# kfkq/DQMC

Measured on AMD Instinct MI355X. Metric: MC sweeps/sec, 2D Hubbard N=256 Ltau=200, higher is better.
Workload: dtype f64; 1 GPU; cfg3: 16x16 Hubbard U=8.0 beta=8.0 Ltau=200 n_stab=10 t=1 mu=-0.1; chains_per_gpu=1, n_chains_total=1, parallelism=independent chains, 1 gpu x 1 chain

## Files before the change

### dqmc_amd/csrc/common.h

```cpp
#pragma once

#include <hip/hip_runtime.h>
#include <cstdint>
#include <memory>
#include <string>

struct dqmc_engine;

namespace dq {

constexpr int WAVE = 64;

void set_error(const std::string& msg);
const char* get_error();

#define DQ_HIP(call)                                                                    \
    do {                                                                                \
        hipError_t _e = (call);                                                         \
        if (_e != hipSuccess) {                                                         \
            ::dq::set_error(std::string(#call) + ": " + hipGetErrorString(_e));         \
            return -2;                                              \
        }                                                                               \
    } while (0)

#define DQ_TRY(expr)                \
    do {                            \
        int _rc = (expr);           \
        if (_rc != 0) return _rc;   \
    } while (0)

template <class T, hipError_t (*Free)(void*)> struct HipDelete { void operator()(T* p) const { (void)Free(p); } };
template <class T> using DevPtr = std::unique_ptr<T[], HipDelete<T, hipFree>>;
using PinnedPtr = std::unique_ptr<char[], HipDelete<char, hipHostFree>>;
template <class T> int dev_alloc(DevPtr<T>& out, size_t count) {
    void* p = nullptr;
    DQ_HIP(hipMalloc(&p, sizeof(T) * count));
    out.reset(static_cast<T*>(p));
    return 0;
}

constexpr int DQ_STATUS_PIVOT = 1;
constexpr int DQ_STATUS_COOP_QR = 2;
constexpr int DQ_STATUS_HANDOFF = 4;
constexpr int DQ_STATUS_CENSUS = 8;

struct Mat {
    double* p = nullptr;
    long stride = 0;
    __host__ __device__ double* at(int c) const { return p + (long)c * stride; }
};
struct CMat {
    const double* p = nullptr;
    long stride = 0;
    CMat() = default;
    __host__ __device__ CMat(const double* p_, long s) : p(p_), stride(s) {}
    __host__ __device__ CMat(const Mat& m) : p(m.p), stride(m.stride) {}
    __host__ __device__ const double* at(int c) const { return p + (long)c * stride; }
};
using Vec = Mat;
using CVec = CMat;

struct GemmDesc {
    CMat A, B;
    Mat C;
    Mat CT{nullptr, 0};
    CVec rs, ks, cs;
    int n = 0;
    int transA = 0;
    int accumulate = 0;
};
int launch_gemm(const GemmDesc& g, int n_chains, hipStream_t s);

int launch_build_expv(const int8_t* fields, long f_stride, int nt, int n, const double* tab_expv ,
                      double* expv, double* invexpv, long v_stride, int n_chains, hipStream_t s);
int launch_split_d(CVec d, Vec dl_inv, Vec ds, double* logsum, int n, int n_chains, hipStream_t s);
int launch_split_d2(CVec d1, Vec dl1, Vec ds1, CVec d2, Vec dl2, Vec ds2, int n, int n_chains, hipStream_t s);
int launch_measure_equal_time(CMat G, double* out, long out_stride, int L1, int L2, int accumulate, int n_chains, hipStream_t s);
int launch_measure_unequal_time(const double* Gtt, const double* Gt0, const double* G0t, double* out, long out_stride, int L1, int L2, int nt,
                                int accumulate, int n_chains, hipStream_t s);
int launch_axpb_identity(CMat in, Mat out, double a, double b, int n, int n_chains, hipStream_t s);
int launch_copy(CMat in, Mat out, long count, int n_chains, hipStream_t s);
int launch_set_identity(Mat out, int n, int n_chains, hipStream_t s);
int launch_transpose_scale(CMat in, Mat out, CVec rs, int n, int n_chains, hipStream_t s);
int launch_max_abs_diff(CMat A, CMat B, double* err, long err_stride, int n, int n_chains, hipStream_t s);
int launch_add_scaled_cols(CMat A, CMat B, CVec cs, Mat C, int n, int n_chains, hipStream_t s);
int launch_scale_rows(CMat in, CVec rs, Mat out, int n, int n_chains, hipStream_t s);
struct DevStats { double acc_rate, max_err, sum_err, n_err; long long n_accepted, n_proposed; };
int launch_fold_stats(DevStats* st, const int* acc, long acc_stride, int n_slices, const double* err, long err_stride, int n_err,
                      int n, int nt, int n_chains, hipStream_t s);

struct QrWork {
    double* tau; long tau_stride;
    int* jpvt; long jpvt_stride;
    unsigned long long* sync = nullptr; long sync_stride = 0;
    int* abort_words = nullptr;
    int* info = nullptr;
    double* pw = nullptr; long pw_stride = 0;
    bool pw_two_launch = false;
    int* pivpos = nullptr; long pivpos_stride = 0;
    bool pw_compact = true;
};
bool qr_panel_fused_fits(int n);
bool qr_panel_fused_default(int n);
long qr_panel_work_doubles(int n, bool two_launch);
int launch_qr_panel(Mat A, Mat L, QrWork w, int n, int n_chains, hipStream_t s);
long qrcp_coop_sync_granules(int n);
int qrcp_coop_workgroups(int n, int n_chains);
enum class QrFamily { Panel, ColumnOwner, Cooperative, Streaming };
int launch_to_ldr(QrFamily f, Mat A, Mat L, Vec d, Mat R, QrWork w, int n, int n_chains, hipStream_t s);

int launch_lu_blocked(Mat A, int* perm, long perm_stride, int* rowpos, long rowpos_stride, double* logabsdet, int accumulate_logdet,
                      int* info, int n, int n_chains, hipStream_t s);
int launch_lu_solve(CMat LU, const int* perm, long perm_stride, Mat X, CVec dg, int mode, int n, int n_chains, hipStream_t s);

int launch_tri_solve(CMat R, const int* perm, long perm_stride, Mat X, CVec dg, double* scratch, long scratch_stride, int n, int n_chains, hipStream_t s);

bool gj_fused_fits(int n);
bool gj_fused_default(int n);
int launch_gj_solve(Mat A, Mat B, Mat X, Mat SA, double* tinv, int* perm, long perm_stride, int* rowpos, int* rowpos_alt, long rowpos_stride,
                    double* logabsdet, int accumulate_logdet, int* info, int n, int n_chains, bool fused, bool compact, hipStream_t s);

struct UpdateTables {
    double rb[4][3];
    double delta[4][3];
    double ev[4];
    double iev[4];
    double pad[32];
};
struct SliceRider {
    const double* A = nullptr; const double* B = nullptr; double* C = nullptr; const double* rs = nullptr; const double* ks = nullptr;
    __host__ __device__ GemmDesc gemm(int n) const { GemmDesc g; g.A = CMat(A, 0); g.B = CMat(B, 0); g.C = Mat{C, 0}; g.rs = CVec(rs, 0); g.ks = CVec(ks, 0); g.n = n; return g; }
};
struct UpdateDesc {
    Mat G;
    int8_t* fields; long f_stride;
    double* expv; double* invexpv; long v_stride;
    const UpdateTables* tabs;
    const int32_t* perm; const uint8_t* kprop; const double* u; long rs_stride;
    double* Upanel; double* Wpanel; long panel_stride;
    double* Cpanel = nullptr;
    int* state; long state_stride;
    double* prep; long prep_stride;
    Mat GT{nullptr, 0};
    int gt_valid = 0;
    void* slice_sync = nullptr;
    unsigned slice_epoch = 0;
    int slice_absent_tile = -1;
    int slice_absent_l = -1;
    int slice_late_tile = -1, slice_late_us = 0;
    int* info = nullptr;
    int* acc_out; long acc_stride;
    int n, nt;
    SliceRider rider;
};
constexpr int UPDATE_KD = 32;

struct SliceSync {
    unsigned long long seq; unsigned int error; unsigned int solo_count; unsigned int pad[12];
    unsigned int arrive[496];
};
constexpr size_t SLICE_SYNC_BYTES = 2048;
static_assert(sizeof(SliceSync) == SLICE_SYNC_BYTES, "SliceSync layout");
constexpr unsigned SLICE_EPOCH_LIMIT = 1u << 24;
constexpr unsigned SLICE_SOLO_BIT = 1u << 30, SLICE_FINAL_BIT = 1u << 31;
constexpr int SLICE_RING_ROWS = 2 * UPDATE_KD;
constexpr unsigned SLICE_K_MASK = 0xffu, SLICE_BASE_SHIFT = 8, SLICE_BASE_MASK = SLICE_RING_ROWS - 1;
__host__ __device__ inline unsigned slice_tag(unsigned epoch, unsigned window) { return (epoch << 8) | window; }
enum class SlicePath { PersistentWalk, PersistentWalkDump, PersistentSubmatrix, Solo, Pairs, PairsTailSolo };
int launch_update_slice(SlicePath path, const UpdateDesc& d, int l, int acc_slot, int n_chains, hipStream_t s);
int launch_update_slice_sm(const UpdateDesc& d, int l, int acc_slot, int n_chains, hipStream_t s);
int slice_flush_workgroups(int n);
bool slice_reserve(int device, int n, int n_chains);
void slice_release(int device, int n, int n_chains);
int launch_rank1(Mat G, int i, double delta, double* scratch , long scratch_stride, int n, int n_chains, hipStream_t s);

int launch_rng_fill(int32_t* perm, uint8_t* kprop, double* u, int n, int nt, unsigned long long seed, unsigned first_chain, unsigned h,
                    int n_chains, hipStream_t s);

struct CbDesc {
    CMat in;
    Mat out{nullptr, 0}, outT{nullptr, 0};
    const int* partner = nullptr;
// ... 20 lines not shown
```

### dqmc_amd/csrc/elementwise.hip

```cpp
#include "common.h"
#include "wave.h"

namespace dq {

__global__ void build_expv_kernel(const int8_t* fields, long f_stride, long total, const double* tab,
                                  double* expv, double* invexpv, long v_stride) {
    const int c = blockIdx.y;
    const double* t = tab + (long)c * 8;
    for (long k = blockIdx.x * (long)blockDim.x + threadIdx.x; k < total; k += (long)gridDim.x * blockDim.x) {
        const int f = fields[(long)c * f_stride + k] & 3;
        expv[(long)c * v_stride + k] = t[f];
        invexpv[(long)c * v_stride + k] = t[4 + f];
    }
}
int launch_build_expv(const int8_t* fields, long f_stride, int nt, int n, const double* tab, double* expv, double* invexpv,
                      long v_stride, int n_chains, hipStream_t s) {
    const long total = (long)nt * n;
    dim3 grid((unsigned)((total + 255) / 256 > 512 ? 512 : (total + 255) / 256), n_chains);
    hipLaunchKernelGGL(build_expv_kernel, grid, dim3(256), 0, s, fields, f_stride, total, tab, expv, invexpv, v_stride);
    DQ_HIP(hipGetLastError());
    return 0;
}

__global__ void split_d_kernel(CVec d, Vec dl_inv, Vec ds, double* logsum, int n) {
// ... 70 lines not shown
    const int ti = blockIdx.x % tiles, tj = blockIdx.x / tiles;
    const int tx = threadIdx.x & 31, ty = threadIdx.x >> 5;
    for (int r = ty; r < 32; r += 8) {
        const int i = ti * 32 + tx, j = tj * 32 + r;
        tile[r][tx] = (i < n && j < n) ? a[i + (long)n * j] : 0.0;
    }
    __syncthreads();
    for (int r = ty; r < 32; r += 8) {
        const int i = tj * 32 + tx, j = ti * 32 + r;
        if (i < n && j < n) {
            double v = tile[tx][r];
            if (rs.p) v *= rs.at(c)[i];
            o[i + (long)n * j] = v;
        }
    }
}
int launch_transpose_scale(CMat in, Mat out, CVec rs, int n, int n_chains, hipStream_t s) {
    const int tiles = (n + 31) / 32;
    hipLaunchKernelGGL(transpose_scale_kernel, dim3(tiles * tiles, n_chains), dim3(256), 0, s, in, out, rs, n, tiles);
    DQ_HIP(hipGetLastError());
    return 0;
}

__global__ __launch_bounds__(256) void max_abs_diff_kernel(CMat A, CMat B, double* err, long err_stride, int n) {
    const int c = blockIdx.y;
    const double* __restrict__ a = A.at(c); const double* __restrict__ b = B.at(c);
    const long total = (long)n * n;
    unsigned long long m = 0ULL;
    for (long k = (long)blockIdx.x * blockDim.x + threadIdx.x; k < total; k += (long)gridDim.x * blockDim.x) {
        const unsigned long long d = (unsigned long long)__double_as_longlong(fabs(a[k] - b[k]));
        m = d > m ? d : m;
    }
    m = wave_max_u64(m);
    __shared__ unsigned long long red[4];
    if ((threadIdx.x & 63) == 0) red[threadIdx.x >> 6] = m;
    __syncthreads();
    if (threadIdx.x == 0) {
        unsigned long long r = red[0];
        for (int q = 1; q < 4; ++q) r = red[q] > r ? red[q] : r;
        atomicMax(reinterpret_cast<unsigned long long*>(err + (long)c * err_stride), r);
    }
}
int launch_max_abs_diff(CMat A, CMat B, double* err, long err_stride, int n, int n_chains, hipStream_t s) {
    const long total = (long)n * n;
    const long want = (total + 4095) / 4096;
    const int blocks = (int)(want < 1 ? 1 : (want > 16 ? 16 : want));
    hipLaunchKernelGGL(max_abs_diff_kernel, dim3(blocks, n_chains), dim3(256), 0, s, A, B, err, err_stride, n);
    DQ_HIP(hipGetLastError());
    return 0;
}

__global__ void add_scaled_cols_kernel(CMat A, CMat B, CVec cs, Mat C, int n) {
    const int c = blockIdx.y;
    const double* a = A.at(c); const double* b = B.at(c); double* o = C.at(c);
    const long total = (long)n * n;
    for (long k = blockIdx.x * (long)blockDim.x + threadIdx.x; k < total; k += (long)gridDim.x * blockDim.x) {
        double bv = b[k];
        if (cs.p) bv *= cs.at(c)[k / n];
        o[k] = a[k] + bv;
    }
}
int launch_add_scaled_cols(CMat A, CMat B, CVec cs, Mat C, int n, int n_chains, hipStream_t s) {
    const long total = (long)n * n;
    long blocks = (total + 255) / 256; if (blocks > 1024) blocks = 1024;
    hipLaunchKernelGGL(add_scaled_cols_kernel, dim3((unsigned)blocks, n_chains), dim3(256), 0, s, A, B, cs, C, n);
    DQ_HIP(hipGetLastError());
    return 0;
}

__global__ void scale_rows_kernel(CMat in, CVec rs, Mat out, int n) {
    const int c = blockIdx.y;
    const double* a = in.at(c); double* o = out.at(c); const double* r = rs.at(c);
    const long total = (long)n * n;
    for (long k = blockIdx.x * (long)blockDim.x + threadIdx.x; k < total; k += (long)gridDim.x * blockDim.x) o[k] = a[k] * r[k % n];
}
int launch_scale_rows(CMat in, CVec rs, Mat out, int n, int n_chains, hipStream_t s) {
    const long total = (long)n * n;
    long blocks = (total + 255) / 256; if (blocks > 1024) blocks = 1024;
    hipLaunchKernelGGL(scale_rows_kernel, dim3((unsigned)blocks, n_chains), dim3(256), 0, s, in, rs, out, n);
    DQ_HIP(hipGetLastError());
    return 0;
}

__global__ void fold_stats_kernel(DevStats* st, const int* acc, long acc_stride, int n_slices, const double* err, long err_stride,
                                  int n_err, int n, int nt, int n_chains) {
    const int c = blockIdx.x * blockDim.x + threadIdx.x;
    if (c >= n_chains) return;
    DevStats s = st[c];
    for (int k = 0; k < n_slices; ++k) {
        const int a = acc[(long)c * acc_stride + k];
        s.acc_rate += (static_cast<double>(a) / n) / nt;
        s.n_accepted += a; s.n_proposed += n;
    }
    for (int k = 0; k < n_err; ++k) {
        const double e = err[(long)c * err_stride + k];
        if (e > s.max_err || e != e) s.max_err = e;
        s.sum_err += e; s.n_err += 1.0;
    }
    st[c] = s;
}
int launch_fold_stats(DevStats* st, const int* acc, long acc_stride, int n_slices, const double* err, long err_stride, int n_err,
                      int n, int nt, int n_chains, hipStream_t s) {
    hipLaunchKernelGGL(fold_stats_kernel, dim3((n_chains + 63) / 64), dim3(64), 0, s, st, acc, acc_stride, n_slices, err, err_stride, n_err, n, nt, n_chains);
    DQ_HIP(hipGetLastError());
    return 0;
}


__global__ __launch_bounds__(1024) void measure_equal_time_kernel(CMat Gm, double* out_p, long out_stride, int L1, int L2, int accumulate) {
    __shared__ double red[3][16];
    __shared__ double s_navg;
    const int chain = blockIdx.y;
    const int n = L1 * L2;
    const double* __restrict__ G = Gm.at(chain);
    double* out = out_p + (long)chain * out_stride;
    const int t = threadIdx.x, lane = t & 63, wave = t >> 6, nwaves = (blockDim.x + 63) >> 6;
    double dens = 0.0, docc = 0.0, sw = 0.0;
    if (t < n) {
        const double c = 1.0 - G[t + (long)n * t];
        dens = 2.0 * c; docc = c * c;
        for (int j = 0; j < n; ++j) { const double x = (j == t ? 1.0 : 0.0) - G[j + (long)n * t]; sw += x * x; }
    }
    dens = wave_sum(dens); docc = wave_sum(docc); sw = wave_sum(sw);
    if (lane == 0) { red[0][wave] = dens; red[1][wave] = docc; red[2][wave] = sw; }
    __syncthreads();
    if (t == 0) {
        double a = 0.0, b = 0.0, c = 0.0;
        for (int q = 0; q < nwaves; ++q) { a += red[0][q]; b += red[1][q]; c += red[2][q]; }
        a /= n; b /= n; c /= n;
        s_navg = a;
        if (accumulate) { out[0] += a; out[1] += b; out[2] += c; } else { out[0] = a; out[1] = b; out[2] = c; }
    }
    __syncthreads();
    if (t < n) {
        const int dx = (t % L1) - (L1 / 2 - 1), dy = (t / L1) - (L2 / 2 - 1);
        const double navg = s_navg;
        double acc = 0.0;
        for (int i = 0; i < n; ++i) {
            const int xi = i % L1, yi = i / L1;
            const int xj = ((xi + dx) % L1 + L1) % L1, yj = ((yi + dy) % L2 + L2) % L2;
            const int j = yj * L1 + xj;
            const double ni = 2.0 * (1.0 - G[i + (long)n * i]), nj = 2.0 * (1.0 - G[j + (long)n * j]);
            acc += ni * nj + 2.0 * (1.0 - G[j + (long)n * i]) * G[i + (long)n * j] - navg * navg;
        }
        acc /= n;
        if (accumulate) out[3 + t] += acc; else out[3 + t] = acc;
    }
}

int launch_measure_equal_time(CMat G, double* out, long out_stride, int L1, int L2, int accumulate, int n_chains, hipStream_t s) {
    const int n = L1 * L2;
    if (n < 1 || n > 1024) { set_error("measure_equal_time: L1*L2 must be in 1..1024"); return -1; }
    const int threads = ((n + 63) / 64) * 64;
    hipLaunchKernelGGL(measure_equal_time_kernel, dim3(1, n_chains), dim3(threads), 0, s, G, out, out_stride, L1, L2, accumulate);
    DQ_HIP(hipGetLastError());
    return 0;
}


__global__ void axpb_identity_kernel(CMat in, Mat out, double a, double b, int n) {
    const int chain = blockIdx.y;
    const double* x = in.at(chain);
    double* y = out.at(chain);
    const long nn = (long)n * n;
    for (long k = (long)blockIdx.x * blockDim.x + threadIdx.x; k < nn; k += (long)gridDim.x * blockDim.x)
        y[k] = a * x[k] + ((k % n) == (k / n) ? b : 0.0);
}
int launch_axpb_identity(CMat in, Mat out, double a, double b, int n, int n_chains, hipStream_t s) {
    hipLaunchKernelGGL(axpb_identity_kernel, dim3(64, n_chains), dim3(256), 0, s, in, out, a, b, n);
    DQ_HIP(hipGetLastError());
    return 0;
}


__global__ __launch_bounds__(1024) void measure_unequal_time_kernel(const double* Gtt_p, const double* Gt0_p, const double* G0t_p, double* out_p,
                                                                    long out_stride, int L1, int L2, int nt, int accumulate, int n_chains) {
    const int tau = blockIdx.x, chain = blockIdx.y;
    const int n = L1 * L2;
    const long nn = (long)n * n;
    const double* __restrict__ Gtt = Gtt_p + ((long)tau * n_chains + chain) * nn;
    const double* __restrict__ Gt0 = Gt0_p + ((long)tau * n_chains + chain) * nn;
    const double* __restrict__ G0t = G0t_p + ((long)tau * n_chains + chain) * nn;
    const double* __restrict__ G00 = Gtt_p + (long)chain * nn;
    double* out = out_p + (long)chain * out_stride;
    const int t = threadIdx.x;
    if (t >= n) return;
// ... 34 lines not shown
```

### dqmc_amd/csrc/engine.hip

```cpp
#include "common.h"
#include "../../include/dqmc_hip.h"

#include <cmath>
#include <cstdlib>
#include <cstring>
#include <map>
#include <memory>
#include <mutex>
#include <vector>

namespace dq {

static thread_local std::string g_err;
void set_error(const std::string& msg) { g_err = msg; }
const char* get_error() { return g_err.c_str(); }

int init_device_kernels(int device) {
    static std::mutex mu; static bool done[64] = {};
    std::lock_guard<std::mutex> lk(mu);
    if (device < 0 || device >= 64) { set_error("device ordinal out of range"); return -1; }
    if (done[device]) return 0;
    DQ_HIP(hipSetDevice(device));
    DQ_TRY(update_init_device()); DQ_TRY(update_sm_init_device()); DQ_TRY(qr_init_device()); DQ_TRY(qr_colown_init_device());
    done[device] = true;
    return 0;
}

struct Switches { bool qr_panel; int qr_panel_fused, gj_fused; bool qr_streaming, walk_submatrix, lu_classic, slice_multikernel, bbar_rider, slice_stream, panel_compact; };
static const Switches& switches() {
    static const Switches sw = [] {
        const char* panel = getenv("DQMC_QR_PANEL");
        const char* fused = getenv("DQMC_QR_PANEL_FUSED");
        const char* gj = getenv("DQMC_GJ_FUSED");
        const char* rider = getenv("DQMC_BBAR_RIDER");
        const char* stream = getenv("DQMC_SLICE_STREAM");
        const char* compact = getenv("DQMC_PANEL_COMPACT");
        return Switches{!(panel && atoi(panel) == 0), fused ? (atoi(fused) != 0 ? 1 : 0) : -1, gj ? (atoi(gj) != 0 ? 1 : 0) : -1, getenv("DQMC_QR_STREAMING") != nullptr, getenv("DQMC_WALK_SUBMATRIX") != nullptr,
                        getenv("DQMC_LU_CLASSIC") != nullptr, getenv("DQMC_SLICE_MULTIKERNEL") != nullptr, !(rider && atoi(rider) == 0), !(stream && atoi(stream) == 0), !(compact && atoi(compact) == 0)};
    }();
    return sw;
}

constexpr int GJ_MAX_N = 1024, GJ_MAX_CHAINS = 8;
constexpr int TRI_MAX_N = 640;

static QrFamily pick_qr(int n, int chains, bool allow_panel) {
    const Switches& sw = switches();
    if (sw.qr_streaming) return QrFamily::Streaming;
    if (allow_panel && sw.qr_panel && n >= 64 && n <= 1024 && n % 16 == 0 && chains <= 8) return QrFamily::Panel;
    if (n <= 256) return QrFamily::ColumnOwner;
    return qrcp_coop_workgroups(n, chains) <= 200 ? QrFamily::Cooperative : QrFamily::Streaming;
}

struct KernelPlan {
    QrFamily qr;
    enum class Solve { GaussJordan, BlockedLu } solve;
    enum class Rinv { Blocked, PerColumn } rinv;
    static KernelPlan pick(int n, int chains) {
        return KernelPlan{pick_qr(n, chains, true),
                          n <= GJ_MAX_N && chains <= GJ_MAX_CHAINS && !switches().lu_classic ? Solve::GaussJordan : Solve::BlockedLu,
                          n <= TRI_MAX_N ? Rinv::Blocked : Rinv::PerColumn};
    }
};

static SlicePath pick_slice_path(int n, int chains, bool reserved) {
    const Switches& sw = switches();
    const bool walk = n <= 256;
    if (sw.slice_multikernel) return SlicePath::Pairs;
    if (reserved) return walk && !sw.walk_submatrix ? (sw.slice_stream ? SlicePath::PersistentWalk : SlicePath::PersistentWalkDump) : SlicePath::PersistentSubmatrix;
    if (!walk) return SlicePath::Pairs;
    return chains >= 224 ? SlicePath::Solo : SlicePath::PairsTailSolo;
}
static bool is_persistent_walk(SlicePath p) { return p == SlicePath::PersistentWalk || p == SlicePath::PersistentWalkDump; }
static bool is_persistent(SlicePath p) { return is_persistent_walk(p) || p == SlicePath::PersistentSubmatrix; }

struct LdrRef {
    Mat L; Vec d; Mat R;
    int* jpvt = nullptr;
    bool* tri = nullptr;
    Mat X{nullptr, 0};
    bool* xok = nullptr;
    void touch() const { if (xok) *xok = false; }
};
struct LdrStore {
    int n = 0, C = 0;
    DevPtr<double> L, d, R, X;
    DevPtr<int> jpvt;
    std::unique_ptr<bool[]> tri, xok;
    int alloc(int k, int n_, int C_, bool with_x = false) {
        n = n_; C = C_;
        const size_t nn = (size_t)n * n;
        DQ_TRY(dev_alloc(L, (size_t)k * C * nn)); DQ_TRY(dev_alloc(d, (size_t)k * C * n));
        DQ_TRY(dev_alloc(R, (size_t)k * C * nn)); DQ_TRY(dev_alloc(jpvt, (size_t)k * C * n));
        if (with_x) DQ_TRY(dev_alloc(X, (size_t)k * C * nn));
        tri.reset(new bool[k]()); xok.reset(new bool[k]());
        return 0;
    }
    LdrRef at(int i) const {
        const long nn = (long)n * n;
        LdrRef f{Mat{L.get() + (long)i * C * nn, nn}, Vec{d.get() + (long)i * C * n, (long)n}, Mat{R.get() + (long)i * C * nn, nn},
                 jpvt.get() + (long)i * C * n, &tri[i]};
        if (X) { f.X = Mat{X.get() + (long)i * C * nn, nn}; f.xok = &xok[i]; }
        return f;
    }
};

struct Ctx {
    int n = 0, C = 0, device = 0;
    long nn = 0;
    hipStream_t stream = nullptr;
    static constexpr int NT = 6, NV = 5;
    DevPtr<double> pool;
    DevPtr<double> vpool;
    DevPtr<int> ipool;
    DevPtr<unsigned long long> qsync;
    DevPtr<int> qabort;
    DevPtr<double> tinv;
    DevPtr<double> qpw;
    bool gj_fused = false;
    bool qpw_two_launch = false;
    DevPtr<int> qpivpos;
    DevPtr<double> trinv;
    KernelPlan plan{};

    Mat T(int k) const { return Mat{pool.get() + (long)k * C * nn, nn}; }
    Vec V(int k) const { return Vec{vpool.get() + (long)k * C * n, (long)n}; }
    int* jpvt() const { return ipool.get(); }
    int* lperm() const { return ipool.get() + (long)C * n; }
    int* rowpos() const { return ipool.get() + 2L * C * n; }
    int* rowpos_alt() const { return ipool.get() + 3L * C * n; }
    int* info() const { return ipool.get() + 4L * C * n; }

    int init(int n_, int C_, int device_) {
        n = n_; C = C_; device = device_; nn = (long)n * n;
        DQ_HIP(hipSetDevice(device));
        DQ_TRY(init_device_kernels(device));
        DQ_HIP(hipStreamCreateWithFlags(&stream, hipStreamNonBlocking));
        DQ_TRY(dev_alloc(pool, (size_t)NT * C * nn));
        DQ_TRY(dev_alloc(vpool, (size_t)NV * C * n));
        DQ_TRY(dev_alloc(ipool, 4L * C * n + 4));
        plan = KernelPlan::pick(n, C);
        if (plan.qr == QrFamily::Cooperative) { DQ_TRY(dev_alloc(qsync, (size_t)qrcp_coop_sync_granules(n) * C)); DQ_TRY(dev_alloc(qabort, C)); }
        if (plan.qr == QrFamily::Panel) {
            const int fused = switches().qr_panel_fused;
            qpw_two_launch = !(fused < 0 ? qr_panel_fused_default(n) : fused == 1 && qr_panel_fused_fits(n));
            const size_t qpw_count = (size_t)qr_panel_work_doubles(n, qpw_two_launch) * C;
            DQ_TRY(dev_alloc(qpw, qpw_count)); DQ_TRY(dev_alloc(qpivpos, (size_t)n * C));
            DQ_HIP(hipMemsetAsync(qpw.get(), 0, sizeof(double) * qpw_count, stream));
        }
        if (plan.solve == KernelPlan::Solve::GaussJordan) {
            DQ_TRY(dev_alloc(tinv, (size_t)2048 * C));
            const int fused = switches().gj_fused;
            gj_fused = fused < 0 ? gj_fused_default(n) : fused == 1 && gj_fused_fits(n);
        }
        if (plan.rinv == KernelPlan::Rinv::Blocked) DQ_TRY(dev_alloc(trinv, (size_t)16 * (n + 16) * C));
        DQ_HIP(hipMemsetAsync(ipool.get(), 0, sizeof(int) * (4L * C * n + 4), stream));
        return 0;
    }
    ~Ctx() { if (stream) (void)hipStreamDestroy(stream); }

    int gemm(CMat A, CMat B, Mat Cm, CVec rs = CVec(), CVec ks = CVec(), CVec cs = CVec(), int transA = 0, int accumulate = 0, Mat CT = Mat{nullptr, 0}) {
        GemmDesc g; g.A = A; g.B = B; g.C = Cm; g.CT = CT; g.rs = rs; g.ks = ks; g.cs = cs; g.n = n; g.transA = transA; g.accumulate = accumulate;
        return launch_gemm(g, C, stream);
    }
    int to_ldr(Mat A, LdrRef out, bool direct = true) {
        const bool keep = direct && out.jpvt != nullptr;
        QrWork w{V(4).p, (long)n, keep ? out.jpvt : jpvt(), (long)n};
        w.sync = qsync.get(); w.sync_stride = qrcp_coop_sync_granules(n); w.abort_words = qabort.get(); w.info = info();
        w.pw = qpw.get(); w.pw_stride = qr_panel_work_doubles(n, qpw_two_launch); w.pw_two_launch = qpw_two_launch; w.pivpos = qpivpos.get(); w.pivpos_stride = n;
        w.pw_compact = switches().panel_compact;
        if (out.tri) *out.tri = keep;
        out.touch();
        return launch_to_ldr(plan.qr, A, out.L, out.d, out.R, w, n, C, stream);
    }
    int r_inverse_scaled(LdrRef F, CVec dinv, Mat scratch, Mat lu_scratch, Mat* Xout) {
        const Mat X = F.X.p ? F.X : scratch;
        *Xout = X;
        if (F.xok && *F.xok) return 0;
        if (F.tri && *F.tri && F.jpvt) {
            if (plan.rinv == KernelPlan::Rinv::Blocked) DQ_TRY(launch_tri_solve(F.R, F.jpvt, n, X, dinv, trinv.get(), 16L * (n + 16), n, C, stream));
            else DQ_TRY(launch_lu_solve(F.R, F.jpvt, n, X, dinv, 2, n, C, stream));
        } else {
            DQ_TRY(launch_copy(F.R, lu_scratch, nn, C, stream));
            DQ_TRY(launch_lu_blocked(lu_scratch, lperm(), n, rowpos(), n, nullptr, 0, info(), n, C, stream));
            DQ_TRY(launch_lu_solve(lu_scratch, lperm(), n, X, dinv, 1, n, C, stream));
        }
        if (F.xok) *F.xok = true;
        return 0;
    }
    int mat_mul_ldr(CMat M, LdrRef F, LdrRef out) {
        DQ_TRY(gemm(M, F.L, T(0), CVec(), CVec(), CVec(F.d)));
        LdrRef q{out.L, out.d, T(1)};
        DQ_TRY(to_ldr(T(0), q));
        if (out.tri) *out.tri = false;
        out.touch();
        return gemm(T(1), F.R, out.R);
    }
    int ldr_mul_mat(LdrRef F, CMat M, LdrRef out) {
        DQ_TRY(gemm(F.R, M, T(0), CVec(F.d)));
        LdrRef q{T(1), out.d, out.R, out.jpvt, out.tri};
        q.xok = out.xok;
        DQ_TRY(to_ldr(T(0), q));
        return gemm(F.L, T(1), out.L);
    }
    int ldr_mul_ldr(LdrRef F1, LdrRef F2, LdrRef out) {
        DQ_TRY(gemm(F1.R, F2.L, T(0), CVec(F1.d), CVec(), CVec(F2.d)));
        LdrRef q{T(1), out.d, T(2)};
        DQ_TRY(to_ldr(T(0), q));
        if (out.tri) *out.tri = false;
        out.touch();
        DQ_TRY(gemm(F1.L, T(1), out.L));
        return gemm(T(2), F2.R, out.R);
    }
    int solve(Mat M, Mat RHS, Mat out, double* logdet_acc, Mat* Y) {
        if (plan.solve == KernelPlan::Solve::GaussJordan) {
            DQ_TRY(launch_gj_solve(M, RHS, out, T(5), tinv.get(), lperm(), n, rowpos(), rowpos_alt(), n, logdet_acc, 1, info(), n, C, gj_fused, switches().panel_compact, stream));
            *Y = out; return 0;
        }
        DQ_TRY(launch_lu_blocked(M, lperm(), n, rowpos(), n, logdet_acc, 1, info(), n, C, stream));
        DQ_TRY(launch_lu_solve(M, lperm(), n, RHS, CVec(), 0, n, C, stream));
        *Y = RHS; return 0;
    }
    int inv_I_plus_ldr(LdrRef F, Mat G, double* logdet ) {
        DQ_TRY(launch_split_d(F.d, V(0), V(1), logdet, n, C, stream));
        Mat X; DQ_TRY(r_inverse_scaled(F, V(0), T(1), T(0), &X));
        DQ_TRY(launch_add_scaled_cols(X, F.L, V(1), T(2), n, C, stream));
        DQ_TRY(launch_transpose_scale(T(2), T(3), CVec(), n, C, stream));
        DQ_TRY(launch_transpose_scale(X, T(4), CVec(), n, C, stream));
        Mat Y; DQ_TRY(solve(T(3), T(4), T(0), logdet, &Y));
        return launch_transpose_scale(Y, G, CVec(), n, C, stream);
    }
    int inv_I_plus_ldr_mul_ldr(LdrRef F1, LdrRef F2, Mat G, Mat GT = Mat{nullptr, 0}) {
        DQ_TRY(launch_split_d2(F1.d, V(0), V(1), F2.d, V(2), V(3), n, C, stream));
        Mat X; DQ_TRY(r_inverse_scaled(F2, V(2), T(1), T(0), &X));
        DQ_TRY(gemm(F1.L, X, T(2), V(0), CVec(), CVec(), 1));
        DQ_TRY(gemm(F1.R, F2.L, T(2), V(1), CVec(), V(3), 0, 1));
        DQ_TRY(launch_transpose_scale(F1.L, T(3), V(0), n, C, stream));
        Mat Y; DQ_TRY(solve(T(2), T(3), T(0), nullptr, &Y));
        return gemm(X, Y, G, CVec(), CVec(), CVec(), 0, 0, GT);
    }
    int inv_invldr_plus_ldr(LdrRef F1, LdrRef F2, Mat G, bool negate) {
        DQ_TRY(launch_split_d(F1.d, V(0), V(1), nullptr, n, C, stream));
        DQ_TRY(launch_split_d(F2.d, V(2), V(3), nullptr, n, C, stream));
        Mat X; DQ_TRY(r_inverse_scaled(F2, V(2), T(1), T(0), &X));
        DQ_TRY(gemm(F1.L, X, T(2), V(0), CVec(), CVec(), 1));
        DQ_TRY(gemm(F1.R, F2.L, T(2), V(1), CVec(), V(3), 0, 1));
        DQ_TRY(launch_scale_rows(F1.R, V(1), T(3), n, C, stream));
        Mat Y; DQ_TRY(solve(T(2), T(3), T(0), nullptr, &Y));
        DQ_TRY(gemm(X, Y, G));
        if (negate) DQ_TRY(launch_axpb_identity(G, G, -1.0, 0.0, n, C, stream));
        return 0;
    }
};

static int take_status(const Ctx& c, int* bits = nullptr) {
    int w[4] = {0, 0, 0, 0};
    DQ_HIP(hipMemcpy(w, c.info(), sizeof w, hipMemcpyDeviceToHost));
    if (bits) *bits = w[0];
    if (w[0] == 0) return 0;
    (void)hipMemset(c.info(), 0, sizeof w);
    if (w[0] & DQ_STATUS_HANDOFF) {
        set_error("persistent slice kernel: a workgroup that had checked in stopped answering (device fault or pre-emption beyond the spin bound); the chain state is undefined -- set the fields again and call dqmc_init; this engine uses the scan / flush kernel pairs from now on");
    } else if (w[0] & DQ_STATUS_CENSUS) {
        char msg[640];
        snprintf(msg, sizeof msg, "persistent sub-matrix slice kernel: its workgroups did not all become resident at time slice %d (device shared with other "
                 "work?).  That slice and every later slice of the call(s) in flight proposed NOTHING (fields unchanged there, acceptance counts 0, their part of "
                 "the random stream is spent); wraps and stabilisations ran, so fields, G and the stack are consistent with each other, but the sweep is not the "
                 "one the stream describes from that slice on.  This engine uses the scan / flush kernel pairs from now on: restore the fields of the last "
                 "completed sweep and call dqmc_init, or keep the state as a valid (shortened) sweep", w[1] - 1);
        set_error(msg);
    } else if (w[0] & DQ_STATUS_COOP_QR) {
        set_error("cooperative QRCP gave up waiting for a partner workgroup (not co-resident?)");
    } else {
        set_error("LU factorisation hit a zero or NaN pivot");
    }
    return DQMC_ENUMERIC;
}

struct Engine {
    int n = 0, nt = 0, n_stab = 0, n_stack = 0, C = 1, device = 0;
    long nn = 0;
    std::vector<int> loc_l_end;
    std::vector<double> g_host, gamma_host, eta_host;
    std::vector<unsigned char> seen;
    Ctx ctx;
    hipStream_t s = nullptr;

    DevPtr<double> expK, invexpK;
    bool cb = false; int cb_groups = 0;
    DevPtr<int> cb_partner;
    DevPtr<double> cb_par;
    DevPtr<int8_t> fields;
    DevPtr<double> expv, invexpv;
    DevPtr<UpdateTables> tabs; DevPtr<double> tab8;
    bool gt_valid = false;
    bool gt_check = false; long long gt_checks = 0; DevPtr<double> gt_err;
    DevPtr<double> G, Gtmp, GT;
    DevPtr<double> pg_eye, pg_ones;
    DevPtr<double> bb0, bb1;
    long long rider_launches = 0;
    LdrStore stack;
    LdrStore spare;
    DevPtr<double> logdet;
    DevPtr<int32_t> rs_perm; DevPtr<uint8_t> rs_k; DevPtr<double> rs_u;
    PinnedPtr h_stage;
    bool rng_seeded = false; uint64_t rng_seed = 0; uint32_t rng_first_chain = 0, rng_counter = 0;
    hipEvent_t stage_free = nullptr;
    DevPtr<double> Upanel, Wpanel;
    int panel_rows = UPDATE_KD;
    DevPtr<double> Cpanel;
    struct InitBatch { DevPtr<double> bb, tau; LdrStore f; } ib;
    DevPtr<int> state;
    DevPtr<double> prep;
    DevPtr<double> meas_now, meas_sum;
    struct UnequalTime { DevPtr<double> G[3], tmp, err, meas_now, meas_sum; LdrStore bt; } ut;
    bool ut_valid = false; long long ut_meas_count = 0;
    struct HalfWarp { DevPtr<double> expK, invexpK, out; } hw;
    long long meas_count = 0;
    DevPtr<char> slice_sync;
    bool reserved = false;
    SlicePath slice_path = SlicePath::Pairs;
    unsigned slice_epoch = 0;
    int slice_absent_l = -1;
    int slice_late_tile = -1, slice_late_us = 0;
    int slice_absent_tile = -1;
    DevPtr<int> acc;
    struct Exchange { DevPtr<int8_t> saved, recv; DevPtr<int> tab; } xch;
    DevPtr<double> err;
    DevPtr<DevStats> dstats;
    bool stack_valid = false;
    bool profiling = false;
    std::vector<std::pair<hipEvent_t, hipEvent_t>> ev_pairs;
    size_t ev_used = 0;
    double upd_ms = 0.0; long long upd_launches = 0; long long upd_accept_base = 0;

    Mat mG() const { return Mat{G.get(), nn}; }
    CVec ev(int l) const { return CVec(expv.get() + (long)l * n, (long)nt * n); }
    CVec iev(int l) const { return CVec(invexpv.get() + (long)l * n, (long)nt * n); }
    int stack_idx(int l) const { return l / n_stab; }
    int local_l(int l) const { return l % n_stab; }

    ~Engine() {
        if (s) (void)hipStreamSynchronize(s);
        if (reserved) slice_release(device, n, C);
        for (auto& p : ev_pairs) { (void)hipEventDestroy(p.first); (void)hipEventDestroy(p.second); }
        if (stage_free) (void)hipEventDestroy(stage_free);
    }

    int create(int device_, int C_, int n_, int nt_, int n_stab_, const double* g, const double* gamma, const double* eta,
               const double* eK, const double* ieK) {
        device = device_; C = C_; n = n_; nt = nt_; n_stab = n_stab_; nn = (long)n * n;
        n_stack = (int)std::ceil(static_cast<double>(nt) / n_stab);
        loc_l_end.assign(n_stack, n_stab - 1);
        if (nt % n_stab != 0) loc_l_end[n_stack - 1] = nt % n_stab - 1;
        g_host.assign(g, g + C); gamma_host.assign(gamma, gamma + 4); eta_host.assign(eta, eta + 4);
        DQ_TRY(ctx.init(n, C, device)); s = ctx.stream;
        reserved = slice_reserve(device, n, C);
        slice_path = pick_slice_path(n, C, reserved);
        if (const char* a = getenv("DQMC_DEBUG_SLICE_ABSENT")) { slice_absent_tile = atoi(a); if (const char* c = strchr(a, ':')) slice_absent_l = atoi(c + 1); }
        if (const char* a = getenv("DQMC_DEBUG_SLICE_LATE")) { slice_late_tile = atoi(a); if (const char* c = strchr(a, ':')) slice_late_us = atoi(c + 1); }
        DQ_TRY(dev_alloc(expK, C * nn)); DQ_TRY(dev_alloc(invexpK, C * nn));
        DQ_TRY(dev_alloc(fields, (size_t)C * nt * n)); DQ_TRY(dev_alloc(expv, (size_t)C * nt * n)); DQ_TRY(dev_alloc(invexpv, (size_t)C * nt * n));
        DQ_TRY(dev_alloc(tabs, C)); DQ_TRY(dev_alloc(tab8, (size_t)C * 8));
        if (C == 1) { DQ_TRY(dev_alloc(pg_eye, nn)); DQ_TRY(dev_alloc(pg_ones, (size_t)n)); DQ_TRY(launch_set_identity(Mat{pg_eye.get(), nn}, n, 1, s)); const std::vector<double> one_h((size_t)n, 1.0); DQ_HIP(hipMemcpy(pg_ones.get(), one_h.data(), sizeof(double) * n, hipMemcpyHostToDevice)); }
        DQ_TRY(dev_alloc(G, C * nn)); DQ_TRY(dev_alloc(Gtmp, C * nn)); DQ_TRY(dev_alloc(GT, C * nn)); DQ_TRY(dev_alloc(bb0, C * nn)); DQ_TRY(dev_alloc(bb1, C * nn));
        DQ_TRY(stack.alloc(n_stack, n, C, C <= 8)); DQ_TRY(spare.alloc(1, n, C));
        DQ_TRY(dev_alloc(logdet, C));
        DQ_TRY(dev_alloc(rs_perm, (size_t)C * nt * n)); DQ_TRY(dev_alloc(rs_k, (size_t)C * nt * n)); DQ_TRY(dev_alloc(rs_u, (size_t)C * nt * n));
        panel_rows = slice_path == SlicePath::PersistentWalk ? SLICE_RING_ROWS : UPDATE_KD;
        DQ_TRY(dev_alloc(Upanel, (size_t)C * panel_rows * n)); DQ_TRY(dev_alloc(Wpanel, (size_t)C * panel_rows * n)); DQ_TRY(dev_alloc(Cpanel, (size_t)C * UPDATE_KD * UPDATE_KD));
        DQ_TRY(dev_alloc(state, (size_t)C * 4)); DQ_TRY(dev_alloc(prep, (size_t)C * 4 * n)); DQ_TRY(dev_alloc(meas_now, (size_t)C * (3 + n))); DQ_TRY(dev_alloc(meas_sum, (size_t)C * (3 + n))); DQ_HIP(hipMemsetAsync(meas_sum.get(), 0, sizeof(double) * C * (3 + n), s)); DQ_TRY(dev_alloc(slice_sync, (size_t)C * SLICE_SYNC_BYTES)); DQ_HIP(hipMemsetAsync(slice_sync.get(), 0, (size_t)C * SLICE_SYNC_BYTES, s)); DQ_TRY(dev_alloc(acc, (size_t)C * nt)); DQ_TRY(dev_alloc(err, (size_t)C * n_stack));
        DQ_TRY(dev_alloc(dstats, C));
        void* stage = nullptr;
        DQ_HIP(hipHostMalloc(&stage, (size_t)C * nt * n * (sizeof(int32_t) + sizeof(uint8_t) + sizeof(double)), hipHostMallocDefault)); h_stage.reset(static_cast<char*>(stage));
        DQ_HIP(hipEventCreateWithFlags(&stage_free, hipEventDisableTiming));
        DQ_HIP(hipEventRecord(stage_free, s));
        DQ_HIP(hipMemcpyAsync(expK.get(), eK, sizeof(double) * C * nn, hipMemcpyHostToDevice, s));
        DQ_HIP(hipMemcpyAsync(invexpK.get(), ieK, sizeof(double) * C * nn, hipMemcpyHostToDevice, s));
        DQ_HIP(hipMemsetAsync(fields.get(), 0, (size_t)C * nt * n, s));
        DQ_HIP(hipMemsetAsync(G.get(), 0, sizeof(double) * C * nn, s));
        DQ_HIP(hipMemsetAsync(dstats.get(), 0, sizeof(DevStats) * C, s));
        DQ_HIP(hipMemsetAsync(logdet.get(), 0, sizeof(double) * C, s));
        DQ_HIP(hipMemsetAsync(state.get(), 0, sizeof(int) * C * 4, s));
        std::vector<UpdateTables> ht(C); std::vector<double> h8((size_t)C * 8);
        static const int proposal[4][3] = {{1, 2, 3}, {0, 2, 3}, {0, 1, 3}, {0, 1, 2}};
        const double alpha = -1.0;
        for (int c = 0; c < C; ++c) {
            std::memset(&ht[c], 0, sizeof(UpdateTables));
            for (int o = 0; o < 4; ++o) for (int k = 0; k < 3; ++k) {
                const int nf = proposal[o][k];
                const double gammaR = gamma[nf] / gamma[o];
                const double d_eta = eta[nf] - eta[o];
                const double bosonR = std::exp(alpha * g[c] * d_eta);
                ht[c].rb[o][k] = gammaR * bosonR;
                ht[c].delta[o][k] = (1.0 / bosonR) - 1.0;
            }
            for (int f = 0; f < 4; ++f) { ht[c].ev[f] = std::exp(g[c] * eta[f]); ht[c].iev[f] = std::exp(-g[c] * eta[f]); h8[(size_t)c * 8 + f] = ht[c].ev[f]; h8[(size_t)c * 8 + 4 + f] = ht[c].iev[f]; }
        }
        DQ_HIP(hipMemcpyAsync(tabs.get(), ht.data(), sizeof(UpdateTables) * C, hipMemcpyHostToDevice, s));
        DQ_HIP(hipMemcpyAsync(tab8.get(), h8.data(), sizeof(double) * C * 8, hipMemcpyHostToDevice, s));
        DQ_TRY(launch_build_expv(fields.get(), (long)nt * n, nt, n, tab8.get(), expv.get(), invexpv.get(), (long)nt * n, C, s));
        DQ_HIP(hipStreamSynchronize(s));
        return 0;
    }

    int cb_apply(CMat in, Mat out, Mat outT, bool reverse, bool inverse, CVec rs_in, CVec cs_in, CVec rs_out, CVec cs_out, int chains, long par_stride) {
        CbDesc d; d.in = in; d.out = out; d.outT = outT; d.partner = cb_partner.get(); d.n_groups = cb_groups; d.reverse = reverse ? 1 : 0; d.inverse = inverse ? 1 : 0;
        d.par = cb_par.get(); d.par_stride = par_stride; d.rs_in = rs_in; d.cs_in = cs_in; d.rs_out = rs_out; d.cs_out = cs_out; d.n = n;
        return launch_cb_apply(d, chains, s);
    }
    int set_checkerboard(int n_groups, const int32_t* bonds, const int32_t* group_sizes, const double* ch, const double* sh, const double* f) {
        if (n_groups < 1 || n_groups > 64 || !bonds || !group_sizes || !ch || !sh || !f) { set_error("set_checkerboard: bad argument"); return DQMC_EINVAL; }
        if (n > 4096) { set_error("set_checkerboard: n_sites > 4096"); return DQMC_EINVAL; }
        std::vector<int> partner((size_t)n_groups * n);
        size_t b = 0;
        for (int g = 0; g < n_groups; ++g) {
            int* pt = partner.data() + (size_t)g * n;
            for (int i = 0; i < n; ++i) pt[i] = i;
            if (group_sizes[g] < 0 || group_sizes[g] > n / 2) { set_error("set_checkerboard: a group holds at most n_sites/2 bonds"); return DQMC_EINVAL; }
            for (int k = 0; k < group_sizes[g]; ++k, ++b) {
                const int i = bonds[2 * b], j = bonds[2 * b + 1];
                if (i < 0 || i >= n || j < 0 || j >= n || i == j) { set_error("set_checkerboard: bond site out of range"); return DQMC_EINVAL; }
                if (pt[i] != i || pt[j] != j) { set_error("set_checkerboard: the bonds of one group must be disjoint"); return DQMC_EINVAL; }
                pt[i] = j; pt[j] = i;
            }
        }
        std::vector<double> par((size_t)C * 4);
        for (int c = 0; c < C; ++c) {
            if (!(f[c] > 0.0) || !std::isfinite(ch[c]) || !std::isfinite(sh[c])) { set_error("set_checkerboard: diag_factor must be positive, cosh / sinh finite"); return DQMC_EINVAL; }
            par[4 * c] = ch[c]; par[4 * c + 1] = sh[c]; par[4 * c + 2] = f[c]; par[4 * c + 3] = 1.0 / f[c];
        }
        DQ_HIP(hipStreamSynchronize(s));
        if (!cb_par) DQ_TRY(dev_alloc(cb_par, (size_t)C * 4));
        DevPtr<int> pt;
        DQ_TRY(dev_alloc(pt, partner.size()));
        DQ_HIP(hipMemcpy(pt.get(), partner.data(), sizeof(int) * partner.size(), hipMemcpyHostToDevice));
        DQ_HIP(hipMemcpy(cb_par.get(), par.data(), sizeof(double) * par.size(), hipMemcpyHostToDevice));
        cb_partner = std::move(pt); cb_groups = n_groups; cb = true;
        Mat id{bb0.get(), nn};
        DQ_TRY(launch_set_identity(id, n, C, s));
        DQ_TRY(cb_apply(id, Mat{expK.get(), nn}, Mat{nullptr, 0}, false, false, CVec(), CVec(), CVec(), CVec(), C, 4));
        DQ_TRY(cb_apply(id, Mat{invexpK.get(), nn}, Mat{nullptr, 0}, true, true, CVec(), CVec(), CVec(), CVec(), C, 4));
        stack_valid = false; gt_valid = false; ut_valid = false;
        DQ_HIP(hipStreamSynchronize(s));
        return 0;
    }

    int Bbar(int is, Mat* out) {
        const int l0 = is * n_stab;
        Mat cur{bb0.get(), nn}, nxt{bb1.get(), nn};
        DQ_TRY(launch_scale_rows(CMat(expK.get(), nn), ev(l0), cur, n, C, s));
        for (int loc = 1; loc <= loc_l_end[is]; ++loc) {
            if (cb) DQ_TRY(cb_apply(cur, nxt, Mat{nullptr, 0}, false, false, CVec(), CVec(), ev(l0 + loc), CVec(), C, 4));
            else DQ_TRY(ctx.gemm(CMat(expK.get(), nn), cur, nxt, ev(l0 + loc)));
// ... 77 lines not shown
        gt_valid = use_gt();
        GemmDesc g; g.A = CMat(ctx.T(0).p, (long)(Pprev - ctx.T(0).p)); g.B = CMat(expK.get(), 0); g.C = Mat{G.get(), (long)(Pnext - G.get())};
        g.ks = CVec(expv.get() + (long)l * n, 0); g.n = n;
        if (use_gt()) g.CT = Mat{GT.get(), (long)(ctx.T(1).p - GT.get())};
        return launch_gemm(g, 2, s);
    }
    int wrap_backward(int l) {
        if (cb) {
            DQ_TRY(cb_apply(mG(), Mat{nullptr, 0}, ctx.T(0), true, true, iev(l), ev(l), CVec(), CVec(), C, 4));
            gt_valid = use_gt();
            return cb_apply(ctx.T(0), Mat{GT.get(), nn}, mG(), true, false, CVec(), CVec(), CVec(), CVec(), C, 4);
        }
        DQ_TRY(ctx.gemm(CMat(invexpK.get(), nn), mG(), ctx.T(0), CVec(), iev(l)));
        gt_valid = use_gt();
        return ctx.gemm(ctx.T(0), CMat(expK.get(), nn), mG(), CVec(), ev(l), CVec(), 0, 0, use_gt() ? Mat{GT.get(), nn} : Mat{nullptr, 0});
    }
    bool use_gt() const { return n <= 256 || slice_path == SlicePath::PersistentSubmatrix; }
    UpdateDesc udesc() const {
        UpdateDesc d; d.G = mG(); d.fields = fields.get(); d.f_stride = (long)nt * n; d.expv = expv.get(); d.invexpv = invexpv.get(); d.v_stride = (long)nt * n;
        d.tabs = tabs.get(); d.perm = rs_perm.get(); d.kprop = rs_k.get(); d.u = rs_u.get(); d.rs_stride = (long)nt * n; d.Upanel = Upanel.get(); d.Wpanel = Wpanel.get(); d.Cpanel = Cpanel.get();
        d.panel_stride = (long)panel_rows * n; d.state = state.get(); d.state_stride = 4; d.prep = prep.get(); d.prep_stride = 4L * n; d.slice_sync = is_persistent(slice_path) ? slice_sync.get() : nullptr; d.slice_epoch = slice_epoch; d.slice_absent_tile = slice_absent_tile; d.slice_absent_l = slice_absent_l; d.slice_late_tile = slice_late_tile; d.slice_late_us = slice_late_us; d.GT = Mat{GT.get(), nn}; d.gt_valid = gt_valid ? 1 : 0; d.info = ctx.info(); d.acc_out = acc.get(); d.acc_stride = nt; d.n = n; d.nt = nt;
        return d;
    }
    int local_update(int l, const SliceRider* rider = nullptr) {
        hipEvent_t e0 = nullptr, e1 = nullptr;
        if (profiling) {
            if (ev_used == ev_pairs.size()) { hipEvent_t a, b; DQ_HIP(hipEventCreate(&a)); DQ_HIP(hipEventCreate(&b)); ev_pairs.emplace_back(a, b); }
            e0 = ev_pairs[ev_used].first; e1 = ev_pairs[ev_used].second; ++ev_used;
            DQ_HIP(hipEventRecord(e0, s));
        }
        if (is_persistent(slice_path)) {
            if (++slice_epoch >= SLICE_EPOCH_LIMIT) { DQ_HIP(hipMemsetAsync(slice_sync.get(), 0, (size_t)C * SLICE_SYNC_BYTES, s)); slice_epoch = 1; }
        }
        UpdateDesc d = udesc();
        if (rider) d.rider = *rider;
        DQ_TRY(launch_update_slice(slice_path, d, l, l, C, s));
        if (rider) ++rider_launches;
        if (profiling) DQ_HIP(hipEventRecord(e1, s));
        return 0;
    }
    int check_stream(const char* who, const int32_t* perm, const uint8_t* kprop, const double* u, size_t rows) {
        if (!perm || !kprop || !u) { set_error(std::string(who) + ": null random-stream pointer"); return DQMC_EINVAL; }
        seen.assign((size_t)n, 0);
        for (size_t row = 0; row < rows; ++row) {
            const int32_t* pr = perm + row * n; const uint8_t* kr = kprop + row * n; const unsigned char mark = (unsigned char)(1 + (row & 1));
            if ((row & 1) == 0) std::fill(seen.begin(), seen.end(), 0);
            for (int idx = 0; idx < n; ++idx) {
                const int32_t i = pr[idx];
                if (i < 0 || i >= n || seen[i] == mark || kr[idx] > 2) { set_error(std::string(who) + ": perm is not a permutation of the sites, or kprop > 2"); return DQMC_EINVAL; }
                seen[i] = mark;
            }
        }
        return 0;
    }
    int upload_stream(const int32_t* perm, const uint8_t* kprop, const double* u) {
        const size_t cnt = (size_t)C * nt * n;
        DQ_TRY(check_stream("sweep", perm, kprop, u, (size_t)C * nt));
        DQ_HIP(hipEventSynchronize(stage_free));
        char* base = h_stage.get();
        double* hu = reinterpret_cast<double*>(base);
        int32_t* hp = reinterpret_cast<int32_t*>(base + cnt * sizeof(double));
        uint8_t* hk = reinterpret_cast<uint8_t*>(base + cnt * (sizeof(double) + sizeof(int32_t)));
        std::memcpy(hu, u, cnt * sizeof(double)); std::memcpy(hp, perm, cnt * sizeof(int32_t)); std::memcpy(hk, kprop, cnt);
        DQ_HIP(hipMemcpyAsync(rs_u.get(), hu, cnt * sizeof(double), hipMemcpyHostToDevice, s));
        DQ_HIP(hipMemcpyAsync(rs_perm.get(), hp, cnt * sizeof(int32_t), hipMemcpyHostToDevice, s));
        DQ_HIP(hipMemcpyAsync(rs_k.get(), hk, cnt, hipMemcpyHostToDevice, s));
        DQ_HIP(hipEventRecord(stage_free, s));
        return 0;
    }
    int fill_stream(uint32_t h) {
        return launch_rng_fill(rs_perm.get(), rs_k.get(), rs_u.get(), n, nt, rng_seed, rng_first_chain, h, C, s);
    }
    int stage_stream(const char* who, const int32_t* perm, const uint8_t* kprop, const double* u) {
        if (perm && kprop && u) return upload_stream(perm, kprop, u);
        if (perm || kprop || u) { set_error(std::string(who) + ": pass all three random-stream arrays or none"); return DQMC_EINVAL; }
        if (!rng_seeded) { set_error(std::string(who) + ": null random-stream pointer (the engine draws its own stream only after dqmc_rng_seed)"); return DQMC_EINVAL; }
        if (rng_counter == UINT32_MAX) { set_error(std::string(who) + ": the half-sweep counter of this seed is used up (2^32 - 1)"); return DQMC_ERANGE; }
        DQ_TRY(fill_stream(rng_counter));
        ++rng_counter;
        return 0;
    }
    int sweep_fwd() {
        int n_err = 0;
        DQ_HIP(hipMemsetAsync(err.get(), 0, sizeof(double) * C * n_stack, s));
        const bool pg = piggyback(), ride = bbar_rides();
        double* Pcur = bb0.get(); double* Pnxt = bb1.get();
        for (int l = 0; l < nt; ++l) {
            const int is = stack_idx(l), loc = local_l(l);
            if (pg && loc >= 1) {
                const double* Pprev = loc == 1 ? pg_eye.get() : Pcur;
                if (ride) { const SliceRider r = rider_forward(l, Pprev, Pnxt); DQ_TRY(wrap_forward(l)); DQ_TRY(local_update(l, &r)); }
                else { DQ_TRY(wrap_forward_piggy(l, Pprev, Pnxt)); DQ_TRY(local_update(l)); }
                std::swap(Pcur, Pnxt);
            } else { DQ_TRY(wrap_forward(l)); DQ_TRY(local_update(l)); }
            if (loc == loc_l_end[is]) {
                std::swap(G, Gtmp);
                Mat bb;
                if (pg) {
                    if (loc == 0) DQ_TRY(launch_scale_rows(CMat(expK.get(), nn), ev(l), Mat{Pnxt, nn}, n, C, s));
                    else DQ_TRY(ctx.gemm(CMat(expK.get(), nn), CMat(Pcur, nn), Mat{Pnxt, nn}, ev(l)));
                    std::swap(Pcur, Pnxt); bb = Mat{Pcur, nn};
                } else DQ_TRY(Bbar(is, &bb));
                if (is == 0) DQ_TRY(ctx.to_ldr(bb, stack.at(0)));
                else DQ_TRY(ctx.mat_mul_ldr(bb, stack.at(is - 1), stack.at(is)));
                gt_valid = false;
                if (l == nt - 1) DQ_TRY(ctx.inv_I_plus_ldr(stack.at(is), mG(), logdet.get()));
                else DQ_TRY(ctx.inv_I_plus_ldr_mul_ldr(stack.at(is), stack.at(is + 1), mG()));
                DQ_TRY(launch_max_abs_diff(CMat(Gtmp.get(), nn), mG(), err.get() + n_err, n_stack, n, C, s));
                ++n_err;
            }
        }
        return launch_fold_stats(dstats.get(), acc.get(), nt, nt, err.get(), n_stack, n_err, n, nt, C, s);
    }
    int sweep_bwd() {
        int n_err = 0;
        DQ_HIP(hipMemsetAsync(err.get(), 0, sizeof(double) * C * n_stack, s));
        const bool pg = piggyback(), ride = bbar_rides();
        double* Pcur = bb0.get(); double* Pnxt = bb1.get();
        SliceRider pending; bool have_pending = false;
        for (int l = nt - 1; l >= 0; --l) {
            DQ_TRY(local_update(l, have_pending ? &pending : nullptr));
            if (have_pending) { std::swap(Pcur, Pnxt); have_pending = false; }
            const int is = stack_idx(l);
            if (pg) {
                const double* Pprev = local_l(l) == loc_l_end[is] ? pg_eye.get() : Pcur;
                if (ride && local_l(l) != 0) { DQ_TRY(wrap_backward(l)); pending = rider_backward(l, Pprev, Pnxt); have_pending = true; }
                else { DQ_TRY(wrap_backward_piggy(l, Pprev, Pnxt)); std::swap(Pcur, Pnxt); }
            } else DQ_TRY(wrap_backward(l));
            if (local_l(l) == 0) {
                std::swap(G, Gtmp);
                Mat bb;
                if (pg) bb = Mat{Pcur, nn}; else DQ_TRY(Bbar(is, &bb));
                if (is == n_stack - 1) DQ_TRY(ctx.to_ldr(bb, stack.at(is)));
                else DQ_TRY(ctx.ldr_mul_mat(stack.at(is + 1), bb, stack.at(is)));
                gt_valid = false;
                if (l == 0) DQ_TRY(ctx.inv_I_plus_ldr(stack.at(is), mG(), logdet.get()));
                else {
                    DQ_TRY(ctx.inv_I_plus_ldr_mul_ldr(stack.at(is - 1), stack.at(is), mG(), use_gt() ? Mat{GT.get(), nn} : Mat{nullptr, 0}));
                    gt_valid = use_gt();
                    if (gt_check && gt_valid) {
                        DQ_TRY(launch_transpose_scale(mG(), ctx.T(0), CVec(), n, C, s));
                        DQ_TRY(launch_max_abs_diff(CMat(GT.get(), nn), ctx.T(0), gt_err.get(), 1, n, C, s));
                        ++gt_checks;
                    }
                }
                DQ_TRY(launch_max_abs_diff(CMat(Gtmp.get(), nn), mG(), err.get() + n_err, n_stack, n, C, s));
                ++n_err;
            }
        }
        return launch_fold_stats(dstats.get(), acc.get(), nt, nt, err.get(), n_stack, n_err, n, nt, C, s);
    }
    Mat utm(int which, int l) const { return Mat{ut.G[which].get() + (long)l * C * nn, nn}; }
    int sweep_unequal() {
        if (!ut.tmp) {
            UnequalTime u;
            for (int w = 0; w < 3; ++w) DQ_TRY(dev_alloc(u.G[w], (size_t)(nt + 1) * C * nn));
            DQ_TRY(dev_alloc(u.tmp, (size_t)3 * C * nn)); DQ_TRY(dev_alloc(u.err, (size_t)C * 3 * n_stack));
            const size_t mcount = (size_t)C * 3 * (nt + 1) * n;
            DQ_TRY(dev_alloc(u.meas_now, mcount)); DQ_TRY(dev_alloc(u.meas_sum, mcount)); DQ_TRY(u.bt.alloc(2, n, C));
            DQ_HIP(hipMemsetAsync(u.meas_sum.get(), 0, sizeof(double) * mcount, s));
            ut = std::move(u);
        }
        auto bt = [&](int b) { return ut.bt.at(b); };
        int cur = 0, n_err = 0;
        DQ_HIP(hipMemsetAsync(ut.err.get(), 0, sizeof(double) * C * 3 * n_stack, s));
        DQ_TRY(launch_copy(mG(), utm(0, 0), nn, C, s));
        for (int l = 0; l < nt; ++l) {
            if (l == 0) {
                DQ_TRY(launch_copy(utm(0, 0), utm(1, 0), nn, C, s));
                DQ_TRY(launch_axpb_identity(utm(0, 0), utm(2, 0), 1.0, -1.0, n, C, s));
            }
            DQ_TRY(ctx.gemm(CMat(expK.get(), nn), utm(0, l), ctx.T(0)));
            DQ_TRY(ctx.gemm(ctx.T(0), CMat(invexpK.get(), nn), utm(0, l + 1), ev(l), CVec(), iev(l)));
            DQ_TRY(ctx.gemm(CMat(expK.get(), nn), utm(1, l), utm(1, l + 1), ev(l)));
            DQ_TRY(ctx.gemm(utm(2, l), CMat(invexpK.get(), nn), utm(2, l + 1), CVec(), CVec(), iev(l)));
            const int is = stack_idx(l);
            if (local_l(l) == loc_l_end[is]) {
                for (int w = 0; w < 3; ++w) DQ_TRY(launch_copy(utm(w, l + 1), Mat{ut.tmp.get() + (long)w * C * nn, nn}, nn, C, s));
                Mat bb; DQ_TRY(Bbar(is, &bb));
                if (is == 0) DQ_TRY(ctx.to_ldr(bb, bt(cur)));
                else { DQ_TRY(ctx.mat_mul_ldr(bb, bt(cur), bt(cur ^ 1))); cur ^= 1; }
                if (l == nt - 1) {
                    DQ_TRY(ctx.inv_I_plus_ldr(bt(cur), utm(0, l + 1), logdet.get()));
                    DQ_TRY(launch_axpb_identity(utm(0, l + 1), utm(1, l + 1), -1.0, 1.0, n, C, s));
                    DQ_TRY(launch_axpb_identity(utm(0, l + 1), utm(2, l + 1), -1.0, 0.0, n, C, s));
                } else {
                    DQ_TRY(ctx.inv_I_plus_ldr_mul_ldr(bt(cur), stack.at(is + 1), utm(0, l + 1)));
                    DQ_TRY(ctx.inv_invldr_plus_ldr(bt(cur), stack.at(is + 1), utm(1, l + 1), false));
                    DQ_TRY(ctx.inv_invldr_plus_ldr(stack.at(is + 1), bt(cur), utm(2, l + 1), true));
                }
                for (int w = 0; w < 3; ++w) {
                    DQ_TRY(launch_max_abs_diff(CMat(ut.tmp.get() + (long)w * C * nn, nn), utm(w, l + 1), ut.err.get() + n_err, 3L * n_stack, n, C, s));
                    ++n_err;
                }
            }
        }
        ut_valid = true;
        return launch_fold_stats(dstats.get(), acc.get(), nt, 0, ut.err.get(), 3L * n_stack, n_err, n, nt, C, s);
    }
    int sync_and_check() {
        DQ_HIP(hipStreamSynchronize(s));
        if (profiling && ev_used) {
            for (size_t k = 0; k < ev_used; ++k) { float ms = 0.f; DQ_HIP(hipEventElapsedTime(&ms, ev_pairs[k].first, ev_pairs[k].second)); upd_ms += ms; }
            upd_launches += (long long)ev_used; ev_used = 0;
        }
        int bits = 0;
        const int rc = take_status(ctx, &bits);
        if (bits & (DQ_STATUS_HANDOFF | DQ_STATUS_CENSUS)) {
            slice_path = pick_slice_path(n, C, false); gt_valid = false;
            if (bits & DQ_STATUS_HANDOFF) { (void)hipMemset(slice_sync.get(), 0, (size_t)C * SLICE_SYNC_BYTES); slice_epoch = 0; }
        }
        return rc;
    }
    int download_fields(std::vector<int8_t>& f) const {
        std::vector<int8_t> dev((size_t)C * nt * n);
        DQ_HIP(hipMemcpy(dev.data(), fields.get(), dev.size(), hipMemcpyDeviceToHost));
        f.resize(dev.size());
        for (int c = 0; c < C; ++c) for (int i = 0; i < n; ++i) for (int l = 0; l < nt; ++l)
            f[(size_t)c * nt * n + l + (size_t)nt * i] = dev[(size_t)c * nt * n + (size_t)l * n + i];
        return 0;
    }
    int copy_out_equal_time(const double* src, double* scalars, double* chi_r) const {
        const size_t w = 3 + (size_t)n;
        std::vector<double> tmp((size_t)C * w);
        DQ_HIP(hipMemcpy(tmp.data(), src, sizeof(double) * tmp.size(), hipMemcpyDeviceToHost));
        for (int c = 0; c < C; ++c) {
            if (scalars) std::copy(tmp.begin() + c * w, tmp.begin() + c * w + 3, scalars + 3 * (size_t)c);
            if (chi_r) std::copy(tmp.begin() + c * w + 3, tmp.begin() + (c + 1) * w, chi_r + (size_t)c * n);
        }
        return 0;
    }
};

struct Stateless {
    Ctx ctx;
    LdrStore ldr;
    DevPtr<double> mats;
    DevPtr<double> logdet;
    Mat M(int k) const { return Mat{mats.get() + k * ctx.nn, ctx.nn}; }
};
static std::mutex g_ctx_mu;
static std::map<int, std::unique_ptr<Stateless>> g_ctx;

static int get_ctx(int n, Stateless** out) {
    if (n <= 0) { set_error("n must be positive"); return DQMC_EINVAL; }
    int count = 0;
    if (hipGetDeviceCount(&count) != hipSuccess || count == 0) { set_error("no HIP device available: this library requires a gfx950 GPU"); return DQMC_ENODEVICE; }
    auto it = g_ctx.find(n);
    if (it == g_ctx.end()) {
        std::unique_ptr<Stateless> x(new Stateless);
        DQ_TRY(x->ctx.init(n, 1, 0));
        DQ_TRY(x->ldr.alloc(3, n, 1)); DQ_TRY(dev_alloc(x->mats, 4L * n * n)); DQ_TRY(dev_alloc(x->logdet, 1));
        it = g_ctx.emplace(n, std::move(x)).first;
    }
    *out = it->second.get();
    return hipSetDevice(0) == hipSuccess ? 0 : DQMC_ENODEVICE;
}
static int upload_ldr(Stateless* x, int k, const double* L, const double* d, const double* R, LdrRef* out) {
    const Ctx& c = x->ctx;
    *out = x->ldr.at(k); *out->tri = false;
    DQ_HIP(hipMemcpyAsync(out->L.p, L, sizeof(double) * c.nn, hipMemcpyHostToDevice, c.stream));
    DQ_HIP(hipMemcpyAsync(out->R.p, R, sizeof(double) * c.nn, hipMemcpyHostToDevice, c.stream));
    DQ_HIP(hipMemcpyAsync(out->d.p, d, sizeof(double) * c.n, hipMemcpyHostToDevice, c.stream));
    return 0;
}
static int download_ldr(Ctx* c, LdrRef f, double* L, double* d, double* R) {
    DQ_HIP(hipMemcpyAsync(L, f.L.p, sizeof(double) * c->nn, hipMemcpyDeviceToHost, c->stream));
    DQ_HIP(hipMemcpyAsync(R, f.R.p, sizeof(double) * c->nn, hipMemcpyDeviceToHost, c->stream));
    DQ_HIP(hipMemcpyAsync(d, f.d.p, sizeof(double) * c->n, hipMemcpyDeviceToHost, c->stream));
    DQ_HIP(hipStreamSynchronize(c->stream));
    return take_status(*c);
}

}

using namespace dq;

struct dqmc_engine { Engine e; };

#define ENGINE_CALL(h) if (!(h)) { set_error("null engine"); return DQMC_EINVAL; } Engine& e = (h)->e; DQ_HIP(hipSetDevice(e.device))

namespace dq {
int engine_fields_view(dqmc_engine* h, EngineFieldsView* v) {
    if (!h || !v) { set_error("null engine"); return DQMC_EINVAL; }
    Engine& e = h->e;
    v->device = e.device; v->n = e.n; v->nt = e.nt; v->n_chains = e.C; v->fields = e.fields.get(); v->stream = e.s;
    return 0;
}
int engine_fields_changed(dqmc_engine* h) {
    ENGINE_CALL(h);
    e.stack_valid = false; e.gt_valid = false;
    return launch_build_expv(e.fields.get(), (long)e.nt * e.n, e.nt, e.n, e.tab8.get(), e.expv.get(), e.invexpv.get(), (long)e.nt * e.n, e.C, e.s);
}
int engine_exchange_scratch(dqmc_engine* h, int8_t** saved, int8_t** recv, int** tab) {
    ENGINE_CALL(h);
    if (!e.xch.tab) {
        Engine::Exchange x; DQ_TRY(dev_alloc(x.saved, (size_t)e.C * e.nt * e.n)); DQ_TRY(dev_alloc(x.recv, (size_t)2 * e.nt * e.n)); DQ_TRY(dev_alloc(x.tab, (size_t)2 * e.C));
        e.xch = std::move(x);
    }
    *saved = e.xch.saved.get(); *recv = e.xch.recv.get(); *tab = e.xch.tab.get();
    return 0;
}
}

#define API_LOCK std::lock_guard<std::mutex> _lk(g_ctx_mu)

extern "C" {

const char* dqmc_last_error(void) { return get_error(); }
const char* dqmc_backend(void) { return "hip:gfx950"; }
int dqmc_device_count(void) { int c = 0; if (hipGetDeviceCount(&c) != hipSuccess) return 0; return c; }

int dqmc_to_ldr(int n, const double* M, double* L, double* d, double* R) {
    API_LOCK; Stateless* x; DQ_TRY(get_ctx(n, &x)); Ctx* c = &x->ctx;
    if (!M || !L || !d || !R) { set_error("null pointer"); return DQMC_EINVAL; }
    DQ_HIP(hipMemcpyAsync(x->M(0).p, M, sizeof(double) * c->nn, hipMemcpyHostToDevice, c->stream));
    LdrRef out = x->ldr.at(0);
    DQ_TRY(c->to_ldr(x->M(0), out));
    return download_ldr(c, out, L, d, R);
}
int dqmc_ldr_mul_mat(int n, const double* L, const double* d, const double* R, const double* M, double* Lo, double* d_o, double* Ro) {
    API_LOCK; Stateless* x; DQ_TRY(get_ctx(n, &x)); Ctx* c = &x->ctx;
    LdrRef F; DQ_TRY(upload_ldr(x, 0, L, d, R, &F));
    DQ_HIP(hipMemcpyAsync(x->M(0).p, M, sizeof(double) * c->nn, hipMemcpyHostToDevice, c->stream));
    LdrRef out = x->ldr.at(2);
    DQ_TRY(c->ldr_mul_mat(F, x->M(0), out));
    return download_ldr(c, out, Lo, d_o, Ro);
}
int dqmc_mat_mul_ldr(int n, const double* M, const double* L, const double* d, const double* R, double* Lo, double* d_o, double* Ro) {
    API_LOCK; Stateless* x; DQ_TRY(get_ctx(n, &x)); Ctx* c = &x->ctx;
    LdrRef F; DQ_TRY(upload_ldr(x, 0, L, d, R, &F));
    DQ_HIP(hipMemcpyAsync(x->M(0).p, M, sizeof(double) * c->nn, hipMemcpyHostToDevice, c->stream));
    LdrRef out = x->ldr.at(2);
    DQ_TRY(c->mat_mul_ldr(x->M(0), F, out));
    return download_ldr(c, out, Lo, d_o, Ro);
}
int dqmc_ldr_mul_ldr(int n, const double* L1, const double* d1, const double* R1, const double* L2, const double* d2, const double* R2, double* Lo, double* d_o, double* Ro) {
    API_LOCK; Stateless* x; DQ_TRY(get_ctx(n, &x)); Ctx* c = &x->ctx;
    LdrRef F1, F2; DQ_TRY(upload_ldr(x, 0, L1, d1, R1, &F1)); DQ_TRY(upload_ldr(x, 1, L2, d2, R2, &F2));
    LdrRef out = x->ldr.at(2);
    DQ_TRY(c->ldr_mul_ldr(F1, F2, out));
    return download_ldr(c, out, Lo, d_o, Ro);
}
// ... 93 lines not shown
    DQ_HIP(hipMemcpy(e.G.get(), G, sizeof(double) * e.C * e.nn, hipMemcpyHostToDevice)); e.gt_valid = false; return 0;
}
int dqmc_get_logdet(dqmc_engine* h, double* ld) {
    ENGINE_CALL(h); DQ_TRY(e.sync_and_check());
    DQ_HIP(hipMemcpy(ld, e.logdet.get(), sizeof(double) * e.C, hipMemcpyDeviceToHost)); return 0;
}
int dqmc_n_stack(dqmc_engine* h) { return h ? h->e.n_stack : 0; }
int dqmc_get_stack(dqmc_engine* h, int i, double* L, double* d, double* R) {
    ENGINE_CALL(h);
    if (i < 0 || i >= e.n_stack) { set_error("LDR Stack index out of bounds"); return DQMC_ERANGE; }
    if (!e.stack_valid) { set_error("stack not initialised: call dqmc_init first"); return DQMC_EINVAL; }
    DQ_TRY(e.sync_and_check());
    LdrRef f = e.stack.at(i);
    DQ_HIP(hipMemcpy(L, f.L.p, sizeof(double) * e.C * e.nn, hipMemcpyDeviceToHost));
    DQ_HIP(hipMemcpy(R, f.R.p, sizeof(double) * e.C * e.nn, hipMemcpyDeviceToHost));
    DQ_HIP(hipMemcpy(d, f.d.p, sizeof(double) * e.C * e.n, hipMemcpyDeviceToHost));
    return 0;
}
int dqmc_sweep_0_to_beta(dqmc_engine* h, const int32_t* perm, const uint8_t* kprop, const double* u) {
    ENGINE_CALL(h);
    if (!e.stack_valid) { set_error("dqmc_init must be called before sweeping"); return DQMC_EINVAL; }
    DQ_TRY(e.stage_stream("sweep_0_to_beta", perm, kprop, u)); return e.sweep_fwd();
}
int dqmc_sweep_beta_to_0(dqmc_engine* h, const int32_t* perm, const uint8_t* kprop, const double* u) {
    ENGINE_CALL(h);
    if (!e.stack_valid) { set_error("dqmc_init must be called before sweeping"); return DQMC_EINVAL; }
    DQ_TRY(e.stage_stream("sweep_beta_to_0", perm, kprop, u)); return e.sweep_bwd();
}
int dqmc_sync(dqmc_engine* h) { ENGINE_CALL(h); return e.sync_and_check(); }
int dqmc_rng_seed(dqmc_engine* h, uint64_t seed, uint32_t first_chain, uint32_t counter) {
    ENGINE_CALL(h);
    if ((uint64_t)first_chain + (uint64_t)e.C - 1 > UINT32_MAX) { set_error("rng_seed: first_chain + n_chains - 1 exceeds 32 bits"); return DQMC_EINVAL; }
    e.rng_seeded = true; e.rng_seed = seed; e.rng_first_chain = first_chain; e.rng_counter = counter;
    return 0;
}
int dqmc_rng_state(dqmc_engine* h, uint64_t* seed, uint32_t* first_chain, uint32_t* counter, int* seeded) {
    if (!h) { set_error("null engine"); return DQMC_EINVAL; }
    const Engine& e = h->e;
    if (seed) *seed = e.rng_seed;
    if (first_chain) *first_chain = e.rng_first_chain;
    if (counter) *counter = e.rng_counter;
    if (seeded) *seeded = e.rng_seeded ? 1 : 0;
    return 0;
}
int dqmc_rng_draw(dqmc_engine* h, uint32_t counter, int32_t* perm, uint8_t* kprop, double* u) {
    ENGINE_CALL(h);
    if (!perm || !kprop || !u) { set_error("rng_draw: null pointer"); return DQMC_EINVAL; }
    if (!e.rng_seeded) { set_error("rng_draw: the engine has no seed (dqmc_rng_seed)"); return DQMC_EINVAL; }
    DQ_TRY(e.fill_stream(counter));
    DQ_TRY(e.sync_and_check());
    const size_t cnt = (size_t)e.C * e.nt * e.n;
    DQ_HIP(hipMemcpy(perm, e.rs_perm.get(), cnt * sizeof(int32_t), hipMemcpyDeviceToHost));
    DQ_HIP(hipMemcpy(kprop, e.rs_k.get(), cnt, hipMemcpyDeviceToHost));
    DQ_HIP(hipMemcpy(u, e.rs_u.get(), cnt * sizeof(double), hipMemcpyDeviceToHost));
    return 0;
}
int dqmc_get_stats(dqmc_engine* h, dqmc_stats* out) {
    ENGINE_CALL(h); DQ_TRY(e.sync_and_check());
    static_assert(sizeof(DevStats) == sizeof(dqmc_stats), "stats layout");
    DQ_HIP(hipMemcpy(out, e.dstats.get(), sizeof(DevStats) * e.C, hipMemcpyDeviceToHost)); return 0;
}
int dqmc_wrap_forward(dqmc_engine* h, int l) {
    ENGINE_CALL(h);
    if (l < 0 || l >= e.nt) { set_error("time slice out of range"); return DQMC_ERANGE; }
    return e.wrap_forward(l);
}
int dqmc_wrap_backward(dqmc_engine* h, int l) {
    ENGINE_CALL(h);
    if (l < 0 || l >= e.nt) { set_error("time slice out of range"); return DQMC_ERANGE; }
    return e.wrap_backward(l);
}
int dqmc_local_update_slice(dqmc_engine* h, int l, const int32_t* perm, const uint8_t* kprop, const double* u, int* accepted) {
    ENGINE_CALL(h);
    if (l < 0 || l >= e.nt) { set_error("time slice out of range"); return DQMC_ERANGE; }
    DQ_TRY(e.check_stream("local_update_slice", perm, kprop, u, e.C));
    DQ_HIP(hipStreamSynchronize(e.s));
    for (int c = 0; c < e.C; ++c) {
        const size_t off = ((size_t)c * e.nt + l) * e.n;
        DQ_HIP(hipMemcpy(e.rs_perm.get() + off, perm + (size_t)c * e.n, sizeof(int32_t) * e.n, hipMemcpyHostToDevice));
        DQ_HIP(hipMemcpy(e.rs_k.get() + off, kprop + (size_t)c * e.n, e.n, hipMemcpyHostToDevice));
        DQ_HIP(hipMemcpy(e.rs_u.get() + off, u + (size_t)c * e.n, sizeof(double) * e.n, hipMemcpyHostToDevice));
    }
    DQ_TRY(e.local_update(l));
    DQ_TRY(launch_fold_stats(e.dstats.get(), e.acc.get() + l, e.nt, 1, e.err.get(), e.n_stack, 0, e.n, e.nt, e.C, e.s));
    DQ_TRY(e.sync_and_check());
    if (accepted) for (int c = 0; c < e.C; ++c) DQ_HIP(hipMemcpy(accepted + c, e.acc.get() + (size_t)c * e.nt + l, sizeof(int), hipMemcpyDeviceToHost));
    return 0;
}
int dqmc_rng_fill_time(dqmc_engine* h, int launches, double* ms_per_launch) {
    ENGINE_CALL(h);
    if (launches < 1 || !ms_per_launch) { set_error("rng_fill_time: launches >= 1 and a result pointer"); return DQMC_EINVAL; }
    if (!e.rng_seeded) { set_error("rng_fill_time: the engine has no seed (dqmc_rng_seed)"); return DQMC_EINVAL; }
    hipEvent_t e0 = nullptr, e1 = nullptr;
    DQ_HIP(hipEventCreate(&e0));
    if (hipEventCreate(&e1) != hipSuccess) { (void)hipEventDestroy(e0); set_error("rng_fill_time: hipEventCreate failed"); return DQMC_ENODEVICE; }
    int rc = e.fill_stream(e.rng_counter);
    if (rc == 0 && hipEventRecord(e0, e.s) != hipSuccess) rc = DQMC_ENODEVICE;
    for (int k = 0; k < launches && rc == 0; ++k) rc = e.fill_stream(e.rng_counter);
    if (rc == 0 && hipEventRecord(e1, e.s) != hipSuccess) rc = DQMC_ENODEVICE;
    if (rc == 0) rc = e.sync_and_check();
    float ms = 0.f;
    if (rc == 0 && hipEventElapsedTime(&ms, e0, e1) != hipSuccess) rc = DQMC_ENODEVICE;
    (void)hipEventDestroy(e0); (void)hipEventDestroy(e1);
    if (rc == 0) *ms_per_launch = (double)ms / launches;
    return rc;
}
int dqmc_calculate_Bbar(dqmc_engine* h, int is, double* out) {
    ENGINE_CALL(h);
    if (is < 0 || is >= e.n_stack) { set_error("stack index out of range"); return DQMC_ERANGE; }
    Mat bb; DQ_TRY(e.Bbar(is, &bb)); DQ_HIP(hipStreamSynchronize(e.s));
    DQ_HIP(hipMemcpy(out, bb.p, sizeof(double) * e.C * e.nn, hipMemcpyDeviceToHost)); return 0;
}
int dqmc_global_action(dqmc_engine* h, double* S) {
    ENGINE_CALL(h); DQ_TRY(e.sync_and_check());
    std::vector<int8_t> tmp; std::vector<double> ld(e.C);
    DQ_TRY(e.download_fields(tmp));
    DQ_HIP(hipMemcpy(ld.data(), e.logdet.get(), sizeof(double) * e.C, hipMemcpyDeviceToHost));
    const double alpha = -1.0;
    const size_t per = (size_t)e.nt * e.n;
    for (int c = 0; c < e.C; ++c) {
        double lb = 0.0, lg = 0.0;
        for (size_t k = 0; k < per; ++k) {
            const int f = tmp[c * per + k];
            lb += alpha * e.g_host[c] * e.eta_host[f]; lg += std::log(e.gamma_host[f]);
        }
        S[c] = -2.0 * ld[c] - (lb + lg);
    }
    return 0;
}
int dqmc_sweep_unequal_time(dqmc_engine* h) {
    ENGINE_CALL(h);
    if (!e.stack_valid) { set_error("sweep_unequal_time: call dqmc_init first"); return DQMC_EINVAL; }
    return e.sweep_unequal();
}
int dqmc_get_G_tau(dqmc_engine* h, int which, int l, double* out) {
    ENGINE_CALL(h);
    if (which < 0 || which > 2 || l < 0 || l > e.nt) { set_error("get_G_tau: which in 0..2, l in 0..nt"); return DQMC_ERANGE; }
    if (!e.ut_valid) { set_error("get_G_tau: run dqmc_sweep_unequal_time first"); return DQMC_EINVAL; }
    DQ_TRY(e.sync_and_check());
    DQ_HIP(hipMemcpy(out, e.utm(which, l).p, sizeof(double) * e.C * e.nn, hipMemcpyDeviceToHost));
    return 0;
}
int dqmc_half_warp(dqmc_engine* h, const double* expK_half, const double* invexpK_half, int which, int l, double* out) {
    ENGINE_CALL(h);
    if (!out) { set_error("half_warp: out is NULL"); return DQMC_EINVAL; }
    if (which < -1 || which > 2 || (which >= 0 && (l < 0 || l > e.nt))) { set_error("half_warp: which in -1..2, l in 0..nt"); return DQMC_ERANGE; }
    if (which >= 0 && !e.ut_valid) { set_error("half_warp: run dqmc_sweep_unequal_time first"); return DQMC_EINVAL; }
    if ((expK_half == nullptr) != (invexpK_half == nullptr)) { set_error("half_warp: pass both half-step matrices or neither"); return DQMC_EINVAL; }
    if (expK_half) {
        if (!e.hw.out) { Engine::HalfWarp x; DQ_TRY(dev_alloc(x.expK, e.nn)); DQ_TRY(dev_alloc(x.invexpK, e.nn)); DQ_TRY(dev_alloc(x.out, (size_t)e.C * e.nn)); e.hw = std::move(x); }
        DQ_HIP(hipStreamSynchronize(e.s));
        DQ_HIP(hipMemcpy(e.hw.expK.get(), expK_half, sizeof(double) * e.nn, hipMemcpyHostToDevice));
        DQ_HIP(hipMemcpy(e.hw.invexpK.get(), invexpK_half, sizeof(double) * e.nn, hipMemcpyHostToDevice));
    } else if (!e.hw.out) { set_error("half_warp: no half-step matrices uploaded yet"); return DQMC_EINVAL; }
    const CMat M = which < 0 ? CMat(e.mG()) : CMat(e.utm(which, l));
    DQ_TRY(e.ctx.gemm(CMat(e.hw.invexpK.get(), 0), M, e.ctx.T(0)));
    DQ_TRY(e.ctx.gemm(e.ctx.T(0), CMat(e.hw.expK.get(), 0), Mat{e.hw.out.get(), e.nn}));
    DQ_TRY(e.sync_and_check());
    DQ_HIP(hipMemcpy(out, e.hw.out.get(), sizeof(double) * e.C * e.nn, hipMemcpyDeviceToHost));
    return 0;
}
int dqmc_measure_unequal_time(dqmc_engine* h, int L1, int L2, int accumulate, double* out) {
    ENGINE_CALL(h);
    if (L1 < 1 || L2 < 1 || L1 * L2 != e.n) { set_error("measure_unequal_time: L1*L2 must equal n_sites"); return DQMC_EINVAL; }
    if (!e.ut_valid) { set_error("measure_unequal_time: run dqmc_sweep_unequal_time first"); return DQMC_EINVAL; }
    const long stride = 3L * (e.nt + 1) * e.n;
    if (accumulate) {
// ... 89 lines not shown
```

### dqmc_amd/csrc/gemm.hip

```cpp
#include "common.h"
#include "gemm_tile.h"
#include <cstdlib>

namespace dq {

using d4 = __attribute__((ext_vector_type(4))) double;

template <bool TRANSA, bool GUARD>
__global__ __launch_bounds__(256) void gemm_kernel(GemmDesc g, int tiles_per_dim) {
    const int chain = blockIdx.y;
    const int n = g.n;
    const double* __restrict__ A = g.A.at(chain);
    const double* __restrict__ B = g.B.at(chain);
    double* __restrict__ C = g.C.at(chain);
    const double* __restrict__ ks = g.ks.p ? g.ks.at(chain) : nullptr;

    const int lane = threadIdx.x & 63;
    const int wave = threadIdx.x >> 6;
    const int bt_i = blockIdx.x % tiles_per_dim, bt_j = blockIdx.x / tiles_per_dim;
    const int i0 = bt_i * 32 + (wave & 1) * 16;
    const int j0 = bt_j * 32 + (wave >> 1) * 16;
    if (GUARD && (i0 >= n || j0 >= n)) return;

    const int r = lane & 15, kk = lane >> 4;
    const int ia = i0 + r;
    const int jb = j0 + r;
    const bool ia_ok = !GUARD || ia < n, jb_ok = !GUARD || jb < n;

    d4 acc = {0.0, 0.0, 0.0, 0.0};
#pragma unroll 2
    for (int k0 = 0; k0 < n; k0 += 16) {
        const int kb = k0 + 4 * kk;
        double av[4], bv[4];
#pragma unroll
        for (int s = 0; s < 4; ++s) {
            const int k = kb + s;
            const bool k_ok = !GUARD || k < n;
            bv[s] = (k_ok && jb_ok) ? B[k + (long)n * jb] : 0.0;
            double a = 0.0;
            if (k_ok && ia_ok) {
                a = TRANSA ? A[k + (long)n * ia] : A[ia + (long)n * k];
                if (ks) a *= ks[k];
            }
            av[s] = a;
        }
#pragma unroll
        for (int s = 0; s < 4; ++s) acc = __builtin_amdgcn_mfma_f64_16x16x4f64(bv[s], av[s], acc, 0, 0, 0);
    }
    if (ia_ok) {
        const double rsv = g.rs.p ? g.rs.at(chain)[ia] : 1.0;
#pragma unroll
        for (int reg = 0; reg < 4; ++reg) {
            const int j = j0 + kk + 4 * reg;
            if (!GUARD || j < n) {
                double v = acc[reg] * rsv;
                if (g.cs.p) v *= g.cs.at(chain)[j];
                double* dst = C + ia + (long)n * j;
                if (g.accumulate) v += *dst;
                *dst = v;
            }
        }
    }
}

template <bool TRANSA, int KQ >
__global__ __launch_bounds__(256) void gemm_splitk_kernel(GemmDesc g, int tiles_per_dim) {
    __shared__ double part[4][4][64];
    gemm_splitk_tile<TRANSA, KQ>(g, blockIdx.y, (blockIdx.x % tiles_per_dim) * 16, (blockIdx.x / tiles_per_dim) * 16, part);
}

template <bool TRANSA>
__global__ __launch_bounds__(256) void gemm_tile64_kernel(GemmDesc g, int tiles_per_dim) {
    constexpr int LDT = 80;
    __shared__ double As[2][16][LDT];
    __shared__ double Bs[2][16][LDT];
    const int tiles2 = tiles_per_dim * tiles_per_dim;
    const int total = tiles2 * (int)gridDim.y;
    int lin = (int)blockIdx.x + tiles2 * (int)blockIdx.y;
    if ((total & 7) == 0) lin = (lin & 7) * (total >> 3) + (lin >> 3);
    const int chain = lin / tiles2, tile = lin % tiles2;
    const int n = g.n;
    const double* __restrict__ A = g.A.at(chain);
    const double* __restrict__ B = g.B.at(chain);
    double* __restrict__ C = g.C.at(chain);
    const double* __restrict__ ks = g.ks.p ? g.ks.at(chain) : nullptr;
    const int t = threadIdx.x, lane = t & 63, wave = t >> 6;
    const int i0 = (tile % tiles_per_dim) * 64, j0 = (tile / tiles_per_dim) * 64;
    const int r = lane & 15, kk = lane >> 4;
    const int wi = (wave & 1) * 32, wj = (wave >> 1) * 32;
    const int ai = t & 63, akq = t >> 6;
    const int bkp = t & 7, bj = t >> 3;
    double ra[4]; double2 rb0, rb1;
    auto load_stage = [&](int kb) {
#pragma unroll
        for (int s = 0; s < 4; ++s) {
            const int k = kb + 4 * akq + s;
            double v = TRANSA ? A[k + (long)n * (i0 + ai)] : A[(i0 + ai) + (long)n * k];
            if (ks) v *= ks[k];
            ra[s] = v;
        }
        rb0 = *reinterpret_cast<const double2*>(B + (kb + 2 * bkp) + (long)n * (j0 + bj));
        rb1 = *reinterpret_cast<const double2*>(B + (kb + 2 * bkp) + (long)n * (j0 + bj + 32));
    };
    auto store_stage = [&](int buf) {
#pragma unroll
        for (int s = 0; s < 4; ++s) As[buf][4 * akq + s][ai] = ra[s];
        Bs[buf][2 * bkp][bj] = rb0.x; Bs[buf][2 * bkp + 1][bj] = rb0.y;
        Bs[buf][2 * bkp][bj + 32] = rb1.x; Bs[buf][2 * bkp + 1][bj + 32] = rb1.y;
    };
    d4 acc[2][2];
#pragma unroll
    for (int a = 0; a < 2; ++a)
#pragma unroll
        for (int b = 0; b < 2; ++b) acc[a][b] = d4{0.0, 0.0, 0.0, 0.0};
    load_stage(0); store_stage(0);
    __syncthreads();
    const int nstage = n / 16;
    for (int st = 0; st < nstage; ++st) {
        const int buf = st & 1;
        if (st + 1 < nstage) load_stage(16 * (st + 1));
#pragma unroll
        for (int q = 0; q < 4; ++q) {
            const int k = 4 * q + kk;
            const double a0 = As[buf][k][wi + r], a1 = As[buf][k][wi + 16 + r];
            const double b0 = Bs[buf][k][wj + r], b1 = Bs[buf][k][wj + 16 + r];
            acc[0][0] = __builtin_amdgcn_mfma_f64_16x16x4f64(b0, a0, acc[0][0], 0, 0, 0);
            acc[0][1] = __builtin_amdgcn_mfma_f64_16x16x4f64(b1, a0, acc[0][1], 0, 0, 0);
            acc[1][0] = __builtin_amdgcn_mfma_f64_16x16x4f64(b0, a1, acc[1][0], 0, 0, 0);
            acc[1][1] = __builtin_amdgcn_mfma_f64_16x16x4f64(b1, a1, acc[1][1], 0, 0, 0);
        }
        if (st + 1 < nstage) store_stage(buf ^ 1);
        __syncthreads();
    }
#pragma unroll
    for (int ti = 0; ti < 2; ++ti) {
        const int i = i0 + wi + 16 * ti + r;
        const double rsv = g.rs.p ? g.rs.at(chain)[i] : 1.0;
#pragma unroll
        for (int tj = 0; tj < 2; ++tj)
#pragma unroll
            for (int reg = 0; reg < 4; ++reg) {
                const int j = j0 + wj + 16 * tj + kk + 4 * reg;
                double v = acc[ti][tj][reg] * rsv;
                if (g.cs.p) v *= g.cs.at(chain)[j];
                double* dst = C + i + (long)n * j;
                if (g.accumulate) v += *dst;
                *dst = v;
            }
    }
}

// ... 54 lines not shown
            const double* qpa = pa[s] + st * sa; const double* qpb = pb[s] + st * KS;
            DQ_GLOAD(a[s], qpa); DQ_GLOAD(b[s], qpb);
            if (HAS_KS) { const double* qpk = pk[s] + st * KS; DQ_GLOAD(kf[s], qpk); }
        }
    };
#undef DQ_GLOAD
    auto wait_stage = [&](double (&a)[NL], double (&b)[NL], double (&kf)[NL]) {
#pragma unroll
        for (int s = 0; s < NL; ++s) asm volatile("s_waitcnt vmcnt(%3)" : "+v"(a[s]), "+v"(b[s]), "+v"(kf[s]) : "n"((D - 1) * LPS) : "memory");
    };
    static_assert((D - 1) * LPS <= 63, "vmcnt is a 6-bit counter");
    auto store_stage = [&](int st, const double (&a)[NL], const double (&b)[NL], const double (&kf)[NL]) {
        const bool masked = !interior || (ragged && st == nst - 1);
#pragma unroll
        for (int s = 0; s < NL; ++s) {
            const int xk = rhi + 8 * s, xr = khi + XS * s;
            double va = a[s], vb = b[s];
            if (HAS_KS) va *= kf[s];
            if (masked) {
                const int k = KS * st + (TRANSA ? klo : xk), row = i0 + (TRANSA ? xr : rlo);
                if (!(k < n && row < n)) va = 0.0;
                if (!(KS * st + klo < n && j0 + xr < n)) vb = 0.0;
            }
            if (TRANSA) As[xr * PK + klo] = va; else As[xk * PR + rlo] = va;
            Bs[xr * PK + klo] = vb;
        }
    };
#pragma unroll
    for (int u = 0; u < D; ++u) load_stage(min(u, nst - 1), qa[u], qb[u], qk[u]);
    d4 acc = {0.0, 0.0, 0.0, 0.0}, acc2 = {0.0, 0.0, 0.0, 0.0};
    for (int st0 = 0; st0 < nst; st0 += D) {
#pragma unroll
        for (int u = 0; u < D; ++u) {
            const int st = st0 + u;
            if (st < nst) {
                wait_stage(qa[u], qb[u], qk[u]);
                lds_only_barrier();
                store_stage(st, qa[u], qb[u], qk[u]);
                load_stage(min(st + D, nst - 1), qa[u], qb[u], qk[u]);
                lds_only_barrier();
#pragma unroll
                for (int q = 0; q < KS / 4; ++q) {
                    const int k = 4 * q + kk;
                    const double av = TRANSA ? As[(wi + r) * PK + k] : As[k * PR + wi + r];
                    if (q & 1) acc2 = __builtin_amdgcn_mfma_f64_16x16x4f64(Bs[(wj + r) * PK + k], av, acc2, 0, 0, 0);
                    else acc = __builtin_amdgcn_mfma_f64_16x16x4f64(Bs[(wj + r) * PK + k], av, acc, 0, 0, 0);
                }
            }
        }
    }
#pragma unroll
    for (int u = 0; u < D; ++u)
#pragma unroll
        for (int s = 0; s < NL; ++s) asm volatile("s_waitcnt vmcnt(0)" : "+v"(qa[u][s]), "+v"(qb[u][s]), "+v"(qk[u][s]) :: "memory");
    const int i = i0 + wi + r;
    const double rsv = (g.rs.p && i < n) ? g.rs.at(chain)[i] : 1.0;
#pragma unroll
    for (int reg = 0; reg < 4; ++reg) {
        const int jl = wj + kk + 4 * reg, j = j0 + jl;
        double v = (acc[reg] + acc2[reg]) * rsv;
        if (i < n && j < n) {
            if (g.cs.p) v *= g.cs.at(chain)[j];
            double* dst = C + i + (long)n * j;
            if (g.accumulate) v += *dst;
            *dst = v;
        }
        Ct[wi + r][jl] = v;
    }
    if (g.CT.p) {
        __syncthreads();
        double* __restrict__ CT = g.CT.at(chain);
#pragma unroll
        for (int s = 0; s < 4; ++s) {
            const int il = rhi + 8 * s;
            if (i0 + il < n && j0 + rlo < n) CT[(j0 + rlo) + (long)n * (i0 + il)] = Ct[il][rlo];
        }
    }
}

template <int KQ>
static void launch_splitk(const GemmDesc& g, int n_chains, hipStream_t s) {
    const int tiles = (g.n + 15) / 16;
    dim3 grid(tiles * tiles, n_chains), block(256);
    if (g.transA) hipLaunchKernelGGL((gemm_splitk_kernel<true, KQ>), grid, block, 0, s, g, tiles);
    else hipLaunchKernelGGL((gemm_splitk_kernel<false, KQ>), grid, block, 0, s, g, tiles);
}

static int launch_gemm_main(const GemmDesc& g, int n_chains, hipStream_t s, bool* ct_done);

int launch_gemm(const GemmDesc& g, int n_chains, hipStream_t s) {
    bool ct_done = false;
    if (int rc = launch_gemm_main(g, n_chains, s, &ct_done)) return rc;
    if (g.CT.p && !ct_done) return launch_transpose_scale(CMat(g.C.p, g.C.stride), g.CT, CVec(), g.n, n_chains, s);
    return 0;
}

static int launch_gemm_main(const GemmDesc& g, int n_chains, hipStream_t s, bool* ct_done) {
    const int n = g.n;
    if (n % 64 == 0 && (long)n_chains * (n / 64) * (n / 64) >= 256) {
        const int tiles = n / 64;
        dim3 grid(tiles * tiles, n_chains), block(256);
        if (g.transA) hipLaunchKernelGGL((gemm_tile64_kernel<true>), grid, block, 0, s, g, tiles);
        else hipLaunchKernelGGL((gemm_tile64_kernel<false>), grid, block, 0, s, g, tiles);
        DQ_HIP(hipGetLastError());
        return 0;
    }
    if (n >= 384) {
        const int T = (n + 31) / 32, chunk = (T * T + 7) / 8;
        dim3 grid(8 * chunk, n_chains), block(256);
#define DQ_ST(TA, KSC) hipLaunchKernelGGL((gemm_stage32_kernel<TA, KSC, 32>), grid, block, 0, s, g, T, chunk)
        if (g.transA) { if (g.ks.p) DQ_ST(true, true); else DQ_ST(true, false); } else { if (g.ks.p) DQ_ST(false, true); else DQ_ST(false, false); }
#undef DQ_ST
        DQ_HIP(hipGetLastError());
        *ct_done = true;
        return 0;
    }
    if (n <= 640) {
        const int kq = gemm_splitk_kq(n);
        if (kq <= 16) launch_splitk<16>(g, n_chains, s);
        else if (kq <= 32) launch_splitk<32>(g, n_chains, s);
        else if (kq <= 48) launch_splitk<48>(g, n_chains, s);
        else if (kq <= 64) launch_splitk<64>(g, n_chains, s);
        else if (kq <= 96) launch_splitk<96>(g, n_chains, s);
        else if (kq <= 128) launch_splitk<128>(g, n_chains, s);
        else launch_splitk<160>(g, n_chains, s);
        DQ_HIP(hipGetLastError());
        *ct_done = true;
        return 0;
    }
    const int tiles = (n + 31) / 32;
    dim3 grid(tiles * tiles, n_chains), block(256);
    const bool guard = (n % 32) != 0;
    if (g.transA) {
        if (guard) hipLaunchKernelGGL((gemm_kernel<true, true>), grid, block, 0, s, g, tiles);
        else hipLaunchKernelGGL((gemm_kernel<true, false>), grid, block, 0, s, g, tiles);
    } else {
        if (guard) hipLaunchKernelGGL((gemm_kernel<false, true>), grid, block, 0, s, g, tiles);
        else hipLaunchKernelGGL((gemm_kernel<false, false>), grid, block, 0, s, g, tiles);
    }
    DQ_HIP(hipGetLastError());
    return 0;
}

}
```

### dqmc_amd/csrc/gemm_tile.h

```cpp
#pragma once

#include "common.h"

namespace dq {

__host__ __device__ inline int gemm_splitk_kq(int n) { return ((n + 3) / 4 + 15) / 16 * 16; }

template <bool TRANSA, int KQ>
__device__ __forceinline__ void gemm_splitk_tile(const GemmDesc& g, int chain, int i0, int j0, double (*part)[4][64], int kq = KQ) {
    using d4 = __attribute__((ext_vector_type(4))) double;
    const int n = g.n;
    const double* __restrict__ A = g.A.at(chain);
    const double* __restrict__ B = g.B.at(chain);
    double* __restrict__ C = g.C.at(chain);
    const double* __restrict__ ks = g.ks.p ? g.ks.at(chain) : nullptr;
    const int lane = threadIdx.x & 63, wave = threadIdx.x >> 6;
    const int r = lane & 15, kk = lane >> 4;
    const int ia = min(i0 + r, n - 1), jb = min(j0 + r, n - 1);
    const bool ia_ok = i0 + r < n, jb_ok = j0 + r < n;
    const int kbeg = wave * kq;
    constexpr int NB = KQ / 16;
    double av[NB][4], bv[NB][4];
#pragma unroll
    for (int b = 0; b < NB; ++b) {
        if (16 * b >= kq) break;
#pragma unroll
        for (int s = 0; s < 4; ++s) {
            const int k = kbeg + 16 * b + 4 * kk + s;
            const int kc = min(k, n - 1);
            double a = TRANSA ? A[kc + (long)n * ia] : A[ia + (long)n * kc];
            double bb = B[kc + (long)n * jb];
            if (ks) a *= ks[kc];
            const bool ok = k < n;
            av[b][s] = (ok && ia_ok) ? a : 0.0;
            bv[b][s] = (ok && jb_ok) ? bb : 0.0;
        }
    }
    d4 acc = {0.0, 0.0, 0.0, 0.0};
#pragma unroll
    for (int b = 0; b < NB; ++b) {
        if (16 * b >= kq) break;
#pragma unroll
        for (int s = 0; s < 4; ++s) acc = __builtin_amdgcn_mfma_f64_16x16x4f64(bv[b][s], av[b][s], acc, 0, 0, 0);
    }
#pragma unroll
    for (int reg = 0; reg < 4; ++reg) part[wave][reg][lane] = acc[reg];
    __syncthreads();
    const double v4 = part[0][wave][lane] + part[1][wave][lane] + part[2][wave][lane] + part[3][wave][lane];
    const int j = j0 + kk + 4 * wave;
    if (ia_ok && j < n) {
        double v = v4;
        if (g.rs.p) v *= g.rs.at(chain)[i0 + r];
        if (g.cs.p) v *= g.cs.at(chain)[j];
        double* dst = C + (i0 + r) + (long)n * j;
        if (g.accumulate) v += *dst;
        *dst = v;
        if (g.CT.p) g.CT.at(chain)[j + (long)n * (i0 + r)] = v;
    }
}

}
```

### dqmc_amd/csrc/lu_gj.hip

```cpp
#include "common.h"
#include "wave.h"
#include <cstdlib>
#include <type_traits>
#include <utility>

namespace dq {

namespace {
constexpr int GJ_NB = 32;
using d4 = __attribute__((ext_vector_type(4))) double;

__device__ __forceinline__ void lds_wait() { asm volatile("s_waitcnt lgkmcnt(0)" ::: "memory"); }

template <int NR, int J>
__device__ __forceinline__ void gj_step(double (&a)[NR][GJ_NB], bool (&live)[NR], int (&mypos)[NR], int& myperm, bool& singular, int lane, int k0) {
    unsigned long long best = 0ULL; int bq = -1;
#pragma unroll
    for (int q = 0; q < NR; ++q) {
        const unsigned long long kq = live[q] ? ((unsigned long long)__double_as_longlong(fabs(a[q][J])) | 1ULL) : 0ULL;
        if (kq > best) { best = kq; bq = q; }
    }
    const unsigned hi = (unsigned)(best >> 32), lo = (unsigned)best;
    const unsigned m1 = wave_max_u32(hi);
    const unsigned m2 = wave_max_u32(hi == m1 ? lo : 0u);
// ... 174 lines not shown
    GST(0)
    double aj = a[0][J]; int bs = 0;
    if (RPL > 1) asm volatile("" : "+v"(aj));
    unsigned long long key = (live & 1u) ? (VAL ? ((unsigned long long)__double_as_longlong(fabs(aj)) & ~0x1FFULL) | 0x100ULL : ((unsigned long long)__double_as_longlong(fabs(aj)) | 1ULL)) : 0ULL;
    static_assert(!VAL || RPL == 1, "the truncated in-wave search is written for one row per lane");
#pragma unroll
    for (int q = 1; q < RPL; ++q) {
        double v = a[q][J];
        asm volatile("" : "+v"(v));
        const unsigned long long kq = ((live >> q) & 1u) ? ((unsigned long long)__double_as_longlong(fabs(v)) | 1ULL) : 0ULL;
        if (kq > key) { key = kq; aj = v; bs = q; }
    }
    double rme = __builtin_amdgcn_rcp(aj);
    rme = fma(fma(-aj, rme, 1.0), rme, rme);
    rme = fma(fma(-aj, rme, 1.0), rme, rme);
    const unsigned hi = (unsigned)(key >> 32), lo = (unsigned)key;
    const unsigned m1 = wave_max_u32(hi);
    const unsigned m2 = wave_max_u32(hi == m1 ? lo : 0u);
    const unsigned long long winners = __ballot(hi == m1 && lo == m2 && key != 0ULL);
    const int cl = winners ? (int)__builtin_ctzll(winners) : 0;
    GST(1)
    if (lane == cl) {
#pragma unroll
        for (int q = 0; q < RPL; ++q) {
            if (bs == q) {
#pragma unroll
                for (int c = C0; c < GJ_NB; c += 2) *reinterpret_cast<double2*>(&slot_row[PAR][wave][c]) = make_double2(a[q][c], a[q][c + 1]);
            }
        }
        slot_row[PAR][wave][GJ_NB] = rme;
        slot_key[PAR][wave] = winners ? ((((unsigned long long)m1 << 32) | m2) & ~0x1FFULL) | (unsigned long long)(cl | (bs << 6)) | 0x100ULL : 0ULL;
    }
    GST(2)
    asm volatile("s_waitcnt lgkmcnt(0)" ::: "memory");
    __builtin_amdgcn_s_barrier();
    asm volatile("" ::: "memory");
    GST(3)
    constexpr int NWK = (NW + 1) & ~1;
    ulonglong2 kp[NWK / 2];
#pragma unroll
    for (int q = 0; q < NWK / 2; ++q) kp[q] = *reinterpret_cast<const ulonglong2*>(&slot_key[PAR][2 * q]);
    unsigned long long best = kp[0].x; int pw = 0;
    if ((kp[0].y >> 9) > (best >> 9)) { best = kp[0].y; pw = 1; }
#pragma unroll
    for (int q = 1; q < NWK / 2; ++q) {
        if ((kp[q].x >> 9) > (best >> 9)) { best = kp[q].x; pw = 2 * q; }
        if ((kp[q].y >> 9) > (best >> 9)) { best = kp[q].y; pw = 2 * q + 1; }
    }
    const int pl = (int)(best & 0x3FULL), ps = (int)((best >> 6) & 3ULL);
    GST(4)
    double prow[GJ_NB - C0];
#pragma unroll
    for (int c = C0; c < GJ_NB; c += 2) { const double2 v = *reinterpret_cast<const double2*>(&slot_row[PAR][pw][c]); prow[c - C0] = v.x; prow[c + 1 - C0] = v.y; }
    const double r = slot_row[PAR][pw][GJ_NB];
    GST(5)
    if (lane == J && wave == 0) myperm = pl + 64 * pw + 64 * NW * ps;
    const bool mine = wave == pw && lane == pl;
    singular = singular || !(fabs(prow[J - C0]) > 0.0);
#pragma unroll
    for (int q = 0; q < RPL; ++q) {
        if (mine && ps == q) { live &= ~(1u << q); mypos[q] = k0 + J; }
        const bool lv = (live >> q) & 1u;
        const double l = lv ? a[q][J] * r : 0.0;
        a[q][J] = lv ? l : a[q][J];
#pragma unroll
        for (int c = J + 1; c < GJ_NB; ++c) a[q][c] = fma(-l, prow[c - C0], a[q][c]);
    }
    GST(6)
}
template <int J, int NW, int RPL, bool VAL>
struct GjStepsMW {
    static __device__ __forceinline__ void run(double (&a)[RPL][GJ_NB], unsigned& live, int (&mypos)[RPL], int& myperm, bool& singular, int lane, int wave, int nbw, int k0,
                                               double (*slot_row)[NW][GJ_NB + 2], unsigned long long (*slot_key)[(NW + 1) & ~1] GST_ARGS) {
        if (J < nbw) gj_step_mw<J, NW, RPL, VAL>(a, live, mypos, myperm, singular, lane, wave, k0, slot_row, slot_key GST_PASS);
        GjStepsMW<J + 1, NW, RPL, VAL>::run(a, live, mypos, myperm, singular, lane, wave, nbw, k0, slot_row, slot_key GST_PASS);
    }
};
template <int NW, int RPL, bool VAL>
struct GjStepsMW<GJ_NB, NW, RPL, VAL> {
    static __device__ __forceinline__ void run(double (&)[RPL][GJ_NB], unsigned&, int (&)[RPL], int&, bool&, int, int, int, int, double (*)[NW][GJ_NB + 2],
                                               unsigned long long (*)[(NW + 1) & ~1] GST_ARGS) {}
};
constexpr int GJ_CMAX = 128;
struct GjCompactShared {
    double rows[GJ_NB][GJ_CMAX];
    int orow[GJ_CMAX];
    int pos[256];
};
template <int J, int C>
__device__ __forceinline__ void gj_step_cw(double (&a)[C][GJ_NB], unsigned& live, const int (&orow)[C], int (&pos)[C], int& myperm, bool& singular, int lane, int k0) {
    unsigned long long key = 0ULL; int bq = 0;
#pragma unroll
    for (int q = 0; q < C; ++q) {
        const unsigned long long kq = ((live >> q) & 1u) ? ((unsigned long long)__double_as_longlong(fabs(a[q][J])) & ~0x1FFULL) | 0x100ULL : 0ULL;
        if (kq > key) { key = kq; bq = q; }
    }
    const unsigned hi = (unsigned)(key >> 32), lo = (unsigned)key;
    const unsigned m1 = wave_max_u32(hi);
    const unsigned m2 = wave_max_u32(hi == m1 ? lo : 0u);
    const unsigned long long winners = __ballot(hi == m1 && lo == m2 && key != 0ULL);
    const int pl = winners ? (int)__builtin_ctzll(winners) : 0;
    const int pq = C > 1 ? __builtin_amdgcn_readlane(bq, pl) : 0;
    double prow[GJ_NB - J]; int prw = 0;
#pragma unroll
    for (int q = 0; q < C; ++q) {
        if (q == pq) {
#pragma unroll
            for (int c = J; c < GJ_NB; ++c) prow[c - J] = readlane_f64(a[q][c], pl);
            prw = __builtin_amdgcn_readlane(orow[q], pl);
        }
    }
    if (lane == J) myperm = prw;
    const double piv = prow[0];
    singular = singular || !(fabs(piv) > 0.0);
    double r = __builtin_amdgcn_rcp(piv);
    r = fma(fma(-piv, r, 1.0), r, r);
    r = fma(fma(-piv, r, 1.0), r, r);
#pragma unroll
    for (int q = 0; q < C; ++q) {
        if (lane == pl && pq == q) { live &= ~(1u << q); pos[q] = k0 + J; }
        const bool lv = (live >> q) & 1u;
        const double l = lv ? a[q][J] * r : 0.0;
        a[q][J] = lv ? l : a[q][J];
#pragma unroll
        for (int c = J + 1; c < GJ_NB; ++c) a[q][c] = fma(-l, prow[c - J], a[q][c]);
    }
}
template <int J, int C>
struct GjStepsCW {
    static __device__ __forceinline__ void run(double (&a)[C][GJ_NB], unsigned& live, const int (&orow)[C], int (&pos)[C], int& myperm, bool& singular, int lane, int nbw, int k0) {
        if (J < nbw) gj_step_cw<J, C>(a, live, orow, pos, myperm, singular, lane, k0);
        GjStepsCW<J + 1, C>::run(a, live, orow, pos, myperm, singular, lane, nbw, k0);
    }
};
template <int C>
struct GjStepsCW<GJ_NB, C> {
    static __device__ __forceinline__ void run(double (&)[C][GJ_NB], unsigned&, const int (&)[C], int (&)[C], int&, bool&, int, int, int) {}
};
template <int C>
__device__ __forceinline__ void gj_chain_cw(GjCompactShared& cs, double (&LU)[GJ_NB][GJ_NB], int& s_sing, int& myperm, int nl, int lane, int nbw, int k0) {
    double a[C][GJ_NB]; int orow[C], pos[C];
    unsigned live = 0u;
#pragma unroll
    for (int q = 0; q < C; ++q) {
        const int slot = C * lane + q;
        const bool ok = slot < nl;
        const int sc = ok ? slot : 0;
#pragma unroll
        for (int c = 0; c < GJ_NB; ++c) { const double v = cs.rows[c][sc]; a[q][c] = ok ? v : 0.0; }
        orow[q] = ok ? cs.orow[sc] : 0;
        pos[q] = -1;
        live |= ok ? (1u << q) : 0u;
    }
    bool singular = false;
    GjStepsCW<0, C>::run(a, live, orow, pos, myperm, singular, lane, nbw, k0);
#pragma unroll
    for (int q = 0; q < C; ++q) {
        if (pos[q] >= 0) {
            cs.pos[orow[q]] = pos[q];
            double* dst = &LU[pos[q] - k0][0];
#pragma unroll
            for (int c = 0; c < GJ_NB; c += 2) *reinterpret_cast<double2*>(dst + c) = make_double2(a[q][c], a[q][c + 1]);
        }
    }
    if (singular && lane == 0) s_sing = 1;
}

template <int NW, int RPL>
struct GjPanelShared {
    double LU[GJ_NB][GJ_NB];
    double slot_row[2][NW][GJ_NB + 2];
    unsigned long long slot_key[2][(NW + 1) & ~1];
    int s_sing;
};
template <int NW, int RPL, bool CLAMPED>
__device__ __forceinline__ void gj_panel_load(const double* __restrict__ A, const int* rowpos, int n, int k0, int nbw, int t, double (&a)[RPL][GJ_NB], unsigned& live,
                                              int (&oldpos)[RPL]) {
    live = 0u;
#pragma unroll
    for (int q = 0; q < RPL; ++q) {
        const int r = t + 64 * NW * q;
        const int rc = r < n ? r : 0;
        if (CLAMPED) {
            double v[GJ_NB];
#pragma unroll
            for (int c = 0; c < GJ_NB; ++c) v[c] = A[rc + (long)n * (k0 + (c < nbw ? c : 0))];
            oldpos[q] = k0 == 0 ? -1 : rowpos[rc];
            const bool lv = r < n && oldpos[q] < 0;
            live |= lv ? (1u << q) : 0u;
#pragma unroll
            for (int c = 0; c < GJ_NB; ++c) a[q][c] = (lv && c < nbw) ? v[c] : 0.0;
        } else {
            oldpos[q] = k0 == 0 ? -1 : rowpos[rc];
            const bool lv = r < n && oldpos[q] < 0;
            live |= lv ? (1u << q) : 0u;
#pragma unroll
            for (int c = 0; c < GJ_NB; ++c) a[q][c] = (lv && c < nbw) ? A[r + (long)n * (k0 + c)] : 0.0;
        }
    }
}
template <int NW, int RPL, bool CMP>
__device__ __forceinline__ void gj_panel_factor(GjPanelShared<NW, RPL>& sh, double (&a)[RPL][GJ_NB], unsigned& live, int (&mypos)[RPL], int& myperm, int t, int nbw, int k0,
                                                GjCompactShared* cs, int nl, int rank
#ifdef DQ_GJ_STAMPS
                                                , unsigned long long& gstart, unsigned long long& gsteps_end
#endif
                                                ) {
    constexpr int NWK = (NW + 1) & ~1;
    static_assert(RPL <= 4, "two key bits name the slot");
    static_assert(!CMP || (NW == 4 && RPL == 1), "the compacted chain is written for one row per lane in at most four waves");
    const int lane = t & 63, wave = t >> 6;
    bool singular = false;
    myperm = 0;
#pragma unroll
    for (int q = 0; q < RPL; ++q) mypos[q] = -1;
    for (int e = t; e < GJ_NB * GJ_NB; e += blockDim.x) (&sh.LU[0][0])[e] = ((e >> 5) == (e & 31)) ? 1.0 : 0.0;
    if (t == 0) sh.s_sing = 0;
    if (t < 2 * NWK) (&sh.slot_key[0][0])[t] = 0ULL;
    if constexpr (CMP) {
        if (cs != nullptr && nl <= GJ_CMAX) {
            cs->pos[t] = -1;
            if ((live & 1u) && rank < GJ_CMAX) {
#pragma unroll
                for (int c = 0; c < GJ_NB; ++c) cs->rows[c][rank] = a[0][c];
                cs->orow[rank] = t;
            }
            lds_wait();
            __builtin_amdgcn_s_barrier();
            asm volatile("" ::: "memory");
#ifdef DQ_GJ_STAMPS
            asm volatile("s_memtime %0\n\ts_waitcnt lgkmcnt(0)" : "=s"(gstart) :: "memory");
#endif
            if (wave == 0) {
                if (nl <= 64) gj_chain_cw<1>(*cs, sh.LU, sh.s_sing, myperm, nl, lane, nbw, k0);
                else gj_chain_cw<2>(*cs, sh.LU, sh.s_sing, myperm, nl, lane, nbw, k0);
            }
#ifdef DQ_GJ_STAMPS
            asm volatile("s_waitcnt lgkmcnt(0)\n\ts_memtime %0\n\ts_waitcnt lgkmcnt(0)" : "=s"(gsteps_end) :: "memory");
            if (t == 0 && k0 == DQ_GJ_STAMP_K0 && blockIdx.x == 0 && blockIdx.y == 0)
                printf("gj panel k0=%d grid.x=%d, compacted: %d live rows on one wave, clocks over %d steps incl. the read-back and the deposit: %llu\n", k0, (int)gridDim.x, nl, nbw, gsteps_end - gstart);
#endif
            lds_wait();
            __builtin_amdgcn_s_barrier();
            asm volatile("" ::: "memory");
            mypos[0] = cs->pos[t];
            return;
        }
    }
    lds_wait();
    __builtin_amdgcn_s_barrier();
    asm volatile("" ::: "memory");

#ifdef DQ_GJ_STAMPS
    unsigned long long gst[8] = {0, 0, 0, 0, 0, 0, 0, 0}, gprev;
    asm volatile("s_waitcnt vmcnt(0)\n\ts_memtime %0\n\ts_waitcnt lgkmcnt(0)" : "=s"(gprev) :: "memory"); gstart = gprev;
#endif
    GjStepsMW<0, NW, RPL, CMP>::run(a, live, mypos, myperm, singular, lane, wave, nbw, k0, sh.slot_row, sh.slot_key GST_PASS);
#ifdef DQ_GJ_STAMPS
    gsteps_end = gprev;
    if (t == 0 && k0 == DQ_GJ_STAMP_K0 && blockIdx.x == 0 && blockIdx.y == 0)
        printf("gj panel k0=%d grid.x=%d, %d waves x %d rows per lane, clocks over %d steps (each segment includes one stamp, ~130): (loop) %llu | search %llu | publish %llu | barrier %llu | keys %llu | row %llu | fma %llu | total %llu\n",
               k0, (int)gridDim.x, (int)(blockDim.x >> 6), RPL, nbw, gst[0], gst[1], gst[2], gst[3], gst[4], gst[5], gst[6], gprev - gstart);
#endif

    lds_wait();
    __builtin_amdgcn_s_barrier();
    asm volatile("" ::: "memory");
#pragma unroll
    for (int q = 0; q < RPL; ++q) {
        if (mypos[q] >= 0) {
            double* dst = &sh.LU[mypos[q] - k0][0];
#pragma unroll
            for (int c = 0; c < GJ_NB; c += 2) *reinterpret_cast<double2*>(dst + c) = make_double2(a[q][c], a[q][c + 1]);
        }
    }
    if (singular && lane == 0) sh.s_sing = 1;
}
__device__ __forceinline__ int gj_compact_rank(const int* rowpos, int n, int t, bool compact, int& nl) {
    int rank = 0;
    nl = GJ_CMAX + 1;
    if (compact) {
        int tot = 0;
        const int lane = t & 63, wave = t >> 6;
        int pw[4];
#pragma unroll
        for (int w = 0; w < 4; ++w) { const int r = lane + 64 * w; pw[w] = rowpos[r < n ? r : n - 1]; }
#pragma unroll
        for (int w = 0; w < 4; ++w) {
            const unsigned long long b = __ballot(lane + 64 * w < n && pw[w] < 0);
            rank += w < wave ? __popcll(b) : (w == wave ? __popcll(b & ((1ULL << lane) - 1ULL)) : 0);
            tot += __popcll(b);
        }
        nl = tot < GJ_CMAX ? tot : GJ_CMAX;
    }
    return rank;
}
#ifdef DQ_GJ_STAMPS
#define GJ_STAMP_VM(x) asm volatile("s_waitcnt vmcnt(0)\n\ts_memtime %0\n\ts_waitcnt lgkmcnt(0)" : "=s"(x) :: "memory")
#endif

template <int NW, int RPL>
__global__ __launch_bounds__(64 * NW) void gj_panel_mw_kernel(CMat Am, int* rowpos_p, long rowpos_stride, int* perm_p, long perm_stride, double* tinv_p,
                                                          double* logabsdet, int accumulate, int* info, int n, int k0, int compact) {
    __shared__ __attribute__((aligned(16))) GjPanelShared<NW, RPL> sh;
    const int chain = blockIdx.y;
    const double* __restrict__ A = Am.at(chain);
    int* rowpos = rowpos_p + (long)chain * rowpos_stride;
    int* perm = perm_p + (long)chain * perm_stride;
    double* tinv = tinv_p + (long)chain * 2 * GJ_NB * GJ_NB;
    const int t = threadIdx.x, lane = t & 63, wave = t >> 6;
#ifdef DQ_GJ_STAMPS
    unsigned long long gentry, gstart, gprev;
    asm volatile("s_memtime %0\n\ts_waitcnt lgkmcnt(0)" : "=s"(gentry) :: "memory");
#endif
    const int nbw = min(GJ_NB, n - k0);
    unsigned live;
    int oldpos[RPL], mypos[RPL], myperm;
    double a[RPL][GJ_NB];
    gj_panel_load<NW, RPL, false>(A, rowpos, n, k0, nbw, t, a, live, oldpos);
    constexpr bool CMP = NW == 4 && RPL == 1;
    __shared__ __attribute__((aligned(16))) std::conditional_t<CMP, GjCompactShared, int> s_cs;
    GjCompactShared* cs = nullptr;
    if constexpr (CMP) { if (compact) cs = &s_cs; }
    int nl = GJ_CMAX + 1;
    const int rank = CMP ? gj_compact_rank(rowpos, n, t, cs != nullptr && k0 > 0 && n - k0 <= GJ_CMAX, nl) : 0;
#ifdef DQ_GJ_STAMPS
    gj_panel_factor<NW, RPL, CMP>(sh, a, live, mypos, myperm, t, nbw, k0, cs, nl, rank, gstart, gprev);
#else
    gj_panel_factor<NW, RPL, CMP>(sh, a, live, mypos, myperm, t, nbw, k0, cs, nl, rank);
#endif
#pragma unroll
    for (int q = 0; q < RPL; ++q) {
        const int r = t + 64 * NW * q;
        if (r < n) { if (k0 == 0) rowpos[r] = mypos[q]; else if (mypos[q] >= 0) rowpos[r] = mypos[q]; }
    }
    if (wave == 0 && lane < nbw) perm[k0 + lane] = myperm;
    __syncthreads();
    for (int e = t; e < GJ_NB * GJ_NB; e += blockDim.x) tinv[e] = (&sh.LU[0][0])[e];
#ifdef DQ_GJ_STAMPS
    unsigned long long gmid;
    GJ_STAMP_VM(gmid);
#endif
    if (wave == 0) gj_panel_tri_inverses(sh.LU, tinv + GJ_NB * GJ_NB, lane);
    else if (wave == 1) gj_panel_logdet(sh.LU, logabsdet, accumulate, info, chain, lane, nbw, k0, sh.s_sing);
#ifdef DQ_GJ_STAMPS
    unsigned long long gend;
    GJ_STAMP_VM(gend);
    if (t == 0 && k0 == DQ_GJ_STAMP_K0 && blockIdx.y == 0) printf("   prologue %llu | steps %llu | LU hand-over (+ printf) %llu | epilogue %llu\n", gstart - gentry, gprev - gstart, gmid - gprev, gend - gmid);
#endif
}

__global__ __launch_bounds__(256) void gj_update_kernel(Mat Am, Mat Bm, Mat SAm, Mat Xm, const int* rowpos_p, long rowpos_stride,
                                                        const int* perm_p, long perm_stride, const double* tinv_p, int n, int k0, int nA, int nS, int nCA) {
    const int chain = blockIdx.y;
    double* __restrict__ A = Am.at(chain);
    double* __restrict__ B = Bm.at(chain);
    double* __restrict__ SA = SAm.at(chain);
    double* __restrict__ X = Xm.at(chain);
    const int* rowpos = rowpos_p + (long)chain * rowpos_stride;
    const int* perm = perm_p + (long)chain * perm_stride;
    const double* __restrict__ LUg = tinv_p + (long)chain * 2 * GJ_NB * GJ_NB;
    const double* __restrict__ Tinv = LUg + GJ_NB * GJ_NB;
    const int nbw = min(GJ_NB, n - k0);
    const int row_tiles = nA + nS + 1;
    const int rt = blockIdx.x % row_tiles, ct = blockIdx.x / row_tiles;
    const int lane = threadIdx.x & 63, wave = threadIdx.x >> 6;
    const int r16 = lane & 15, kk = lane >> 4;
    const int wr = wave & 1, wc = wave >> 1;
    const bool colA = ct < nCA;
    const int col = (colA ? k0 + nbw + 32 * ct : 32 * (ct - nCA)) + 16 * wc + r16;
    const bool col_ok = col < n;
    const long coff = (long)n * (col_ok ? col : n - 1);
    const double* __restrict__ src12 = colA ? A : B;
    double* __restrict__ dstS = colA ? SA : X;

    double a12[2][4];
#pragma unroll
    for (int h = 0; h < 2; ++h)
#pragma unroll
        for (int s = 0; s < 4; ++s) {
            const int k = 16 * h + 4 * s + kk;
            const int pr = perm[k0 + (k < nbw ? k : 0)];
            const double v = src12[pr + coff];
            a12[h][s] = (k < nbw && col_ok) ? v : 0.0;
        }
    const bool writer = rt == nA + nS;
    const bool rowS = rt >= nA;
    const int row0 = (rowS ? 32 * (rt - nA) : 32 * rt) + 16 * wr;
    const int rowlim = rowS ? k0 : n;
    const double* __restrict__ msrc = rowS ? SA : A;
    double* __restrict__ dst = rowS ? dstS : (colA ? A : B);
    double mult[2][4];
    double cold[4];
    bool st_ok[4];
    if (!writer) {
        const int mrow = min(row0 + r16, rowlim - 1);
#pragma unroll
        for (int h = 0; h < 2; ++h)
#pragma unroll
            for (int s = 0; s < 4; ++s) {
                const int k = 16 * h + kk + 4 * s;
                const double v = msrc[mrow + (long)n * (k0 + (k < nbw ? k : 0))];
                mult[h][s] = k < nbw ? v : 0.0;
            }
#pragma unroll
        for (int reg = 0; reg < 4; ++reg) {
            const int r = row0 + kk + 4 * reg;
            const int rc = min(r, rowlim - 1);
            st_ok[reg] = col_ok && r < rowlim && (rowS || rowpos[rc] < 0);
            cold[reg] = dst[rc + coff];
        }
    }
    double lai[4], lbi[4], uai[4], ubi[4], cl[4], cu[4];
#pragma unroll
    for (int s = 0; s < 4; ++s) {
        const int k = 4 * s + kk;
        lai[s] = Tinv[0 * 256 + r16 + 16 * k]; lbi[s] = Tinv[1 * 256 + r16 + 16 * k];
        uai[s] = Tinv[2 * 256 + r16 + 16 * k]; ubi[s] = Tinv[3 * 256 + r16 + 16 * k];
        cl[s] = -LUg[(16 + r16) * 32 + k];
        cu[s] = -LUg[r16 * 32 + 16 + k];
    }
    const d4 zero4 = {0.0, 0.0, 0.0, 0.0};
    d4 t1[2], u[2];
    t1[0] = zero4;
#pragma unroll
    for (int s = 0; s < 4; ++s) t1[0] = __builtin_amdgcn_mfma_f64_16x16x4f64(lai[s], a12[0][s], t1[0], 0, 0, 0);
    d4 w = {a12[1][0], a12[1][1], a12[1][2], a12[1][3]};
#pragma unroll
    for (int s = 0; s < 4; ++s) w = __builtin_amdgcn_mfma_f64_16x16x4f64(cl[s], t1[0][s], w, 0, 0, 0);
    t1[1] = zero4;
#pragma unroll
    for (int s = 0; s < 4; ++s) t1[1] = __builtin_amdgcn_mfma_f64_16x16x4f64(lbi[s], w[s], t1[1], 0, 0, 0);
    u[1] = zero4;
#pragma unroll
    for (int s = 0; s < 4; ++s) u[1] = __builtin_amdgcn_mfma_f64_16x16x4f64(ubi[s], t1[1][s], u[1], 0, 0, 0);
    w = t1[0];
#pragma unroll
    for (int s = 0; s < 4; ++s) w = __builtin_amdgcn_mfma_f64_16x16x4f64(cu[s], u[1][s], w, 0, 0, 0);
    u[0] = zero4;
#pragma unroll
    for (int s = 0; s < 4; ++s) u[0] = __builtin_amdgcn_mfma_f64_16x16x4f64(uai[s], w[s], u[0], 0, 0, 0);
    if (writer) {
#pragma unroll
        for (int reg = 0; reg < 4; ++reg) {
            const int i = 16 * wr + kk + 4 * reg;
            if (i < nbw && col_ok) dstS[k0 + i + coff] = u[wr][reg];
        }
        return;
    }
    d4 acc = {0.0, 0.0, 0.0, 0.0};
#pragma unroll
    for (int h = 0; h < 2; ++h)
#pragma unroll
        for (int s = 0; s < 4; ++s) acc = __builtin_amdgcn_mfma_f64_16x16x4f64(mult[h][s], u[h][s], acc, 0, 0, 0);
#pragma unroll
    for (int reg = 0; reg < 4; ++reg)
        if (st_ok[reg]) dst[row0 + kk + 4 * reg + coff] = cold[reg] - acc[reg];
}

template <int NW, int RPL>
__global__ __launch_bounds__(64 * NW) void gj_step_kernel(Mat Am, Mat Bm, Mat SAm, Mat Xm, const int* rowpos_old_p, int* rowpos_new_p, long rowpos_stride,
                                                          double* logabsdet, int accumulate, int* info, int n, int k0, int nA, int nS, int nCA, int compact) {
    static_assert(NW == 4, "the update's 2 x 2 waves are the panel's");
    __shared__ __attribute__((aligned(16))) GjPanelShared<NW, RPL> sh;
    __shared__ __attribute__((aligned(16))) double s_inv[4 * 256];
    __shared__ int s_rowpos[64 * NW * RPL];
    __shared__ int s_perm[GJ_NB];
    const int chain = blockIdx.y;
    double* __restrict__ A = Am.at(chain);
    double* __restrict__ B = Bm.at(chain);
    double* __restrict__ SA = SAm.at(chain);
    double* __restrict__ X = Xm.at(chain);
    const int* rowpos_old = rowpos_old_p + (long)chain * rowpos_stride;
    int* rowpos_new = rowpos_new_p + (long)chain * rowpos_stride;
    const int t = threadIdx.x, lane = t & 63, wave = t >> 6;
#ifdef DQ_GJ_STAMPS
    unsigned long long gentry, gstart, gprev;
    asm volatile("s_memtime %0\n\ts_waitcnt lgkmcnt(0)" : "=s"(gentry) :: "memory");
#endif
    const int nbw = min(GJ_NB, n - k0);

    unsigned live;
    int oldpos[RPL], mypos[RPL], myperm;
    double a[RPL][GJ_NB];
    gj_panel_load<NW, RPL, true>(A, rowpos_old, n, k0, nbw, t, a, live, oldpos);
    constexpr bool CMP = NW == 4 && RPL == 1;
    __shared__ __attribute__((aligned(16))) std::conditional_t<CMP, GjCompactShared, int> s_cs;
    GjCompactShared* cs = nullptr;
    if constexpr (CMP) { if (compact) cs = &s_cs; }
    int nl = GJ_CMAX + 1;
    const int rank = CMP ? gj_compact_rank(rowpos_old, n, t, cs != nullptr && k0 > 0 && n - k0 <= GJ_CMAX, nl) : 0;

    const int row_tiles = nA + nS + 1;
    const int rt = blockIdx.x % row_tiles, ct = blockIdx.x / row_tiles;
    const int r16 = lane & 15, kk = lane >> 4;
    const int wr = wave & 1, wc = wave >> 1;
    const bool colA = ct < nCA;
    const int col = (colA ? k0 + nbw + 32 * ct : 32 * (ct - nCA)) + 16 * wc + r16;
    const bool col_ok = col < n;
    const long coff = (long)n * (col_ok ? col : n - 1);
    const double* __restrict__ src12 = colA ? A : B;
    double* __restrict__ dstS = colA ? SA : X;
    const bool writer = rt == nA + nS;
    const bool rowS = rt >= nA;
    const int row0 = (rowS ? 32 * (rt - nA) : 32 * rt) + 16 * wr;
    const int rowlim = rowS ? k0 : n;
    const double* __restrict__ msrc = rowS ? SA : A;
    double* __restrict__ dst = rowS ? dstS : (colA ? A : B);
    double mult[2][4];
    double cold[4];
    {
        const int mrow = max(min(row0 + r16, rowlim - 1), 0);
#pragma unroll
        for (int h = 0; h < 2; ++h)
#pragma unroll
            for (int s = 0; s < 4; ++s) {
                const int k = 16 * h + kk + 4 * s;
                const double v = msrc[mrow + (long)n * (k0 + (k < nbw ? k : 0))];
                mult[h][s] = k < nbw ? v : 0.0;
            }
#pragma unroll
        for (int reg = 0; reg < 4; ++reg) cold[reg] = dst[max(min(row0 + kk + 4 * reg, rowlim - 1), 0) + coff];
    }

#ifdef DQ_GJ_STAMPS
    gj_panel_factor<NW, RPL, CMP>(sh, a, live, mypos, myperm, t, nbw, k0, cs, nl, rank, gstart, gprev);
#else
    gj_panel_factor<NW, RPL, CMP>(sh, a, live, mypos, myperm, t, nbw, k0, cs, nl, rank);
#endif
#pragma unroll
    for (int q = 0; q < RPL; ++q) {
        const int r = t + 64 * NW * q;
        const int np = mypos[q] >= 0 ? mypos[q] : oldpos[q];
        s_rowpos[r] = np;
        if (blockIdx.x == 0 && r < n) rowpos_new[r] = np;
    }
    if (wave == 0 && lane < GJ_NB) s_perm[lane] = lane < nbw ? myperm : 0;
    __syncthreads();
#ifdef DQ_GJ_STAMPS
    unsigned long long gmid, ginv, ggather;
    GJ_STAMP_VM(gmid);
#endif

    double a12[2][4];
#pragma unroll
    for (int h = 0; h < 2; ++h)
#pragma unroll
        for (int s = 0; s < 4; ++s) {
            const int k = 16 * h + 4 * s + kk;
            const double v = src12[s_perm[k < nbw ? k : 0] + coff];
            a12[h][s] = (k < nbw && col_ok) ? v : 0.0;
        }
    bool st_ok[4];
#pragma unroll
    for (int reg = 0; reg < 4; ++reg) {
        const int r = row0 + kk + 4 * reg;
        st_ok[reg] = !writer && col_ok && r < rowlim && (rowS || s_rowpos[max(min(r, rowlim - 1), 0)] < 0);
    }
    if (wave == 0) gj_panel_tri_inverses(sh.LU, s_inv, lane);
    else if (wave == 1 && blockIdx.x == 0) gj_panel_logdet(sh.LU, logabsdet, accumulate, info, chain, lane, nbw, k0, sh.s_sing);
#ifdef DQ_GJ_STAMPS
    asm volatile("s_waitcnt lgkmcnt(0)\n\ts_memtime %0\n\ts_waitcnt lgkmcnt(0)" : "=s"(ginv) :: "memory");
#endif
    __syncthreads();
#ifdef DQ_GJ_STAMPS
    GJ_STAMP_VM(ggather);
#endif

    const double* LUs = &sh.LU[0][0];
    double lai[4], lbi[4], uai[4], ubi[4], cl[4], cu[4];
#pragma unroll
    for (int s = 0; s < 4; ++s) {
        const int k = 4 * s + kk;
        lai[s] = s_inv[0 * 256 + r16 + 16 * k]; lbi[s] = s_inv[1 * 256 + r16 + 16 * k];
        uai[s] = s_inv[2 * 256 + r16 + 16 * k]; ubi[s] = s_inv[3 * 256 + r16 + 16 * k];
        cl[s] = -LUs[(16 + r16) * 32 + k];
        cu[s] = -LUs[r16 * 32 + 16 + k];
    }
    const d4 zero4 = {0.0, 0.0, 0.0, 0.0};
    d4 t1[2], u[2];
    t1[0] = zero4;
#pragma unroll
    for (int s = 0; s < 4; ++s) t1[0] = __builtin_amdgcn_mfma_f64_16x16x4f64(lai[s], a12[0][s], t1[0], 0, 0, 0);
    d4 w = {a12[1][0], a12[1][1], a12[1][2], a12[1][3]};
#pragma unroll
    for (int s = 0; s < 4; ++s) w = __builtin_amdgcn_mfma_f64_16x16x4f64(cl[s], t1[0][s], w, 0, 0, 0);
    t1[1] = zero4;
#pragma unroll
    for (int s = 0; s < 4; ++s) t1[1] = __builtin_amdgcn_mfma_f64_16x16x4f64(lbi[s], w[s], t1[1], 0, 0, 0);
    u[1] = zero4;
#pragma unroll
    for (int s = 0; s < 4; ++s) u[1] = __builtin_amdgcn_mfma_f64_16x16x4f64(ubi[s], t1[1][s], u[1], 0, 0, 0);
    w = t1[0];
#pragma unroll
    for (int s = 0; s < 4; ++s) w = __builtin_amdgcn_mfma_f64_16x16x4f64(cu[s], u[1][s], w, 0, 0, 0);
    u[0] = zero4;
#pragma unroll
    for (int s = 0; s < 4; ++s) u[0] = __builtin_amdgcn_mfma_f64_16x16x4f64(uai[s], w[s], u[0], 0, 0, 0);
    if (writer) {
#pragma unroll
        for (int reg = 0; reg < 4; ++reg) {
            const int i = 16 * wr + kk + 4 * reg;
            if (i < nbw && col_ok) dstS[k0 + i + coff] = u[wr][reg];
        }
    } else {
        d4 acc = {0.0, 0.0, 0.0, 0.0};
#pragma unroll
        for (int h = 0; h < 2; ++h)
#pragma unroll
            for (int s = 0; s < 4; ++s) acc = __builtin_amdgcn_mfma_f64_16x16x4f64(mult[h][s], u[h][s], acc, 0, 0, 0);
#pragma unroll
        for (int reg = 0; reg < 4; ++reg)
            if (st_ok[reg]) dst[row0 + kk + 4 * reg + coff] = cold[reg] - acc[reg];
    }
#ifdef DQ_GJ_STAMPS
    unsigned long long gend;
    GJ_STAMP_VM(gend);
    if (t == 0 && k0 == DQ_GJ_STAMP_K0 && blockIdx.x == 0 && blockIdx.y == 0)
        printf("   fused step: prologue %llu | chain %llu | deposit (+ printf) %llu | inverses (wave 0) %llu | gather wait %llu | update %llu\n", gstart - gentry, gprev - gstart,
               gmid - gprev, ginv - gmid, ggather - ginv, gend - ggather);
#endif
}
bool gj_fused_fits(int n) { return n > 64 && n <= 256; }
bool gj_fused_default(int n) { return n > 128 && n <= 256; }

int launch_gj_solve(Mat A, Mat B, Mat X, Mat SA, double* tinv, int* perm, long perm_stride, int* rowpos, int* rowpos_alt, long rowpos_stride,
                    double* logabsdet, int accumulate_logdet, int* info, int n, int n_chains, bool fused, bool compact, hipStream_t s) {
    if (n > 1024) { set_error("gj_solve supports n <= 1024"); return -1; }
    if (fused && rowpos_alt && gj_fused_fits(n)) {
        int p = 0;
        for (int k0 = 0; k0 < n; k0 += GJ_NB, ++p) {
            const int nbw = n - k0 < GJ_NB ? n - k0 : GJ_NB;
            const int nA = (n + 31) / 32, nS = k0 / 32;
            const int nCA = (n - k0 - nbw + 31) / 32, nCB = (n + 31) / 32;
            hipLaunchKernelGGL((gj_step_kernel<4, 1>), dim3((nA + nS + 1) * (nCA + nCB), n_chains), dim3(256), 0, s, A, B, SA, X, (const int*)((p & 1) ? rowpos_alt : rowpos),
                               (p & 1) ? rowpos : rowpos_alt, rowpos_stride, logabsdet, accumulate_logdet, info, n, k0, nA, nS, nCA, compact ? 1 : 0);
        }
        DQ_HIP(hipGetLastError());
        return 0;
    }
    for (int k0 = 0; k0 < n; k0 += GJ_NB) {
        const dim3 pg(1, n_chains);
#define DQ_GJ_PANEL(NW, RPL) hipLaunchKernelGGL((gj_panel_mw_kernel<NW, RPL>), pg, dim3(RPL == 1 ? 64 * ((n + 63) / 64) : 64 * NW), 0, s, CMat(A), rowpos, rowpos_stride, perm, perm_stride, tinv, logabsdet, accumulate_logdet, info, n, k0, compact ? 1 : 0)
        if (n > 768) DQ_GJ_PANEL(8, 2);
        else if (n > 576) DQ_GJ_PANEL(4, 3);
        else if (n > 512) DQ_GJ_PANEL(3, 3);
        else if (n > 256) DQ_GJ_PANEL(4, 2);
        else if (n > 64) DQ_GJ_PANEL(4, 1);
        else hipLaunchKernelGGL((gj_panel_kernel<1>), pg, dim3(64), 0, s, CMat(A), rowpos, rowpos_stride, perm, perm_stride, tinv, logabsdet, accumulate_logdet, info, n, k0);
        const int nbw = n - k0 < GJ_NB ? n - k0 : GJ_NB;
        const int nA = (n + 31) / 32, nS = k0 / 32;
        const int nCA = (n - k0 - nbw + 31) / 32, nCB = (n + 31) / 32;
        hipLaunchKernelGGL(gj_update_kernel, dim3((nA + nS + 1) * (nCA + nCB), n_chains), dim3(256), 0, s, A, B, SA, X, (const int*)rowpos, rowpos_stride,
                           (const int*)perm, perm_stride, (const double*)tinv, n, k0, nA, nS, nCA);
    }
#undef DQ_GJ_PANEL
    DQ_HIP(hipGetLastError());
    return 0;
}

}
```

### dqmc_amd/csrc/qr.hip

```cpp
#include "common.h"
#include "wave.h"
#include <cstdlib>

namespace dq {


template <int NR>
__global__ __launch_bounds__(1024) void qrcp_kernel(Mat Am, QrWork w, int n) {
    extern __shared__ __attribute__((aligned(16))) unsigned char smem[];
    double* vn1 = reinterpret_cast<double*>(smem);
    double* vn2 = vn1 + n;
    double* v = vn2 + n;
    double* candcol = v + n;
    double* cand_v = candcol + 16 * (size_t)n;
    double* red = cand_v + 16;
    int* cand_i = reinterpret_cast<int*>(red + 16);
    int* pivpos = cand_i + 16;
    const int chain = blockIdx.y;
    double* __restrict__ A = Am.at(chain);
    double* tau = w.tau + (long)chain * w.tau_stride;
    int* jpvt = w.jpvt + (long)chain * w.jpvt_stride;
    const int t = threadIdx.x, lane = t & 63, wave = t >> 6;
    const double tol3z = 1.0536712127723509e-08;
    constexpr int QR_CB = NR <= 2 ? 8 : (NR <= 4 ? 4 : (NR <= 9 ? 2 : 1));
// ... 180 lines not shown
                                                 int n, int rg, int ii) {
        const int ic = ii > 0 ? ii : 0;
        const long cb = (long)n * s_jpvt[ic]; t = s_tau[ic];
#pragma unroll
        for (int j = J0; j < NRR; ++j) v[j] = A[16 * j + rg + cb];
    }
    static __device__ __forceinline__ void apply(double (&q)[NRR], const double (&v)[NRR], double ti, int c, int i, int rg) {
        if (ti == 0.0) return;
        const int rm = 16 * M + rg;
        const double vm = (rm > i) ? v[M] : (rm == i ? 1.0 : 0.0);
        double s0 = vm * q[M], s1 = 0.0;
#pragma unroll
        for (int j = M + 1; j < NRR; ++j) { if ((j - M) & 1) s1 = fma(v[j], q[j], s1); else s0 = fma(v[j], q[j], s0); }
        double s = row16_sum(s0 + s1) * ti;
        if (c < i) s = 0.0;
        q[M] = fma(-s, vm, q[M]);
#pragma unroll
        for (int j = M + 1; j < NRR; ++j) q[j] = fma(-s, v[j], q[j]);
    }
    static __device__ __forceinline__ void run(double (&q)[NRR], double (&vq)[4][NRR], double (&tq)[4], const double* __restrict__ A, const int* s_jpvt,
                                               const double* s_tau, int n, int rg, int c, int cw_max) {
        const int mtop = cw_max >> 4;
        if (M <= mtop) {
            const int hi = M == mtop ? cw_max : 16 * M + 15;
            if (M == mtop) {
#pragma unroll
                for (int e = 0; e < 4; ++e) fetch(vq[e], tq[e], A, s_jpvt, s_tau, n, rg, hi - e);
            }
            for (int top = hi; top >= 16 * M; top -= 4) {
#pragma unroll
                for (int e = 0; e < 4; ++e) {
                    apply(q, vq[e], tq[e], c, top - e, rg);
                    fetch(vq[e], tq[e], A, s_jpvt, s_tau, n, rg, top - e - 4);
                }
            }
        }
        FormQBlock<NRR, M - 1>::run(q, vq, tq, A, s_jpvt, s_tau, n, rg, c, cw_max);
    }
};
template <int NRR>
struct FormQBlock<NRR, -1> {
    static __device__ __forceinline__ void run(double (&)[NRR], double (&)[4][NRR], double (&)[4], const double*, const int*, const double*, int, int, int, int) {}
};
template <int NRR>
__global__ __launch_bounds__(256) void formq_blocked_kernel(CMat Am, const double* tau_p, long tau_stride, const int* jpvt_p, long jpvt_stride, Mat Qm, int n) {
    const int chain = blockIdx.y;
    const double* __restrict__ A = Am.at(chain);
    const double* __restrict__ tau = tau_p + (long)chain * tau_stride;
    const int* __restrict__ jpvt = jpvt_p + (long)chain * jpvt_stride;
    double* __restrict__ Q = Qm.at(chain);
    const int lane = threadIdx.x & 63, wave = threadIdx.x >> 6;
    const int rg = lane & 15, cq = lane >> 4;
    const int c = blockIdx.x * 16 + wave * 4 + cq;
    const int cw_max = blockIdx.x * 16 + wave * 4 + 3;
    __shared__ int s_jpvt[16 * NRR];
    __shared__ double s_tau[16 * NRR];
    for (int k = threadIdx.x; k < n; k += blockDim.x) { s_jpvt[k] = jpvt[k]; s_tau[k] = tau[k]; }
    __syncthreads();
    double q[NRR];
#pragma unroll
    for (int j = 0; j < NRR; ++j) q[j] = (16 * j + rg == c) ? 1.0 : 0.0;
    double vq[4][NRR]; double tq[4];
#pragma unroll
    for (int e = 0; e < 4; ++e) {
        tq[e] = 0.0;
#pragma unroll
        for (int j = 0; j < NRR; ++j) vq[e][j] = 0.0;
    }
    FormQBlock<NRR, NRR - 1>::run(q, vq, tq, A, s_jpvt, s_tau, n, rg, c, cw_max);
#pragma unroll
    for (int j = 0; j < NRR; ++j) { const int r = 16 * j + rg; if (r < n) Q[r + (long)n * c] = q[j]; }
}

static bool formq_blocked_ok(int n) {
    return (n == 16 || n == 32 || n == 64 || n == 128 || n == 256 || n == 576);
}
static void launch_formq_blocked(CMat A, const QrWork& w, Mat L, int n, int n_chains, hipStream_t s) {
    const dim3 grid(n / 16, n_chains), block(256);
#define DQ_FQ(NRR) hipLaunchKernelGGL((formq_blocked_kernel<NRR>), grid, block, 0, s, A, (const double*)w.tau, w.tau_stride, (const int*)w.jpvt, w.jpvt_stride, L, n)
    if (n <= 16) DQ_FQ(1); else if (n <= 32) DQ_FQ(2); else if (n <= 64) DQ_FQ(4); else if (n <= 128) DQ_FQ(8); else if (n <= 256) DQ_FQ(16); else DQ_FQ(36);
#undef DQ_FQ
}

__global__ void assemble_r_kernel(CMat Am, const int* jpvt_p, long jpvt_stride, Vec dv, Mat Rm, int n) {
    const int chain = blockIdx.y;
    const double* __restrict__ A = Am.at(chain);
    const int* jpvt = jpvt_p + (long)chain * jpvt_stride;
    double* __restrict__ R = Rm.at(chain);
    double* d = dv.at(chain);
    const int j = blockIdx.x;
    const int col = jpvt[j];
    for (int r = threadIdx.x; r < n; r += blockDim.x) {
        double val = 0.0;
        if (r <= j) val = A[r + (long)n * col] / fabs(A[r + (long)n * jpvt[r]]);
        R[r + (long)n * col] = val;
    }
    if (threadIdx.x == 0) d[j] = fabs(A[j + (long)n * col]);
}

int qr_init_device() {
    DQ_HIP(hipFuncSetAttribute(reinterpret_cast<const void*>(qrcp_kernel<1>), hipFuncAttributeMaxDynamicSharedMemorySize, 160 * 1024));
    DQ_HIP(hipFuncSetAttribute(reinterpret_cast<const void*>(qrcp_kernel<2>), hipFuncAttributeMaxDynamicSharedMemorySize, 160 * 1024));
    DQ_HIP(hipFuncSetAttribute(reinterpret_cast<const void*>(qrcp_kernel<4>), hipFuncAttributeMaxDynamicSharedMemorySize, 160 * 1024));
    DQ_HIP(hipFuncSetAttribute(reinterpret_cast<const void*>(qrcp_kernel<9>), hipFuncAttributeMaxDynamicSharedMemorySize, 160 * 1024));
    DQ_HIP(hipFuncSetAttribute(reinterpret_cast<const void*>(qrcp_kernel<16>), hipFuncAttributeMaxDynamicSharedMemorySize, 160 * 1024));
    return 0;
}

int launch_qrcp_coop(Mat A, QrWork w, int n, int n_chains, hipStream_t s);
int launch_qrcp_colown(Mat A, QrWork w, int n, int n_chains, hipStream_t s);

static int launch_assemble_r(Mat A, Vec d, Mat R, const QrWork& w, int n, int n_chains, hipStream_t s) {
    hipLaunchKernelGGL(assemble_r_kernel, dim3(n, n_chains), dim3(128), 0, s, CMat(A), (const int*)w.jpvt, w.jpvt_stride, d, R, n);
    DQ_HIP(hipGetLastError());
    return 0;
}
static int formq_assemble(Mat A, Mat L, Vec d, Mat R, const QrWork& w, int n, int n_chains, hipStream_t s) {
    if (formq_blocked_ok(n)) launch_formq_blocked(CMat(A), w, L, n, n_chains, s);
    else if (n <= 256) hipLaunchKernelGGL((formq_kernel<16>), dim3((n + 15) / 16, n_chains), dim3(256), 0, s, CMat(A), (const double*)w.tau, w.tau_stride,
                                          (const int*)w.jpvt, w.jpvt_stride, L, n);
    else if (n <= 576) hipLaunchKernelGGL((formq_kernel<36>), dim3((n + 15) / 16, n_chains), dim3(256), 0, s, CMat(A), (const double*)w.tau, w.tau_stride,
                                          (const int*)w.jpvt, w.jpvt_stride, L, n);
    else hipLaunchKernelGGL((formq_kernel<64>), dim3((n + 15) / 16, n_chains), dim3(256), 0, s, CMat(A), (const double*)w.tau, w.tau_stride,
                            (const int*)w.jpvt, w.jpvt_stride, L, n);
    return launch_assemble_r(A, d, R, w, n, n_chains, s);
}
static int to_ldr_panel(Mat A, Mat L, Vec d, Mat R, const QrWork& w, int n, int n_chains, hipStream_t s) {
    DQ_TRY(launch_qr_panel(A, L, w, n, n_chains, s));
    return launch_assemble_r(A, d, R, w, n, n_chains, s);
}
template <int NR>
static int to_ldr_streaming(Mat A, Mat L, Vec d, Mat R, const QrWork& w, int n, int n_chains, hipStream_t s) {
    const size_t lds = sizeof(double) * ((size_t)3 * n + (size_t)16 * n + 32) + sizeof(int) * (16 + (size_t)n) + 64;
    hipLaunchKernelGGL((qrcp_kernel<NR>), dim3(1, n_chains), dim3(1024), lds, s, A, w, n);
    hipLaunchKernelGGL((formq_kernel<4 * NR>), dim3((n + 15) / 16, n_chains), dim3(256), 0, s, CMat(A), (const double*)w.tau, w.tau_stride,
                       (const int*)w.jpvt, w.jpvt_stride, L, n);
    return launch_assemble_r(A, d, R, w, n, n_chains, s);
}

int launch_to_ldr(QrFamily f, Mat A, Mat L, Vec d, Mat R, QrWork w, int n, int n_chains, hipStream_t s) {
    if (n > 1024) { set_error("to_LDR kernel supports n <= 1024"); return -1; }
    switch (f) {
    case QrFamily::Panel: return to_ldr_panel(A, L, d, R, w, n, n_chains, s);
    case QrFamily::ColumnOwner:
        if (n > 256) break;
        DQ_TRY(launch_qrcp_colown(A, w, n, n_chains, s));
        return formq_assemble(A, L, d, R, w, n, n_chains, s);
    case QrFamily::Cooperative:
        DQ_TRY(launch_qrcp_coop(A, w, n, n_chains, s));
        return formq_assemble(A, L, d, R, w, n, n_chains, s);
    case QrFamily::Streaming:
        if (n <= 64) return to_ldr_streaming<1>(A, L, d, R, w, n, n_chains, s);
        if (n <= 128) return to_ldr_streaming<2>(A, L, d, R, w, n, n_chains, s);
        if (n <= 256) return to_ldr_streaming<4>(A, L, d, R, w, n, n_chains, s);
        if (n <= 576) return to_ldr_streaming<9>(A, L, d, R, w, n, n_chains, s);
        return to_ldr_streaming<16>(A, L, d, R, w, n, n_chains, s);
    }
    set_error("to_LDR: kernel family not available at this n");
    return -1;
}

}
```

Before: 13.77 sweeps/s.

## Fold stabilization split, transpose-scale and error check into QR and GEMM riders

The D-split (dl/ds) is now computed inside the QR assemble_r kernel and cached per LDR stack entry, so split_d launches can be skipped on later use. The two GEMMs and the transpose-scale in inv_I_plus_ldr_mul_ldr are merged into one GEMM launch with rider descriptors. The max-abs-diff stability check is folded into the final GEMM through sharded atomic maxima that fold_stats reduces. The aim is fewer small kernel launches per stabilization step, at the cost of a more complex GEMM kernel and extra bookkeeping for cache validity. The GJ compaction flag also moves from a runtime argument to a template parameter.

```diff
diff --git a/dqmc_amd/csrc/common.h b/dqmc_amd/csrc/common.h
--- a/dqmc_amd/csrc/common.h
+++ b/dqmc_amd/csrc/common.h
@@ -60,6 +60,7 @@
 using Vec = Mat;
 using CVec = CMat;
 
+constexpr int GEMM_ERR_SHARDS = 16;
 struct GemmDesc {
     CMat A, B;
     Mat C;
@@ -68,6 +69,10 @@
     int n = 0;
     int transA = 0;
     int accumulate = 0;
+    CMat A2, B2; CVec rs2, ks2, cs2; int transA2 = 0;
+    CMat TS; Mat TSout{nullptr, 0};
+    CMat ref; unsigned long long* err = nullptr; long err_stride = 0;
+    bool has_riders() const { return A2.p || TS.p || ref.p; }
 };
 int launch_gemm(const GemmDesc& g, int n_chains, hipStream_t s);
 
@@ -86,7 +91,7 @@
 int launch_add_scaled_cols(CMat A, CMat B, CVec cs, Mat C, int n, int n_chains, hipStream_t s);
 int launch_scale_rows(CMat in, CVec rs, Mat out, int n, int n_chains, hipStream_t s);
 struct DevStats { double acc_rate, max_err, sum_err, n_err; long long n_accepted, n_proposed; };
-int launch_fold_stats(DevStats* st, const int* acc, long acc_stride, int n_slices, const double* err, long err_stride, int n_err,
+int launch_fold_stats(DevStats* st, const int* acc, long acc_stride, int n_slices, double* err, const unsigned long long* shards, long err_stride, int n_err,
                       int n, int nt, int n_chains, hipStream_t s);
 
 struct QrWork {
@@ -98,6 +103,7 @@
     double* pw = nullptr; long pw_stride = 0;
     bool pw_two_launch = false;
     int* pivpos = nullptr; long pivpos_stride = 0;
+    double* dl = nullptr; double* ds = nullptr; long split_stride = 0;
     bool pw_compact = true;
 };
 bool qr_panel_fused_fits(int n);
diff --git a/dqmc_amd/csrc/elementwise.hip b/dqmc_amd/csrc/elementwise.hip
--- a/dqmc_amd/csrc/elementwise.hip
+++ b/dqmc_amd/csrc/elementwise.hip
@@ -176,7 +176,7 @@
     return 0;
 }
 
-__global__ void fold_stats_kernel(DevStats* st, const int* acc, long acc_stride, int n_slices, const double* err, long err_stride,
+__global__ void fold_stats_kernel(DevStats* st, const int* acc, long acc_stride, int n_slices, double* err, const unsigned long long* shards, long err_stride,
                                   int n_err, int n, int nt, int n_chains) {
     const int c = blockIdx.x * blockDim.x + threadIdx.x;
     if (c >= n_chains) return;
@@ -187,15 +187,22 @@
         s.n_accepted += a; s.n_proposed += n;
     }
     for (int k = 0; k < n_err; ++k) {
-        const double e = err[(long)c * err_stride + k];
+        double e = err[(long)c * err_stride + k];
+        if (shards) {
+            unsigned long long m = (unsigned long long)__double_as_longlong(e);
+            const unsigned long long* sh = shards + ((long)c * err_stride + k) * GEMM_ERR_SHARDS;
+            for (int q = 0; q < GEMM_ERR_SHARDS; ++q) m = sh[q] > m ? sh[q] : m;
+            e = __longlong_as_double((long long)m);
+            err[(long)c * err_stride + k] = e;
+        }
         if (e > s.max_err || e != e) s.max_err = e;
         s.sum_err += e; s.n_err += 1.0;
     }
     st[c] = s;
 }
-int launch_fold_stats(DevStats* st, const int* acc, long acc_stride, int n_slices, const double* err, long err_stride, int n_err,
+int launch_fold_stats(DevStats* st, const int* acc, long acc_stride, int n_slices, double* err, const unsigned long long* shards, long err_stride, int n_err,
                       int n, int nt, int n_chains, hipStream_t s) {
-    hipLaunchKernelGGL(fold_stats_kernel, dim3((n_chains + 63) / 64), dim3(64), 0, s, st, acc, acc_stride, n_slices, err, err_stride, n_err, n, nt, n_chains);
+    hipLaunchKernelGGL(fold_stats_kernel, dim3((n_chains + 63) / 64), dim3(64), 0, s, st, acc, acc_stride, n_slices, err, shards, err_stride, n_err, n, nt, n_chains);
     DQ_HIP(hipGetLastError());
     return 0;
 }
diff --git a/dqmc_amd/csrc/engine.hip b/dqmc_amd/csrc/engine.hip
--- a/dqmc_amd/csrc/engine.hip
+++ b/dqmc_amd/csrc/engine.hip
@@ -26,7 +26,7 @@
     return 0;
 }
 
-struct Switches { bool qr_panel; int qr_panel_fused, gj_fused; bool qr_streaming, walk_submatrix, lu_classic, slice_multikernel, bbar_rider, slice_stream, panel_compact; };
+struct Switches { bool qr_panel; int qr_panel_fused, gj_fused; bool qr_streaming, walk_submatrix, lu_classic, slice_multikernel, bbar_rider, slice_stream, panel_compact, stab_fold; };
 static const Switches& switches() {
     static const Switches sw = [] {
         const char* panel = getenv("DQMC_QR_PANEL");
@@ -35,8 +35,9 @@
         const char* rider = getenv("DQMC_BBAR_RIDER");
         const char* stream = getenv("DQMC_SLICE_STREAM");
         const char* compact = getenv("DQMC_PANEL_COMPACT");
+        const char* fold = getenv("DQMC_STAB_FOLD");
         return Switches{!(panel && atoi(panel) == 0), fused ? (atoi(fused) != 0 ? 1 : 0) : -1, gj ? (atoi(gj) != 0 ? 1 : 0) : -1, getenv("DQMC_QR_STREAMING") != nullptr, getenv("DQMC_WALK_SUBMATRIX") != nullptr,
-                        getenv("DQMC_LU_CLASSIC") != nullptr, getenv("DQMC_SLICE_MULTIKERNEL") != nullptr, !(rider && atoi(rider) == 0), !(stream && atoi(stream) == 0), !(compact && atoi(compact) == 0)};
+                        getenv("DQMC_LU_CLASSIC") != nullptr, getenv("DQMC_SLICE_MULTIKERNEL") != nullptr, !(rider && atoi(rider) == 0), !(stream && atoi(stream) == 0), !(compact && atoi(compact) == 0), !(fold && atoi(fold) == 0)};
     }();
     return sw;
 }
@@ -80,20 +81,24 @@
     bool* tri = nullptr;
     Mat X{nullptr, 0};
     bool* xok = nullptr;
-    void touch() const { if (xok) *xok = false; }
+    Vec dl{nullptr, 0}, ds{nullptr, 0};
+    bool* sok = nullptr;
+    void touch() const { if (xok) *xok = false; if (sok) *sok = false; }
+    void touch_r() const { if (xok) *xok = false; }
 };
 struct LdrStore {
-    int n = 0, C = 0;
-    DevPtr<double> L, d, R, X;
+    int n = 0, C = 0, kcount = 0;
+    DevPtr<double> L, d, R, X, split;
     DevPtr<int> jpvt;
-    std::unique_ptr<bool[]> tri, xok;
+    std::unique_ptr<bool[]> tri, xok, sok;
     int alloc(int k, int n_, int C_, bool with_x = false) {
         n = n_; C = C_;
         const size_t nn = (size_t)n * n;
         DQ_TRY(dev_alloc(L, (size_t)k * C * nn)); DQ_TRY(dev_alloc(d, (size_t)k * C * n));
         DQ_TRY(dev_alloc(R, (size_t)k * C * nn)); DQ_TRY(dev_alloc(jpvt, (size_t)k * C * n));
         if (with_x) DQ_TRY(dev_alloc(X, (size_t)k * C * nn));
-        tri.reset(new bool[k]()); xok.reset(new bool[k]());
+        DQ_TRY(dev_alloc(split, (size_t)2 * k * C * n)); kcount = k;
+        tri.reset(new bool[k]()); xok.reset(new bool[k]()); sok.reset(new bool[k]());
         return 0;
     }
     LdrRef at(int i) const {
@@ -101,6 +106,7 @@
         LdrRef f{Mat{L.get() + (long)i * C * nn, nn}, Vec{d.get() + (long)i * C * n, (long)n}, Mat{R.get() + (long)i * C * nn, nn},
                  jpvt.get() + (long)i * C * n, &tri[i]};
         if (X) { f.X = Mat{X.get() + (long)i * C * nn, nn}; f.xok = &xok[i]; }
+        f.dl = Vec{split.get() + (long)i * C * n, (long)n}; f.ds = Vec{split.get() + ((long)kcount + i) * C * n, (long)n}; f.sok = &sok[i];
         return f;
     }
 };
@@ -169,9 +175,19 @@
         w.sync = qsync.get(); w.sync_stride = qrcp_coop_sync_granules(n); w.abort_words = qabort.get(); w.info = info();
         w.pw = qpw.get(); w.pw_stride = qr_panel_work_doubles(n, qpw_two_launch); w.pw_two_launch = qpw_two_launch; w.pivpos = qpivpos.get(); w.pivpos_stride = n;
         w.pw_compact = switches().panel_compact;
+        const bool split = switches().stab_fold && out.sok != nullptr;
+        if (split) { w.dl = out.dl.p; w.ds = out.ds.p; w.split_stride = out.dl.stride; }
         if (out.tri) *out.tri = keep;
         out.touch();
-        return launch_to_ldr(plan.qr, A, out.L, out.d, out.R, w, n, C, stream);
+        DQ_TRY(launch_to_ldr(plan.qr, A, out.L, out.d, out.R, w, n, C, stream));
+        if (split) *out.sok = true;
+        return 0;
+    }
+    bool split_cached(LdrRef F, Vec& dl, Vec& ds) const { if (!(F.sok && *F.sok)) return false; dl = F.dl; ds = F.ds; return true; }
+    int split_d(LdrRef F, int v, Vec& dl, Vec& ds) {
+        if (split_cached(F, dl, ds)) return 0;
+        dl = V(v); ds = V(v + 1);
+        return launch_split_d(F.d, dl, ds, nullptr, n, C, stream);
     }
     int r_inverse_scaled(LdrRef F, CVec dinv, Mat scratch, Mat lu_scratch, Mat* Xout) {
         const Mat X = F.X.p ? F.X : scratch;
@@ -191,15 +207,17 @@
     int mat_mul_ldr(CMat M, LdrRef F, LdrRef out) {
         DQ_TRY(gemm(M, F.L, T(0), CVec(), CVec(), CVec(F.d)));
         LdrRef q{out.L, out.d, T(1)};
+        q.dl = out.dl; q.ds = out.ds; q.sok = out.sok;
         DQ_TRY(to_ldr(T(0), q));
         if (out.tri) *out.tri = false;
-        out.touch();
+        out.touch_r();
         return gemm(T(1), F.R, out.R);
     }
     int ldr_mul_mat(LdrRef F, CMat M, LdrRef out) {
         DQ_TRY(gemm(F.R, M, T(0), CVec(F.d)));
         LdrRef q{T(1), out.d, out.R, out.jpvt, out.tri};
         q.xok = out.xok;
+        q.dl = out.dl; q.ds = out.ds; q.sok = out.sok;
         DQ_TRY(to_ldr(T(0), q));
         return gemm(F.L, T(1), out.L);
     }
@@ -230,22 +248,39 @@
         Mat Y; DQ_TRY(solve(T(3), T(4), T(0), logdet, &Y));
         return launch_transpose_scale(Y, G, CVec(), n, C, stream);
     }
-    int inv_I_plus_ldr_mul_ldr(LdrRef F1, LdrRef F2, Mat G, Mat GT = Mat{nullptr, 0}) {
-        DQ_TRY(launch_split_d2(F1.d, V(0), V(1), F2.d, V(2), V(3), n, C, stream));
-        Mat X; DQ_TRY(r_inverse_scaled(F2, V(2), T(1), T(0), &X));
-        DQ_TRY(gemm(F1.L, X, T(2), V(0), CVec(), CVec(), 1));
-        DQ_TRY(gemm(F1.R, F2.L, T(2), V(1), CVec(), V(3), 0, 1));
-        DQ_TRY(launch_transpose_scale(F1.L, T(3), V(0), n, C, stream));
+    int inv_I_plus_ldr_mul_ldr(LdrRef F1, LdrRef F2, Mat G, Mat GT = Mat{nullptr, 0}, CMat ref = CMat(), double* err = nullptr, unsigned long long* err_shards = nullptr,
+                               long err_stride = 0) {
+        const bool fold = switches().stab_fold;
+        Vec v0, v1, v2, v3;
+        const bool c1 = split_cached(F1, v0, v1), c2 = split_cached(F2, v2, v3);
+        if (!c1 && !c2) { v0 = V(0); v1 = V(1); v2 = V(2); v3 = V(3); DQ_TRY(launch_split_d2(F1.d, v0, v1, F2.d, v2, v3, n, C, stream)); }
+        else { DQ_TRY(split_d(F1, 0, v0, v1)); DQ_TRY(split_d(F2, 2, v2, v3)); }
+        Mat X; DQ_TRY(r_inverse_scaled(F2, v2, T(1), T(0), &X));
+        if (fold) {
+            GemmDesc g; g.A = F1.L; g.B = X; g.C = T(2); g.rs = v0; g.transA = 1; g.n = n;
+            g.A2 = F1.R; g.B2 = F2.L; g.rs2 = v1; g.cs2 = v3;
+            g.TS = F1.L; g.TSout = T(3);
+            DQ_TRY(launch_gemm(g, C, stream));
+        } else {
+            DQ_TRY(gemm(F1.L, X, T(2), v0, CVec(), CVec(), 1));
+            DQ_TRY(gemm(F1.R, F2.L, T(2), v1, CVec(), v3, 0, 1));
+            DQ_TRY(launch_transpose_scale(F1.L, T(3), v0, n, C, stream));
+        }
         Mat Y; DQ_TRY(solve(T(2), T(3), T(0), nullptr, &Y));
-        return gemm(X, Y, G, CVec(), CVec(), CVec(), 0, 0, GT);
+        GemmDesc g; g.A = X; g.B = Y; g.C = G; g.CT = GT; g.n = n;
+        if (fold && ref.p) { g.ref = ref; g.err = err_shards; g.err_stride = err_stride * GEMM_ERR_SHARDS; }
+        DQ_TRY(launch_gemm(g, C, stream));
+        if (!fold && ref.p) DQ_TRY(launch_max_abs_diff(ref, G, err, err_stride, n, C, stream));
+        return 0;
     }
     int inv_invldr_plus_ldr(LdrRef F1, LdrRef F2, Mat G, bool negate) {
-        DQ_TRY(launch_split_d(F1.d, V(0), V(1), nullptr, n, C, stream));
-        DQ_TRY(launch_split_d(F2.d, V(2), V(3), nullptr, n, C, stream));
-        Mat X; DQ_TRY(r_inverse_scaled(F2, V(2), T(1), T(0), &X));
-        DQ_TRY(gemm(F1.L, X, T(2), V(0), CVec(), CVec(), 1));
-        DQ_TRY(gemm(F1.R, F2.L, T(2), V(1), CVec(), V(3), 0, 1));
-        DQ_TRY(launch_scale_rows(F1.R, V(1), T(3), n, C, stream));
+        Vec v0, v1, v2, v3;
+        DQ_TRY(split_d(F1, 0, v0, v1));
+        DQ_TRY(split_d(F2, 2, v2, v3));
+        Mat X; DQ_TRY(r_inverse_scaled(F2, v2, T(1), T(0), &X));
+        DQ_TRY(gemm(F1.L, X, T(2), v0, CVec(), CVec(), 1));
+        DQ_TRY(gemm(F1.R, F2.L, T(2), v1, CVec(), v3, 0, 1));
+        DQ_TRY(launch_scale_rows(F1.R, v1, T(3), n, C, stream));
         Mat Y; DQ_TRY(solve(T(2), T(3), T(0), nullptr, &Y));
         DQ_TRY(gemm(X, Y, G));
         if (negate) DQ_TRY(launch_axpb_identity(G, G, -1.0, 0.0, n, C, stream));
@@ -327,6 +362,7 @@
     DevPtr<int> acc;
     struct Exchange { DevPtr<int8_t> saved, recv; DevPtr<int> tab; } xch;
     DevPtr<double> err;
+    unsigned long long* err_shards() const { return reinterpret_cast<unsigned long long*>(err.get() + (long)C * n_stack); }
     DevPtr<DevStats> dstats;
     bool stack_valid = false;
     bool profiling = false;
@@ -369,7 +405,7 @@
         DQ_TRY(dev_alloc(rs_perm, (size_t)C * nt * n)); DQ_TRY(dev_alloc(rs_k, (size_t)C * nt * n)); DQ_TRY(dev_alloc(rs_u, (size_t)C * nt * n));
         panel_rows = slice_path == SlicePath::PersistentWalk ? SLICE_RING_ROWS : UPDATE_KD;
         DQ_TRY(dev_alloc(Upanel, (size_t)C * panel_rows * n)); DQ_TRY(dev_alloc(Wpanel, (size_t)C * panel_rows * n)); DQ_TRY(dev_alloc(Cpanel, (size_t)C * UPDATE_KD * UPDATE_KD));
-        DQ_TRY(dev_alloc(state, (size_t)C * 4)); DQ_TRY(dev_alloc(prep, (size_t)C * 4 * n)); DQ_TRY(dev_alloc(meas_now, (size_t)C * (3 + n))); DQ_TRY(dev_alloc(meas_sum, (size_t)C * (3 + n))); DQ_HIP(hipMemsetAsync(meas_sum.get(), 0, sizeof(double) * C * (3 + n), s)); DQ_TRY(dev_alloc(slice_sync, (size_t)C * SLICE_SYNC_BYTES)); DQ_HIP(hipMemsetAsync(slice_sync.get(), 0, (size_t)C * SLICE_SYNC_BYTES, s)); DQ_TRY(dev_alloc(acc, (size_t)C * nt)); DQ_TRY(dev_alloc(err, (size_t)C * n_stack));
+        DQ_TRY(dev_alloc(state, (size_t)C * 4)); DQ_TRY(dev_alloc(prep, (size_t)C * 4 * n)); DQ_TRY(dev_alloc(meas_now, (size_t)C * (3 + n))); DQ_TRY(dev_alloc(meas_sum, (size_t)C * (3 + n))); DQ_HIP(hipMemsetAsync(meas_sum.get(), 0, sizeof(double) * C * (3 + n), s)); DQ_TRY(dev_alloc(slice_sync, (size_t)C * SLICE_SYNC_BYTES)); DQ_HIP(hipMemsetAsync(slice_sync.get(), 0, (size_t)C * SLICE_SYNC_BYTES, s)); DQ_TRY(dev_alloc(acc, (size_t)C * nt)); DQ_TRY(dev_alloc(err, (size_t)C * n_stack * (1 + GEMM_ERR_SHARDS)));
         DQ_TRY(dev_alloc(dstats, C));
         void* stage = nullptr;
         DQ_HIP(hipHostMalloc(&stage, (size_t)C * nt * n * (sizeof(int32_t) + sizeof(uint8_t) + sizeof(double)), hipHostMallocDefault)); h_stage.reset(static_cast<char*>(stage));
@@ -613,7 +649,7 @@
     }
     int sweep_fwd() {
         int n_err = 0;
-        DQ_HIP(hipMemsetAsync(err.get(), 0, sizeof(double) * C * n_stack, s));
+        DQ_HIP(hipMemsetAsync(err.get(), 0, sizeof(double) * C * n_stack * (switches().stab_fold ? 1 + GEMM_ERR_SHARDS : 1), s));
         const bool pg = piggyback(), ride = bbar_rides();
         double* Pcur = bb0.get(); double* Pnxt = bb1.get();
         for (int l = 0; l < nt; ++l) {
@@ -635,17 +671,19 @@
                 if (is == 0) DQ_TRY(ctx.to_ldr(bb, stack.at(0)));
                 else DQ_TRY(ctx.mat_mul_ldr(bb, stack.at(is - 1), stack.at(is)));
                 gt_valid = false;
-                if (l == nt - 1) DQ_TRY(ctx.inv_I_plus_ldr(stack.at(is), mG(), logdet.get()));
-                else DQ_TRY(ctx.inv_I_plus_ldr_mul_ldr(stack.at(is), stack.at(is + 1), mG()));
-                DQ_TRY(launch_max_abs_diff(CMat(Gtmp.get(), nn), mG(), err.get() + n_err, n_stack, n, C, s));
+                if (l == nt - 1) {
+                    DQ_TRY(ctx.inv_I_plus_ldr(stack.at(is), mG(), logdet.get()));
+                    DQ_TRY(launch_max_abs_diff(CMat(Gtmp.get(), nn), mG(), err.get() + n_err, n_stack, n, C, s));
+                } else DQ_TRY(ctx.inv_I_plus_ldr_mul_ldr(stack.at(is), stack.at(is + 1), mG(), Mat{nullptr, 0}, CMat(Gtmp.get(), nn), err.get() + n_err,
+                                                         err_shards() + (long)n_err * GEMM_ERR_SHARDS, n_stack));
                 ++n_err;
             }
         }
-        return launch_fold_stats(dstats.get(), acc.get(), nt, nt, err.get(), n_stack, n_err, n, nt, C, s);
+        return launch_fold_stats(dstats.get(), acc.get(), nt, nt, err.get(), switches().stab_fold ? err_shards() : nullptr, n_stack, n_err, n, nt, C, s);
     }
     int sweep_bwd() {
         int n_err = 0;
-        DQ_HIP(hipMemsetAsync(err.get(), 0, sizeof(double) * C * n_stack, s));
+        DQ_HIP(hipMemsetAsync(err.get(), 0, sizeof(double) * C * n_stack * (switches().stab_fold ? 1 + GEMM_ERR_SHARDS : 1), s));
         const bool pg = piggyback(), ride = bbar_rides();
         double* Pcur = bb0.get(); double* Pnxt = bb1.get();
         SliceRider pending; bool have_pending = false;
@@ -665,9 +703,12 @@
                 if (is == n_stack - 1) DQ_TRY(ctx.to_ldr(bb, stack.at(is)));
                 else DQ_TRY(ctx.ldr_mul_mat(stack.at(is + 1), bb, stack.at(is)));
                 gt_valid = false;
-                if (l == 0) DQ_TRY(ctx.inv_I_plus_ldr(stack.at(is), mG(), logdet.get()));
-                else {
-                    DQ_TRY(ctx.inv_I_plus_ldr_mul_ldr(stack.at(is - 1), stack.at(is), mG(), use_gt() ? Mat{GT.get(), nn} : Mat{nullptr, 0}));
+                if (l == 0) {
+                    DQ_TRY(ctx.inv_I_plus_ldr(stack.at(is), mG(), logdet.get()));
+                    DQ_TRY(launch_max_abs_diff(CMat(Gtmp.get(), nn), mG(), err.get() + n_err, n_stack, n, C, s));
+                } else {
+                    DQ_TRY(ctx.inv_I_plus_ldr_mul_ldr(stack.at(is - 1), stack.at(is), mG(), use_gt() ? Mat{GT.get(), nn} : Mat{nullptr, 0}, CMat(Gtmp.get(), nn),
+                                                      err.get() + n_err, err_shards() + (long)n_err * GEMM_ERR_SHARDS, n_stack));
                     gt_valid = use_gt();
                     if (gt_check && gt_valid) {
                         DQ_TRY(launch_transpose_scale(mG(), ctx.T(0), CVec(), n, C, s));
@@ -675,11 +716,10 @@
                         ++gt_checks;
                     }
                 }
-                DQ_TRY(launch_max_abs_diff(CMat(Gtmp.get(), nn), mG(), err.get() + n_err, n_stack, n, C, s));
                 ++n_err;
             }
         }
-        return launch_fold_stats(dstats.get(), acc.get(), nt, nt, err.get(), n_stack, n_err, n, nt, C, s);
+        return launch_fold_stats(dstats.get(), acc.get(), nt, nt, err.get(), switches().stab_fold ? err_shards() : nullptr, n_stack, n_err, n, nt, C, s);
     }
     Mat utm(int which, int l) const { return Mat{ut.G[which].get() + (long)l * C * nn, nn}; }
     int sweep_unequal() {
@@ -727,7 +767,7 @@
             }
         }
         ut_valid = true;
-        return launch_fold_stats(dstats.get(), acc.get(), nt, 0, ut.err.get(), 3L * n_stack, n_err, n, nt, C, s);
+        return launch_fold_stats(dstats.get(), acc.get(), nt, 0, ut.err.get(), nullptr, 3L * n_stack, n_err, n, nt, C, s);
     }
     int sync_and_check() {
         DQ_HIP(hipStreamSynchronize(s));
@@ -790,6 +830,7 @@
 static int upload_ldr(Stateless* x, int k, const double* L, const double* d, const double* R, LdrRef* out) {
     const Ctx& c = x->ctx;
     *out = x->ldr.at(k); *out->tri = false;
+    out->touch();
     DQ_HIP(hipMemcpyAsync(out->L.p, L, sizeof(double) * c.nn, hipMemcpyHostToDevice, c.stream));
     DQ_HIP(hipMemcpyAsync(out->R.p, R, sizeof(double) * c.nn, hipMemcpyHostToDevice, c.stream));
     DQ_HIP(hipMemcpyAsync(out->d.p, d, sizeof(double) * c.n, hipMemcpyHostToDevice, c.stream));
@@ -1049,7 +1090,7 @@
         DQ_HIP(hipMemcpy(e.rs_u.get() + off, u + (size_t)c * e.n, sizeof(double) * e.n, hipMemcpyHostToDevice));
     }
     DQ_TRY(e.local_update(l));
-    DQ_TRY(launch_fold_stats(e.dstats.get(), e.acc.get() + l, e.nt, 1, e.err.get(), e.n_stack, 0, e.n, e.nt, e.C, e.s));
+    DQ_TRY(launch_fold_stats(e.dstats.get(), e.acc.get() + l, e.nt, 1, e.err.get(), nullptr, e.n_stack, 0, e.n, e.nt, e.C, e.s));
     DQ_TRY(e.sync_and_check());
     if (accepted) for (int c = 0; c < e.C; ++c) DQ_HIP(hipMemcpy(accepted + c, e.acc.get() + (size_t)c * e.nt + l, sizeof(int), hipMemcpyDeviceToHost));
     return 0;
diff --git a/dqmc_amd/csrc/gemm.hip b/dqmc_amd/csrc/gemm.hip
--- a/dqmc_amd/csrc/gemm.hip
+++ b/dqmc_amd/csrc/gemm.hip
@@ -63,10 +63,10 @@
     }
 }
 
-template <bool TRANSA, int KQ >
+template <bool TRANSA, int KQ , bool RIDERS = false>
 __global__ __launch_bounds__(256) void gemm_splitk_kernel(GemmDesc g, int tiles_per_dim) {
-    __shared__ double part[4][4][64];
-    gemm_splitk_tile<TRANSA, KQ>(g, blockIdx.y, (blockIdx.x % tiles_per_dim) * 16, (blockIdx.x / tiles_per_dim) * 16, part);
+    __shared__ double part[RIDERS ? 8 : 4][4][64];
+    gemm_splitk_tile<TRANSA, KQ, RIDERS>(g, blockIdx.y, (blockIdx.x % tiles_per_dim) * 16, (blockIdx.x / tiles_per_dim) * 16, part);
 }
 
 template <bool TRANSA>
@@ -287,13 +287,28 @@
 static void launch_splitk(const GemmDesc& g, int n_chains, hipStream_t s) {
     const int tiles = (g.n + 15) / 16;
     dim3 grid(tiles * tiles, n_chains), block(256);
-    if (g.transA) hipLaunchKernelGGL((gemm_splitk_kernel<true, KQ>), grid, block, 0, s, g, tiles);
+    if (g.has_riders()) {
+        if (g.transA) hipLaunchKernelGGL((gemm_splitk_kernel<true, KQ, true>), grid, block, 0, s, g, tiles);
+        else hipLaunchKernelGGL((gemm_splitk_kernel<false, KQ, true>), grid, block, 0, s, g, tiles);
+    } else if (g.transA) hipLaunchKernelGGL((gemm_splitk_kernel<true, KQ>), grid, block, 0, s, g, tiles);
     else hipLaunchKernelGGL((gemm_splitk_kernel<false, KQ>), grid, block, 0, s, g, tiles);
 }
+static bool gemm_takes_splitk(int n, int n_chains) { return !(n % 64 == 0 && (long)n_chains * (n / 64) * (n / 64) >= 256) && n < 384; }
 
 static int launch_gemm_main(const GemmDesc& g, int n_chains, hipStream_t s, bool* ct_done);
 
 int launch_gemm(const GemmDesc& g, int n_chains, hipStream_t s) {
+    if (g.has_riders() && !gemm_takes_splitk(g.n, n_chains)) {
+        GemmDesc p = g; p.A2 = p.B2 = p.TS = p.ref = CMat(); p.CT = g.A2.p ? Mat{nullptr, 0} : g.CT;
+        DQ_TRY(launch_gemm(p, n_chains, s));
+        if (g.A2.p) {
+            GemmDesc q; q.A = g.A2; q.B = g.B2; q.C = g.C; q.CT = g.CT; q.rs = g.rs2; q.ks = g.ks2; q.cs = g.cs2; q.n = g.n; q.transA = g.transA2; q.accumulate = 1;
+            DQ_TRY(launch_gemm(q, n_chains, s));
+        }
+        if (g.TS.p) DQ_TRY(launch_transpose_scale(g.TS, g.TSout, g.rs, g.n, n_chains, s));
+        if (g.ref.p) DQ_TRY(launch_max_abs_diff(g.ref, CMat(g.C.p, g.C.stride), reinterpret_cast<double*>(g.err), g.err_stride, g.n, n_chains, s));
+        return 0;
+    }
     bool ct_done = false;
     if (int rc = launch_gemm_main(g, n_chains, s, &ct_done)) return rc;
     if (g.CT.p && !ct_done) return launch_transpose_scale(CMat(g.C.p, g.C.stride), g.CT, CVec(), g.n, n_chains, s);
diff --git a/dqmc_amd/csrc/gemm_tile.h b/dqmc_amd/csrc/gemm_tile.h
--- a/dqmc_amd/csrc/gemm_tile.h
+++ b/dqmc_amd/csrc/gemm_tile.h
@@ -1,24 +1,16 @@
 #pragma once
 
 #include "common.h"
+#include "wave.h"
 
 namespace dq {
 
 __host__ __device__ inline int gemm_splitk_kq(int n) { return ((n + 3) / 4 + 15) / 16 * 16; }
 
-template <bool TRANSA, int KQ>
-__device__ __forceinline__ void gemm_splitk_tile(const GemmDesc& g, int chain, int i0, int j0, double (*part)[4][64], int kq = KQ) {
+template <int KQ>
+__device__ __forceinline__ __attribute__((ext_vector_type(4))) double gemm_splitk_partial(const double* __restrict__ A, const double* __restrict__ B, const double* __restrict__ ks,
+                                                                                        bool transA, int n, int ia, int jb, bool ia_ok, bool jb_ok, int kbeg, int kk, int kq) {
     using d4 = __attribute__((ext_vector_type(4))) double;
-    const int n = g.n;
-    const double* __restrict__ A = g.A.at(chain);
-    const double* __restrict__ B = g.B.at(chain);
-    double* __restrict__ C = g.C.at(chain);
-    const double* __restrict__ ks = g.ks.p ? g.ks.at(chain) : nullptr;
-    const int lane = threadIdx.x & 63, wave = threadIdx.x >> 6;
-    const int r = lane & 15, kk = lane >> 4;
-    const int ia = min(i0 + r, n - 1), jb = min(j0 + r, n - 1);
-    const bool ia_ok = i0 + r < n, jb_ok = j0 + r < n;
-    const int kbeg = wave * kq;
     constexpr int NB = KQ / 16;
     double av[NB][4], bv[NB][4];
 #pragma unroll
@@ -28,7 +20,7 @@
         for (int s = 0; s < 4; ++s) {
             const int k = kbeg + 16 * b + 4 * kk + s;
             const int kc = min(k, n - 1);
-            double a = TRANSA ? A[kc + (long)n * ia] : A[ia + (long)n * kc];
+            double a = transA ? A[kc + (long)n * ia] : A[ia + (long)n * kc];
             double bb = B[kc + (long)n * jb];
             if (ks) a *= ks[kc];
             const bool ok = k < n;
@@ -43,19 +35,75 @@
 #pragma unroll
         for (int s = 0; s < 4; ++s) acc = __builtin_amdgcn_mfma_f64_16x16x4f64(bv[b][s], av[b][s], acc, 0, 0, 0);
     }
+    return acc;
+}
+__device__ __forceinline__ double gemm_splitk_finish(double p0, double p1, double p2, double p3, const double* rs, const double* cs, const double* old) {
+#pragma clang fp contract(off)
+    double v = p0 + p1 + p2 + p3;
+    if (rs) v *= *rs;
+    if (cs) v *= *cs;
+    if (old) v += *old;
+    return v;
+}
+
+template <bool TRANSA, int KQ, bool RIDERS = false>
+__device__ __forceinline__ void gemm_splitk_tile(const GemmDesc& g, int chain, int i0, int j0, double (*part)[4][64], int kq = KQ) {
+    using d4 = __attribute__((ext_vector_type(4))) double;
+    const int n = g.n;
+    double* __restrict__ C = g.C.at(chain);
+    const int lane = threadIdx.x & 63, wave = threadIdx.x >> 6;
+    const int r = lane & 15, kk = lane >> 4;
+    const int ia = min(i0 + r, n - 1), jb = min(j0 + r, n - 1);
+    const bool ia_ok = i0 + r < n, jb_ok = j0 + r < n;
+    const int j = j0 + kk + 4 * wave;
+    const bool mine = ia_ok && j < n;
+    double ts = 0.0, refv = 0.0;
+    if constexpr (RIDERS) {
+        if (g.TS.p) ts = g.TS.at(chain)[min(j, n - 1) + (long)n * ia];
+        if (g.ref.p) refv = g.ref.at(chain)[ia + (long)n * min(j, n - 1)];
+    }
+    const d4 acc = gemm_splitk_partial<KQ>(g.A.at(chain), g.B.at(chain), g.ks.p ? g.ks.at(chain) : nullptr, TRANSA, n, ia, jb, ia_ok, jb_ok, wave * kq, kk, kq);
 #pragma unroll
     for (int reg = 0; reg < 4; ++reg) part[wave][reg][lane] = acc[reg];
+    if constexpr (RIDERS) {
+        if (g.A2.p) {
+            const d4 acc2 = gemm_splitk_partial<KQ>(g.A2.at(chain), g.B2.at(chain), g.ks2.p ? g.ks2.at(chain) : nullptr, g.transA2 != 0, n, ia, jb, ia_ok, jb_ok, wave * kq, kk, kq);
+#pragma unroll
+            for (int reg = 0; reg < 4; ++reg) part[4 + wave][reg][lane] = acc2[reg];
+        }
+    }
     __syncthreads();
-    const double v4 = part[0][wave][lane] + part[1][wave][lane] + part[2][wave][lane] + part[3][wave][lane];
-    const int j = j0 + kk + 4 * wave;
-    if (ia_ok && j < n) {
-        double v = v4;
-        if (g.rs.p) v *= g.rs.at(chain)[i0 + r];
-        if (g.cs.p) v *= g.cs.at(chain)[j];
+    unsigned long long dev = 0ULL;
+    if (mine) {
         double* dst = C + (i0 + r) + (long)n * j;
-        if (g.accumulate) v += *dst;
+        double v = gemm_splitk_finish(part[0][wave][lane], part[1][wave][lane], part[2][wave][lane], part[3][wave][lane],
+                                      g.rs.p ? g.rs.at(chain) + i0 + r : nullptr, g.cs.p ? g.cs.at(chain) + j : nullptr, g.accumulate ? dst : nullptr);
+        if constexpr (RIDERS) {
+            if (g.A2.p) {
+                const double first = v;
+                v = gemm_splitk_finish(part[4][wave][lane], part[5][wave][lane], part[6][wave][lane], part[7][wave][lane],
+                                       g.rs2.p ? g.rs2.at(chain) + i0 + r : nullptr, g.cs2.p ? g.cs2.at(chain) + j : nullptr, &first);
+            }
+        }
         *dst = v;
         if (g.CT.p) g.CT.at(chain)[j + (long)n * (i0 + r)] = v;
+        if constexpr (RIDERS) {
+            if (g.TS.p) g.TSout.at(chain)[(i0 + r) + (long)n * j] = g.rs.p ? ts * g.rs.at(chain)[i0 + r] : ts;
+            if (g.ref.p) dev = (unsigned long long)__double_as_longlong(fabs(refv - v));
+        }
+    }
+    if constexpr (RIDERS) {
+        if (g.ref.p) {
+            __shared__ unsigned long long red[4];
+            dev = wave_max_u64(dev);
+            if (lane == 0) red[wave] = dev;
+            __syncthreads();
+            if (threadIdx.x == 0) {
+                unsigned long long m = red[0];
+                for (int q = 1; q < 4; ++q) m = red[q] > m ? red[q] : m;
+                atomicMax(g.err + (long)chain * g.err_stride + (blockIdx.x % GEMM_ERR_SHARDS), m);
+            }
+        }
     }
 }
 
diff --git a/dqmc_amd/csrc/lu_gj.hip b/dqmc_amd/csrc/lu_gj.hip
--- a/dqmc_amd/csrc/lu_gj.hip
+++ b/dqmc_amd/csrc/lu_gj.hip
@@ -280,6 +280,7 @@
                                                unsigned long long (*)[(NW + 1) & ~1] GST_ARGS) {}
 };
 constexpr int GJ_CMAX = 128;
+__host__ __device__ inline bool gj_panel_compacts(int n, int k0) { return k0 > 0 && n - k0 <= GJ_CMAX; }
 struct GjCompactShared {
     double rows[GJ_NB][GJ_CMAX];
     int orow[GJ_CMAX];
@@ -415,36 +416,35 @@
     for (int e = t; e < GJ_NB * GJ_NB; e += blockDim.x) (&sh.LU[0][0])[e] = ((e >> 5) == (e & 31)) ? 1.0 : 0.0;
     if (t == 0) sh.s_sing = 0;
     if (t < 2 * NWK) (&sh.slot_key[0][0])[t] = 0ULL;
-    if constexpr (CMP) {
-        if (cs != nullptr && nl <= GJ_CMAX) {
-            cs->pos[t] = -1;
-            if ((live & 1u) && rank < GJ_CMAX) {
-#pragma unroll
-                for (int c = 0; c < GJ_NB; ++c) cs->rows[c][rank] = a[0][c];
-                cs->orow[rank] = t;
-            }
-            lds_wait();
-            __builtin_amdgcn_s_barrier();
-            asm volatile("" ::: "memory");
-#ifdef DQ_GJ_STAMPS
-            asm volatile("s_memtime %0\n\ts_waitcnt lgkmcnt(0)" : "=s"(gstart) :: "memory");
-#endif
-            if (wave == 0) {
-                if (nl <= 64) gj_chain_cw<1>(*cs, sh.LU, sh.s_sing, myperm, nl, lane, nbw, k0);
-                else gj_chain_cw<2>(*cs, sh.LU, sh.s_sing, myperm, nl, lane, nbw, k0);
-            }
-#ifdef DQ_GJ_STAMPS
-            asm volatile("s_waitcnt lgkmcnt(0)\n\ts_memtime %0\n\ts_waitcnt lgkmcnt(0)" : "=s"(gsteps_end) :: "memory");
-            if (t == 0 && k0 == DQ_GJ_STAMP_K0 && blockIdx.x == 0 && blockIdx.y == 0)
-                printf("gj panel k0=%d grid.x=%d, compacted: %d live rows on one wave, clocks over %d steps incl. the read-back and the deposit: %llu\n", k0, (int)gridDim.x, nl, nbw, gsteps_end - gstart);
-#endif
-            lds_wait();
-            __builtin_amdgcn_s_barrier();
-            asm volatile("" ::: "memory");
-            mypos[0] = cs->pos[t];
-            return;
-        }
-    }
+    if constexpr (CMP) if (nl <= GJ_CMAX) {
+        cs->pos[t] = -1;
+        if ((live & 1u) && rank < GJ_CMAX) {
+#pragma unroll
+            for (int c = 0; c < GJ_NB; ++c) cs->rows[c][rank] = a[0][c];
+            cs->orow[rank] = t;
+        }
+        lds_wait();
+        __builtin_amdgcn_s_barrier();
+        asm volatile("" ::: "memory");
+#ifdef DQ_GJ_STAMPS
+        asm volatile("s_memtime %0\n\ts_waitcnt lgkmcnt(0)" : "=s"(gstart) :: "memory");
+#endif
+        if (wave == 0) {
+            if (nl <= 64) gj_chain_cw<1>(*cs, sh.LU, sh.s_sing, myperm, nl, lane, nbw, k0);
+            else gj_chain_cw<2>(*cs, sh.LU, sh.s_sing, myperm, nl, lane, nbw, k0);
+        }
+#ifdef DQ_GJ_STAMPS
+        asm volatile("s_waitcnt lgkmcnt(0)\n\ts_memtime %0\n\ts_waitcnt lgkmcnt(0)" : "=s"(gsteps_end) :: "memory");
+        if (t == 0 && k0 == DQ_GJ_STAMP_K0 && blockIdx.x == 0 && blockIdx.y == 0)
+            printf("gj panel k0=%d grid.x=%d, compacted: %d live rows on one wave, clocks over %d steps incl. the read-back and the deposit: %llu\n", k0, (int)gridDim.x, nl, nbw, gsteps_end - gstart);
+#endif
+        lds_wait();
+        __builtin_amdgcn_s_barrier();
+        asm volatile("" ::: "memory");
+        mypos[0] = cs->pos[t];
+        return;
+    }
+    constexpr bool VAL = NW == 4 && RPL == 1;
     lds_wait();
     __builtin_amdgcn_s_barrier();
     asm volatile("" ::: "memory");
@@ -453,7 +453,7 @@
     unsigned long long gst[8] = {0, 0, 0, 0, 0, 0, 0, 0}, gprev;
     asm volatile("s_waitcnt vmcnt(0)\n\ts_memtime %0\n\ts_waitcnt lgkmcnt(0)" : "=s"(gprev) :: "memory"); gstart = gprev;
 #endif
-    GjStepsMW<0, NW, RPL, CMP>::run(a, live, mypos, myperm, singular, lane, wave, nbw, k0, sh.slot_row, sh.slot_key GST_PASS);
+    GjStepsMW<0, NW, RPL, VAL>::run(a, live, mypos, myperm, singular, lane, wave, nbw, k0, sh.slot_row, sh.slot_key GST_PASS);
 #ifdef DQ_GJ_STAMPS
     gsteps_end = gprev;
     if (t == 0 && k0 == DQ_GJ_STAMP_K0 && blockIdx.x == 0 && blockIdx.y == 0)
@@ -476,7 +476,6 @@
 }
 __device__ __forceinline__ int gj_compact_rank(const int* rowpos, int n, int t, bool compact, int& nl) {
     int rank = 0;
-    nl = GJ_CMAX + 1;
     if (compact) {
         int tot = 0;
         const int lane = t & 63, wave = t >> 6;
@@ -497,9 +496,9 @@
 #define GJ_STAMP_VM(x) asm volatile("s_waitcnt vmcnt(0)\n\ts_memtime %0\n\ts_waitcnt lgkmcnt(0)" : "=s"(x) :: "memory")
 #endif
 
-template <int NW, int RPL>
+template <int NW, int RPL, bool CMP = false>
 __global__ __launch_bounds__(64 * NW) void gj_panel_mw_kernel(CMat Am, int* rowpos_p, long rowpos_stride, int* perm_p, long perm_stride, double* tinv_p,
-                                                          double* logabsdet, int accumulate, int* info, int n, int k0, int compact) {
+                                                          double* logabsdet, int accumulate, int* info, int n, int k0) {
     __shared__ __attribute__((aligned(16))) GjPanelShared<NW, RPL> sh;
     const int chain = blockIdx.y;
     const double* __restrict__ A = Am.at(chain);
@@ -516,12 +515,10 @@
     int oldpos[RPL], mypos[RPL], myperm;
     double a[RPL][GJ_NB];
     gj_panel_load<NW, RPL, false>(A, rowpos, n, k0, nbw, t, a, live, oldpos);
-    constexpr bool CMP = NW == 4 && RPL == 1;
     __shared__ __attribute__((aligned(16))) std::conditional_t<CMP, GjCompactShared, int> s_cs;
     GjCompactShared* cs = nullptr;
-    if constexpr (CMP) { if (compact) cs = &s_cs; }
-    int nl = GJ_CMAX + 1;
-    const int rank = CMP ? gj_compact_rank(rowpos, n, t, cs != nullptr && k0 > 0 && n - k0 <= GJ_CMAX, nl) : 0;
+    int nl = GJ_CMAX + 1, rank = 0;
+    if constexpr (CMP) { cs = &s_cs; rank = gj_compact_rank(rowpos, n, t, gj_panel_compacts(n, k0), nl); }
 #ifdef DQ_GJ_STAMPS
     gj_panel_factor<NW, RPL, CMP>(sh, a, live, mypos, myperm, t, nbw, k0, cs, nl, rank, gstart, gprev);
 #else
@@ -656,9 +653,9 @@
         if (st_ok[reg]) dst[row0 + kk + 4 * reg + coff] = cold[reg] - acc[reg];
 }
 
-template <int NW, int RPL>
+template <int NW, int RPL, bool CMP = false>
 __global__ __launch_bounds__(64 * NW) void gj_step_kernel(Mat Am, Mat Bm, Mat SAm, Mat Xm, const int* rowpos_old_p, int* rowpos_new_p, long rowpos_stride,
-                                                          double* logabsdet, int accumulate, int* info, int n, int k0, int nA, int nS, int nCA, int compact) {
+                                                          double* logabsdet, int accumulate, int* info, int n, int k0, int nA, int nS, int nCA) {
     static_assert(NW == 4, "the update's 2 x 2 waves are the panel's");
     __shared__ __attribute__((aligned(16))) GjPanelShared<NW, RPL> sh;
     __shared__ __attribute__((aligned(16))) double s_inv[4 * 256];
@@ -682,12 +679,10 @@
     int oldpos[RPL], mypos[RPL], myperm;
     double a[RPL][GJ_NB];
     gj_panel_load<NW, RPL, true>(A, rowpos_old, n, k0, nbw, t, a, live, oldpos);
-    constexpr bool CMP = NW == 4 && RPL == 1;
     __shared__ __attribute__((aligned(16))) std::conditional_t<CMP, GjCompactShared, int> s_cs;
     GjCompactShared* cs = nullptr;
-    if constexpr (CMP) { if (compact) cs = &s_cs; }
-    int nl = GJ_CMAX + 1;
-    const int rank = CMP ? gj_compact_rank(rowpos_old, n, t, cs != nullptr && k0 > 0 && n - k0 <= GJ_CMAX, nl) : 0;
+    int nl = GJ_CMAX + 1, rank = 0;
+    if constexpr (CMP) { cs = &s_cs; rank = gj_compact_rank(rowpos_old, n, t, gj_panel_compacts(n, k0), nl); }
 
     const int row_tiles = nA + nS + 1;
     const int rt = blockIdx.x % row_tiles, ct = blockIdx.x / row_tiles;
@@ -831,20 +826,22 @@
             const int nbw = n - k0 < GJ_NB ? n - k0 : GJ_NB;
             const int nA = (n + 31) / 32, nS = k0 / 32;
             const int nCA = (n - k0 - nbw + 31) / 32, nCB = (n + 31) / 32;
-            hipLaunchKernelGGL((gj_step_kernel<4, 1>), dim3((nA + nS + 1) * (nCA + nCB), n_chains), dim3(256), 0, s, A, B, SA, X, (const int*)((p & 1) ? rowpos_alt : rowpos),
-                               (p & 1) ? rowpos : rowpos_alt, rowpos_stride, logabsdet, accumulate_logdet, info, n, k0, nA, nS, nCA, compact ? 1 : 0);
+#define DQ_GJ_STEP(CMP) hipLaunchKernelGGL((gj_step_kernel<4, 1, CMP>), dim3((nA + nS + 1) * (nCA + nCB), n_chains), dim3(256), 0, s, A, B, SA, X, (const int*)((p & 1) ? rowpos_alt : rowpos), \
+                               (p & 1) ? rowpos : rowpos_alt, rowpos_stride, logabsdet, accumulate_logdet, info, n, k0, nA, nS, nCA)
+            if (compact && gj_panel_compacts(n, k0)) DQ_GJ_STEP(true); else DQ_GJ_STEP(false);
+#undef DQ_GJ_STEP
         }
         DQ_HIP(hipGetLastError());
         return 0;
     }
     for (int k0 = 0; k0 < n; k0 += GJ_NB) {
         const dim3 pg(1, n_chains);
-#define DQ_GJ_PANEL(NW, RPL) hipLaunchKernelGGL((gj_panel_mw_kernel<NW, RPL>), pg, dim3(RPL == 1 ? 64 * ((n + 63) / 64) : 64 * NW), 0, s, CMat(A), rowpos, rowpos_stride, perm, perm_stride, tinv, logabsdet, accumulate_logdet, info, n, k0, compact ? 1 : 0)
-        if (n > 768) DQ_GJ_PANEL(8, 2);
-        else if (n > 576) DQ_GJ_PANEL(4, 3);
-        else if (n > 512) DQ_GJ_PANEL(3, 3);
-        else if (n > 256) DQ_GJ_PANEL(4, 2);
-        else if (n > 64) DQ_GJ_PANEL(4, 1);
+#define DQ_GJ_PANEL(NW, RPL, CMP) hipLaunchKernelGGL((gj_panel_mw_kernel<NW, RPL, CMP>), pg, dim3(RPL == 1 ? 64 * ((n + 63) / 64) : 64 * NW), 0, s, CMat(A), rowpos, rowpos_stride, perm, perm_stride, tinv, logabsdet, accumulate_logdet, info, n, k0)
+        if (n > 768) DQ_GJ_PANEL(8, 2, false);
+        else if (n > 576) DQ_GJ_PANEL(4, 3, false);
+        else if (n > 512) DQ_GJ_PANEL(3, 3, false);
+        else if (n > 256) DQ_GJ_PANEL(4, 2, false);
+        else if (n > 64) { if (compact && gj_panel_compacts(n, k0)) DQ_GJ_PANEL(4, 1, true); else DQ_GJ_PANEL(4, 1, false); }
         else hipLaunchKernelGGL((gj_panel_kernel<1>), pg, dim3(64), 0, s, CMat(A), rowpos, rowpos_stride, perm, perm_stride, tinv, logabsdet, accumulate_logdet, info, n, k0);
         const int nbw = n - k0 < GJ_NB ? n - k0 : GJ_NB;
         const int nA = (n + 31) / 32, nS = k0 / 32;
diff --git a/dqmc_amd/csrc/qr.hip b/dqmc_amd/csrc/qr.hip
--- a/dqmc_amd/csrc/qr.hip
+++ b/dqmc_amd/csrc/qr.hip
@@ -286,7 +286,7 @@
 #undef DQ_FQ
 }
 
-__global__ void assemble_r_kernel(CMat Am, const int* jpvt_p, long jpvt_stride, Vec dv, Mat Rm, int n) {
+__global__ void assemble_r_kernel(CMat Am, const int* jpvt_p, long jpvt_stride, Vec dv, Mat Rm, int n, Vec dl, Vec ds) {
     const int chain = blockIdx.y;
     const double* __restrict__ A = Am.at(chain);
     const int* jpvt = jpvt_p + (long)chain * jpvt_stride;
@@ -299,7 +299,15 @@
         if (r <= j) val = A[r + (long)n * col] / fabs(A[r + (long)n * jpvt[r]]);
         R[r + (long)n * col] = val;
     }
-    if (threadIdx.x == 0) d[j] = fabs(A[j + (long)n * col]);
+    if (threadIdx.x == 0) {
+        const double v = fabs(A[j + (long)n * col]);
+        d[j] = v;
+        if (dl.p) {
+            const bool large = v >= 1.0;
+            dl.at(chain)[j] = large ? 1.0 / v : 1.0;
+            ds.at(chain)[j] = large ? 1.0 : v;
+        }
+    }
 }
 
 int qr_init_device() {
@@ -315,7 +323,8 @@
 int launch_qrcp_colown(Mat A, QrWork w, int n, int n_chains, hipStream_t s);
 
 static int launch_assemble_r(Mat A, Vec d, Mat R, const QrWork& w, int n, int n_chains, hipStream_t s) {
-    hipLaunchKernelGGL(assemble_r_kernel, dim3(n, n_chains), dim3(128), 0, s, CMat(A), (const int*)w.jpvt, w.jpvt_stride, d, R, n);
+    hipLaunchKernelGGL(assemble_r_kernel, dim3(n, n_chains), dim3(128), 0, s, CMat(A), (const int*)w.jpvt, w.jpvt_stride, d, R, n, Vec{w.dl, w.split_stride},
+                       Vec{w.ds, w.split_stride});
     DQ_HIP(hipGetLastError());
     return 0;
 }
```

Result: no change. 13.85 sweeps/s, median of 6 (+0.6%).
